# ultravideo/kvazzup

Hardware: AMD Instinct MI355X
Metric: hevc_encode_decode_fps (higher is better)
Workload: dtype u8

## Files before the change

### kvazzup_amd/csrc/enc_kernels.h

```cpp
#pragma once
#include <hip/hip_runtime.h>
#include "hevc_core.h"
namespace kvzx {
void launch_pad_input(const uint8_t *in, int w, int h, uint8_t *dy, uint8_t *du, uint8_t *dv, int cw, int ch, hipStream_t st);
void launch_me(const EncFrame &f, hipStream_t st);
void launch_luma_quarter(const uint8_t *src, uint8_t *q, int cw, int ch, hipStream_t st);
void launch_me_coarse(const EncFrame &f, hipStream_t st);
void launch_subpel(const EncFrame &f, hipStream_t st);
void launch_inter_recon(const EncFrame &f, hipStream_t st);
void launch_inter_signal(const EncFrame &f, hipStream_t st);
void launch_intra_analyse(const EncFrame &f, hipStream_t st);
void launch_intra_recon(const EncFrame &f, hipStream_t st);
void launch_deblock(const EncFrame &f, hipStream_t st);
void launch_vaq(const EncFrame &f, int vaq, int *act, int *sum, hipStream_t st);
void launch_sao(const EncFrame &f, hipStream_t st);
void launch_qp_resolve(const EncFrame &f, hipStream_t st);
void launch_deblock_v(const EncFrame &f, hipStream_t st);
void launch_deblock_h(const EncFrame &f, hipStream_t st, int part = 0);
void launch_tokenize(const EncFrame &f, hipStream_t st);
void launch_tok_compact(const EncFrame &f, hipStream_t st);
void launch_picture_begin(RcState *rc, uint32_t bits3, int slot3, int have3, int8_t *ctu_qt, const int8_t *roi, int nctu, int qp, int vaq, hipStream_t st,
                          void *zero_a = nullptr, size_t bytes_a = 0, void *zero_b = nullptr, size_t bytes_b = 0);
struct WpArgs {
  const unsigned long long *partial; int nblk;
  long long n;
  int64_t *stat;
  const int64_t *stat_ref[KVZ_MAX_LP_REFS];
  const uint8_t *in_ref[KVZ_MAX_LP_REFS];
  int nref;
  int32_t *cand; unsigned long long *acc;
  int32_t *rec, *rec_host;
};
struct WpPlaneArgs { const int32_t *rec; const uint8_t *from[KVZ_MAX_LP_REFS]; uint8_t *to[KVZ_MAX_LP_REFS]; };
int wp_stat_blocks(int height);
void launch_wp_stats(const uint8_t *src, int cw, int width, int height, unsigned long long *partial, hipStream_t st);
void launch_wp_decide(const WpArgs &a, int phase, hipStream_t st);
void launch_wp_check(const WpArgs &a, const uint8_t *cur, int cw, int width, int height, hipStream_t st);
void launch_wp_plane(const WpPlaneArgs &a, int nref, int cw, int ch, hipStream_t st);
struct CabacRowsArgs {
  const uint16_t *tok; const int32_t *count; const uint32_t *off;
  uint8_t *stage; uint32_t stage_cap;
  uint8_t *out; uint32_t out_cap;
  uint32_t *cursors;
  uint32_t *sub_off, *sub_len, *sub_bins;
  uint32_t *ctx_save, *ctx_ready;
  uint32_t gen;
  uint32_t *err;
  int wc, hc, wpp, tile_rows, init_type, qp, first_sub;
};
void launch_cabac_rows(const CabacRowsArgs &a, int nsub, hipStream_t st);
}
```

### kvazzup_amd/csrc/enc_kernels.hip

```cpp
#include <hip/hip_runtime.h>
#include <type_traits>
#include "hevc_core.h"
#include "enc_kernels.h"
#include "kernel_common.h"

namespace kvzx {

#define SPLIT_BITS 8
#define INTRA_P_GATE 24
#define INTRA_P_BITS 16

#define ME_MAXR 32
#define ME_WPITCH 100

template <bool MR, bool CO = false>
__global__ __launch_bounds__(256) void k_me(EncFrame f)
{
  using Key = typename std::conditional<MR || CO, unsigned long long, uint32_t>::type;
  constexpr int KS = CO ? 17 : (MR ? 16 : 13);
  constexpr Key KMAX = ~(Key)0;
  __shared__ __attribute__((aligned(16))) uint8_t wbuf[(32 + 2 * ME_MAXR + 1) * ME_WPITCH + 16];
  __shared__ __attribute__((aligned(16))) uint32_t cur[32 * 8];
  __shared__ Key red[5];
  const int tid = threadIdx.x, nthreads = blockDim.x;
  int bx_, by_; xcd_block_2d(bx_, by_);
  const int x0 = bx_ * 32, y0 = by_ * 32 + f.row0 * 64;
  const int R = f.range, W = 2 * R + 1, WW = 32 + 2 * R;
  const uint8_t *ref = f.me_ref, *src = f.src[0];
  const uint32_t lam = (uint32_t)f.lambda_q4;
  if (f.pb_on && blockIdx.x == 0 && blockIdx.y == 0) picture_begin_body(f.pb_rc, f.pb_bits3, f.pb_slot3, f.pb_have3, f.pb_qt, f.pb_roi, f.pb_nctu, f.qp, 0, tid, nthreads);
  if (tid == 0) red[0] = 0;
  __syncthreads();
  {
    uint32_t s0 = 0;
    for (int i = tid; i < 256; i += nthreads) {
      const size_t g = (size_t)(y0 + (i >> 3)) * f.cw + x0 + (i & 7) * 4;
      const uint32_t c = *reinterpret_cast<const uint32_t *>(src + g);
      cur[i] = c;
      if (f.me_early) s0 = __builtin_amdgcn_sad_u8(c, *reinterpret_cast<const uint32_t *>(ref + g), s0);
    }
    if (f.me_early) { s0 = wave_sum_u32(s0); if ((tid & 63) == 0) atomicAdd(&red[0], (Key)s0); }
  }
  __syncthreads();
  if (f.me_early && red[0] <= 64u * lam) {
    if (tid < 16) {
      const int i = b8idx(f, x0 + (tid & 3) * 8, y0 + (tid >> 2) * 8);
      f.cu_log2[i] = 5; f.cu_intra[i] = 0; f.cu_mv[i * 2] = 0; f.cu_mv[i * 2 + 1] = 0;
      f.cu_mvp_idx[i] = 0;
      if (MR) f.cu_ref[i] = 0;
    }
    if (f.intra_p && tid < 4) f.me_cost16[((y0 >> 4) + (tid >> 1)) * (f.cw >> 4) + (x0 >> 4) + (tid & 1)] = 0;
    return;
  }
  Key best[5] = {KMAX, KMAX, KMAX, KMAX, KMAX};
  const int nr = MR ? f.nref : 1;
#pragma unroll 1
  for (int it = 0; it < (CO ? 2 * nr : nr); it++) {
// ... 655 lines not shown
  __syncthreads();
  {
    auto px1 = [](int tu, int y, int x) { return tu * 256 + y * 16 + x; };
    auto px4 = [](int tu, int y, int x) { return (tu >> 2) * 256 + (((tu >> 1) & 1) * 8 + y) * 16 + (tu & 1) * 8 + x; };
    const size_t base = (size_t)(y0 >> 1) * cw2 + (x0 >> 1);
    int16_t *cb = f.coef[1] + base, *cr = f.coef[2] + base;
    auto ci1 = [=](int tu, int y, int x) { return (tu ? cr : cb) + (size_t)y * cw2 + x; };
    auto ci4 = [=](int tu, int y, int x) { return ((tu >> 2) ? cr : cb) + (size_t)(((tu >> 1) & 1) * 8 + y) * cw2 + (tu & 1) * 8 + x; };
    auto qpc_known = [&]() -> int { return qpc; };
    if constexpr (LL) { }
    else if (split) inter_transform<DEC, 3, 1, RC>(s, qpc, &s.nz[1], px4, ci4, tid, adj, qpc_known, &rc_cost, f.scaling ? f.scaling + scaling_offset(3, 1, 1) : nullptr, 4);
    else inter_transform<DEC, 4, 1, RC>(s, qpc, &s.nz[1], px1, ci1, tid, adj, qpc_known, &rc_cost, f.scaling ? f.scaling + scaling_offset(4, 1, 1) : nullptr, 1);
  }
  if (tid < 128) {
    const int pl = tid >> 6, y = (tid >> 2) & 15, x = (tid & 3) * 4;
    *(uint32_t *)&f.rec[1 + pl][(size_t)((y0 >> 1) + y) * cw2 + (x0 >> 1) + x] = *(const uint32_t *)&s.px[pl * 256 + y * 16 + x];
  }
  if (!DEC && tid < 16) {
    int bx = tid & 3, by = tid >> 2, k = split ? ((by >> 1) * 2 + (bx >> 1)) : 0;
    int cbf = (int)((s.nz[0] >> k) & 1);
    if (split) cbf |= (int)((s.nz[1] >> k) & 1) << 1 | (int)((s.nz[1] >> (4 + k)) & 1) << 2;
    else cbf |= (int)(s.nz[1] & 1) << 1 | (int)((s.nz[1] >> 1) & 1) << 2;
    f.cu_cbf[b8idx(f, x0 + bx * 8, y0 + by * 8)] = (uint8_t)cbf;
  }
  if constexpr (RC) rc_group_done(f, s, grp, rc_cost, tid);
}

template <bool TMVP, bool GOP = false>
__global__ __launch_bounds__(1024) void k_inter_signal(EncFrame f)
{
  const int w8 = f.cw >> 3, h8 = band_rows(f) * 8;
  const int i = blockIdx.x * blockDim.x + threadIdx.x;
  const bool valid = i < w8 * h8;
  const int x = valid ? (i % w8) * 8 : 0, y = valid ? (i / w8) * 8 + f.row0 * 64 : 0, g = b8idx(f, x, y);
  const int cl = f.cu_log2[g];
  const bool intra = f.cu_intra[g] != 0;
  int flags = 0;
  if (valid && !intra) {
    const int n = 1 << cl;
    CuSignal r;
    if constexpr (GOP) { FrameMvView v{f}; [[clang::always_inline]] r = decide_signalling_values(v, f.cw, f.chp, x & ~(n - 1), y & ~(n - 1), cl, f.cu_ref && f.nref > 1 ? f.nref : 1, TMVP ? f.col_prev : nullptr, TabDist{f.ref_dist}); }
    else if constexpr (TMVP) { FrameMvView v{f}; [[clang::always_inline]] r = decide_signalling_values(v, f.cw, f.chp, x & ~(n - 1), y & ~(n - 1), cl, f.cu_ref && f.nref > 1 ? f.nref : 1, f.col_prev); }
    else r = decide_signalling_values(f, x & ~(n - 1), y & ~(n - 1), cl);
    flags = r.flags;
    f.cu_flags[g] = (uint8_t)r.flags; f.cu_merge_idx[g] = (uint8_t)r.midx; f.cu_mvp_idx[g] = (uint8_t)r.mvp;
    *reinterpret_cast<uint32_t *>(&f.cu_mvd[g * 2]) = ((uint32_t)r.mvdx & 0xffffu) | ((uint32_t)r.mvdy << 16);
  }
  if constexpr (TMVP) {
    if (valid && !((x | y) & 15)) {
      ColMv c; c.mx = intra ? 0 : f.cu_mv[g * 2]; c.my = intra ? 0 : f.cu_mv[g * 2 + 1]; c.dist = intra ? 0 : (int16_t)(GOP ? TabDist{f.ref_dist}(cu_ref_at(f, g)) : cu_ref_at(f, g) + 1); c.pad = 0;
      f.col_out[(y >> 4) * (f.cw >> 4) + (x >> 4)] = c;
    }
  }
  if (f.tok_list) {
    uint32_t roles = 0;
    if (valid && !((x | y) & 15)) {
      const bool owner = !(cl == 5 && ((x | y) & 31));
      if (owner || ((x & 63) == 48 && (y & 63) == 48)) roles |= 8u;
      if (owner) {
        uint32_t cbf = 0;
        if (cl == 3) { cbf = f.cu_cbf[g] | f.cu_cbf[g + 1] | f.cu_cbf[g + w8] | f.cu_cbf[g + w8 + 1]; }
        else if (!(flags & CU_SKIP)) cbf = f.cu_cbf[g];
        roles |= cbf & 7u;
      }
    }
    const int lane = threadIdx.x & 63, nr = __builtin_popcount(roles);
    int pre = nr;
    for (int o = 1; o < 64; o <<= 1) { const int t = __shfl_up(pre, o); if (lane >= o) pre += t; }
    const int total = __shfl(pre, 63);
    uint32_t base = 0;
    if (lane == 63 && total) base = atomicAdd(&f.tok_list[0], (uint32_t)total);
    base = (uint32_t)__shfl((int)base, 63);
    uint32_t o = base + (uint32_t)(pre - nr);
    const uint32_t unit = (uint32_t)((y >> 4) * (f.cw >> 4) + (x >> 4));
    for (uint32_t m = roles; m; m &= m - 1) f.tok_list[1 + o++] = (unit << 2) | (uint32_t)__builtin_ctz(m);
  }
}

#ifdef KVZ_PROF
__shared__ long long g_prof[16];
#define PROF(k) do { if (threadIdx.x == 0) { long long t_ = clock64(); g_prof[k] += t_ - g_prof[15]; g_prof[15] = t_; } } while (0)
#else
#define PROF(k) do { } while (0)
#endif
struct IntraCtuLds {
  alignas(16) uint8_t pic[65 * 144];
  alignas(16) uint8_t src[64 * 64];
  alignas(16) int16_t lev[64 * 64];
  alignas(16) XfLaneF16 xf[4][64];
};


struct AnalyseLds {
  alignas(16) uint8_t src[32 * 32];
  alignas(16) uint8_t R[2][16 * 36 + 4 * 68 + 132];
  int dc[21];
  uint32_t cost[21][35];
  uint32_t bestc[21]; int bestm[21];
  int last;
  alignas(16) uint8_t srcT[32 * 32];
  alignas(16) uint8_t ext[16][4 * 32];
};
__device__ __forceinline__ int an_tile_of(int b) { return b < 16 ? (b >> 3) * 2 + ((b >> 1) & 1) : b - 16; }
__device__ __forceinline__ int an_roff(int b) { return b < 16 ? b * 36 : (b < 20 ? 16 * 36 + (b - 16) * 68 : 16 * 36 + 4 * 68); }

template <int L2>
__device__ __forceinline__ uint32_t analyse_item(const AnalyseLds &s, int b, int bx, int by, int mode, int lane)
{
  constexpr int N = 1 << L2;
  const bool filt = intra_filter_needed(N, 0, mode);
  const uint8_t *R = s.R[filt ? 1 : 0] + an_roff(b);
  const int angle = kIntraAngle[mode], inv = kInvAngle[mode];
  const bool edge = N < 32, vert = mode >= 18, e2 = edge && (mode == 26 || mode == 10);
  const int dcv = s.dc[b];
  uint32_t sad = 0;
#pragma unroll
  for (int it = 0; it < N * N / 64; it++) {
    const int pxi = it * 64 + lane, y = pxi >> L2, x = pxi & (N - 1);
    int p;
    if (mode == 0) p = pred_planar<L2>(R, x, y);
    else if (mode == 1) p = pred_dc<L2>(R, edge, dcv, x, y);
    else p = pred_angular<L2>(R, vert, e2, angle, inv, x, y);
    sad += (uint32_t)iabs((int)s.src[(by + y) * 32 + bx + x] - p);
  }
  return wave_sum_u32(sad);
}

__device__ __forceinline__ void analyse_tile_satd(AnalyseLds &s, int wave, int tile, int kind, int mode, int lane, uint32_t (&q)[4])
{
// ... 639 lines not shown
    } else *(uint32_t *)g = *(const uint32_t *)&ty_[y * P + x];
  }
  for (int i = tid; i < 2 * (TH / 2) * 9; i += 256) {
    const int pl = i / ((TH / 2) * 9), r = i - pl * ((TH / 2) * 9), y = r / 9, k = r - y * 9, gx = CX0 - 2 + 4 * k, gy = CY0 + y;
    if (gy < 0 || gx < 0) continue;
    uint8_t *g = &f.rec[1 + pl][(size_t)gy * cw2 + gx];
    const uint32_t v = *(const uint32_t *)&tc_[pl][y * PC + 4 * k];
    if (k == 0) *(uint16_t *)(g + 2) = (uint16_t)(v >> 16);
    else if (k == 8 && TW == 64) *(uint16_t *)g = (uint16_t)v;
    else *(uint32_t *)g = v;
  }
}

__global__ __launch_bounds__(256) void k_deblock_v(EncFrame f)
{
  int t = blockIdx.x * blockDim.x + threadIdx.x;
  int ne = (f.cw >> 3) - 1, ns = band_rows(f) * 16;
  if (t >= ne * ns) return;
  int x = ((t % ne) + 1) * 8, y = (t / ne) * 4 + f.row0 * 64;
  if (!is_cu_edge_v(f, x, y)) return;
  int bs = edge_bs(f, x - 1, y, x, y);
  if (!bs) return;
  const int qp = (cu_qpy(f, x - 1, y) + cu_qpy(f, x, y) + 1) >> 1;
  deblock_luma_segment(f.rec[0] + y * f.cw + x, 1, f.cw, bs, qp);
  if (bs == 2 && (x & 15) == 0) {
    int cw2 = f.cw >> 1;
    deblock_chroma_segment(f.rec[1] + (y >> 1) * cw2 + (x >> 1), 1, cw2, 2, qp);
    deblock_chroma_segment(f.rec[2] + (y >> 1) * cw2 + (x >> 1), 1, cw2, 2, qp);
  }
}
__global__ __launch_bounds__(256) void k_deblock_h(EncFrame f, int part)
{
  int t = blockIdx.x * blockDim.x + threadIdx.x;
  const int ylo = imax(8, f.row0 * 64), yhi = imin(f.ch - 8, (f.row0 + band_rows(f)) * 64);
  int ns = f.cw >> 2, ne = (yhi - ylo) / 8 + 1;
  if (t >= ne * ns) return;
  int x = (t % ns) * 4, y = ylo + (t / ns) * 8;
  if (part) {
    const bool boundary = y == f.row0 * 64 || y == (f.row0 + band_rows(f)) * 64;
    if (boundary != (part == 2)) return;
  }
  if (!is_cu_edge_h(f, x, y)) return;
  int bs = edge_bs(f, x, y - 1, x, y);
  if (!bs) return;
  const int qp = (cu_qpy(f, x, y - 1) + cu_qpy(f, x, y) + 1) >> 1;
  deblock_luma_segment(f.rec[0] + y * f.cw + x, f.cw, 1, bs, qp);
  if (bs == 2 && (y & 15) == 0) {
    int cw2 = f.cw >> 1;
    deblock_chroma_segment(f.rec[1] + (y >> 1) * cw2 + (x >> 1), cw2, 1, 2, qp);
    deblock_chroma_segment(f.rec[2] + (y >> 1) * cw2 + (x >> 1), cw2, 1, 2, qp);
  }
}

struct TileView {
  const CuRec *tile;
  int bx0, by0;
  __device__ CuRec at(int x, int y) const { return tile[((y >> 3) - by0) * 3 + ((x >> 3) - bx0)]; }
};

struct alignas(16) TokTabs { uint8_t sigk[3][5][16]; };
constexpr CoreTabs make_core_tabs() { CoreTabs t{}; for (int i = 0; i < 64; i++) core_tabs_fill_entry(t, i); return t; }
constexpr TokTabs make_tok_tabs()
{
  const CoreTabs c = make_core_tabs();
  TokTabs t{};
  for (int sc = 0; sc < 3; sc++) for (int k = 0; k < 16; k++) {
    for (int pc = 0; pc < 4; pc++) t.sigk[sc][pc][k] = c.sigpat[pc][c.pos4[sc][k]];
    t.sigk[sc][4][k] = c.ctxmap4x4[c.pos4[sc][k]];
  }
  return t;
}
static __device__ const CoreTabs g_core_tabs = make_core_tabs();
static __device__ const TokTabs g_tok_tabs = make_tok_tabs();
static_assert(sizeof(CoreTabs) % 4 == 0 && sizeof(TokTabs) % 16 == 0, "copied by dwords / 16-byte words");

struct SbRegs { uint32_t w[8]; uint32_t m; };
__device__ __forceinline__ int sb_level(const SbRegs &r, int k) { return (int)(int16_t)(uint16_t)(r.w[k >> 1] >> ((k & 1) * 16)); }

template <bool KEEP_LDS>
__device__ __forceinline__ void digest_build_wave(const CoreTabs *t, TuDigest &d, const int16_t *lv, int stride, int log2, int scan_idx, int lane, SbRegs &sb)
{
  const int sbl = log2 - 2, nsb2 = 1 << (2 * sbl);
  d.csbf[lane] = 0;
  wave_sync();
  bool nz = false;
  sb.m = 0;
#pragma unroll
  for (int k = 0; k < 8; k++) sb.w[k] = 0;
  if (lane < nsb2) {
    int xs, ys; scan_pos(t, scan_idx, sbl, lane, xs, ys);
    const int16_t *p = lv + (ys << 2) * stride + (xs << 2);
    uint2 r0 = *reinterpret_cast<const uint2 *>(p), r1 = *reinterpret_cast<const uint2 *>(p + stride);
    uint2 r2 = *reinterpret_cast<const uint2 *>(p + 2 * stride), r3 = *reinterpret_cast<const uint2 *>(p + 3 * stride);
    uint2 *dst = reinterpret_cast<uint2 *>(&d.scan[lane * 16]);
    dst[0] = r0; dst[1] = r1; dst[2] = r2; dst[3] = r3;
    const uint8_t *pos = t->pos4[scan_idx];
    int v[16];
    uint32_t m = 0;
#pragma unroll
    for (int k = 0; k < 16; k++) { v[k] = d.scan[lane * 16 + pos[k]]; if (v[k]) m |= 1u << k; }
#pragma unroll
    for (int k = 0; k < 8; k++) sb.w[k] = ((uint32_t)v[2 * k] & 0xffffu) | ((uint32_t)v[2 * k + 1] << 16);
    if (KEEP_LDS) {
      uint32_t *d32 = reinterpret_cast<uint32_t *>(&d.scan[lane * 16]);
#pragma unroll
      for (int k = 0; k < 8; k++) d32[k] = sb.w[k];
    }
    sb.m = m;
    d.mask[lane] = (uint16_t)m;
    nz = m != 0;
    if (nz) d.csbf[ys * 8 + xs] = 1;
  }
  uint64_t sb64 = __ballot(nz);
  if (lane == 0) d.sbmask = sb64;
  wave_sync();
}

__device__ __forceinline__ bool sb_g1_any(const SbRegs &r)
{
  bool any = false; int seen = 0;
#pragma unroll
  for (int k = 15; k >= 0; k--) if ((r.m >> k) & 1) { const int v = sb_level(r, k); if (seen < 8 && (v > 1 || v < -1)) any = true; seen++; }
  return any;
}

template <class S>
__device__ __forceinline__ void enc_subblock_regs(S &c, const TuDigest &d, const SbRegs &r, const uint32_t (&sk)[4], int i, int last_sb, int last_pos, bool prev_g1, int log2, int cidx, int scan_idx, int sign_hiding)
{
  const int sbl = log2 - 2, nsb = 1 << sbl;
  int xs, ys; scan_pos(c.tabs, scan_idx, sbl, i, xs, ys);
  const int right = (xs < nsb - 1) ? d.csbf[ys * 8 + xs + 1] : 0;
  const int below = (ys < nsb - 1) ? d.csbf[(ys + 1) * 8 + xs] : 0;
  const uint32_t m = r.m;
  int coded = m != 0, infer_dc = 0;
  if (i < last_sb && i > 0) {
    cabac_bin(c, CTX_CSBF + ((right | below) ? 1 : 0) + (cidx ? 2 : 0), coded);
    infer_dc = 1;
  } else coded = 1;
  if (!coded) return;
  const int sigbase = CTX_SIG + (cidx ? 27 : 0);
  const int off = log2 == 2 ? 0 : (cidx == 0 ? ((i > 0 ? 3 : 0) + ((log2 == 3) ? ((scan_idx == 0) ? 9 : 15) : 21)) : ((log2 == 3) ? 9 : 12));
  const int start = (i == last_sb) ? last_pos - 1 : 15;
  if constexpr (sink_counts_only<S>::value) {
    if (start >= 0) c.n += start + 1 - ((infer_dc && (m >> 1) == 0) ? 1 : 0);
  } else {
#pragma unroll
    for (int k = 15; k >= 1; k--) if (k <= start) cabac_bin(c, sigbase + (int)((sk[k >> 2] >> ((k & 3) * 8)) & 0xffu) + off, (int)((m >> k) & 1));
    if (start >= 0 && !(infer_dc && (m >> 1) == 0))
      cabac_bin(c, sigbase + ((i == 0 && log2 != 2) ? 0 : (int)(sk[0] & 0xffu) + off), (int)(m & 1));
  }
  if (!m) return;
  int ctx_set = (i > 0 && cidx == 0) ? 2 : 0;
  if (prev_g1) ctx_set++;
  int c1 = 1, nsig = 0, g1idx = -1, g2 = 0;
  uint32_t signs = 0;
#pragma unroll
  for (int k = 15; k >= 0; k--) if ((m >> k) & 1) {
    const int v = sb_level(r, k), a = v < 0 ? -v : v;
    signs = (signs << 1) | (v < 0 ? 1u : 0u);
    if (nsig < 8) {
      const int g1 = a > 1;
      cabac_bin(c, CTX_GT1 + (cidx ? 16 : 0) + ctx_set * 4 + c1, g1);
      if (g1) { c1 = 0; if (g1idx < 0) { g1idx = nsig; g2 = a > 2; } }
      else if (c1 > 0 && c1 < 3) c1++;
    }
    nsig++;
  }
  if (g1idx >= 0) cabac_bin(c, CTX_GT2 + (cidx ? 4 : 0) + ctx_set, g2);
  if (sign_hiding && (31 - __builtin_clz(m)) - __builtin_ctz(m) > 3) cabac_bypass_bits(c, signs >> 1, nsig - 1);
  else cabac_bypass_bits(c, signs, nsig);
  int rice = 0, j = 0;
#pragma unroll
  for (int k = 15; k >= 0; k--) if ((m >> k) & 1) {
    const int v = sb_level(r, k), a = v < 0 ? -v : v;
    const int base = (j < 8) ? ((j == g1idx) ? 3 : 2) : 1;
    if (a >= base) {
      enc_abs_remaining(c, a - base, rice);
      if (a > 3 * (1 << rice)) rice = imin(rice + 1, 4);
    }
    j++;
  }
}

#define TOK_HDR_CAP 192
#define TOK_ARENA 512
#define TOK_PIECES 17

#ifndef KVZ_TOK_WAVES
#define KVZ_TOK_WAVES 5
#endif
struct alignas(16) TokWave {
  TuDigest dg;
  TokTabs tk;
  CoreTabs tabs;
  CuRec tile[9];
  uint16_t hdr[TOK_HDR_CAP];
  uint16_t arena[TOK_ARENA];
  int hdr_n;
  uint32_t piece_off;
  uint32_t seg[TOK_PIECES][2];
};
template <bool ALLC, bool HDRW, bool REGS>
__device__ __forceinline__ void tok_unit(const EncFrame &f, TokWave &W, const int ux, const int uy, const int comp, const int lane, const bool have_tabs)
{
  CuRec *tile = W.tile; TuDigest &dg = W.dg; CoreTabs &tabs = W.tabs; uint16_t *hdr = W.hdr, *arena = W.arena;
  int &hdr_n = W.hdr_n; uint32_t &piece_off = W.piece_off; uint32_t (&seg)[TOK_PIECES][2] = W.seg;
  const int wc = f.cw >> 6, hc = f.ch >> 6;
  const int hdr_comp = HDRW ? 3 : 0;
  const bool hdr_role = ALLC || comp == hdr_comp;
  const int cx = ux >> 2, cy = uy >> 2, ctu = cy * wc + cx;
  const int X0 = ux * 16, Y0 = uy * 16;
  int z4 = 0;
  for (int b = 0; b < 2; b++) z4 |= (((ux & 3) >> b) & 1) << (2 * b) | (((uy & 3) >> b) & 1) << (2 * b + 1);
  unsigned long long *tr = (f.trace && hdr_role && lane == 0 && (z4 == 0 || z4 == 15)) ? f.trace + (size_t)wc * hc * 32 + (size_t)ctu * 8 : nullptr;
  if (tr) tr[z4 == 0 ? 5 : 6] = wall_clock64();
  unsigned long long *census = f.trace ? f.trace + (size_t)wc * hc * 40 + (size_t)ctu * 16 + (f.is_intra ? 6 : 0) : nullptr;
  const unsigned long long t_begin = census ? wall_clock64() : 0;
  int wave_class = 1;
#ifdef KVZ_TOK_PHASES
  unsigned long long *ph = (f.trace && comp == 0 && !f.is_intra) ? f.trace + (size_t)wc * hc * 56 + (size_t)ctu * 16 : nullptr;
  unsigned long long ph_t[9]; int ph_n = 0;
#define TOK_PH() do { if (ph && ph_n < 9) ph_t[ph_n++] = wall_clock64(); } while (0)
#define TOK_PH_SYNC() wave_sync()
#else
#define TOK_PH() do { } while (0)
#define TOK_PH_SYNC() do { } while (0)
#endif
  TOK_PH();
  auto mine = [&](int piece) { return ALLC || ((piece == 16 || (piece & 3) == 0) ? hdr_comp : (piece & 3) - 1) == comp; };
  if (!(hdr_role && z4 == 15)) {
    const int g0 = (uy * 2) * f.b8w + ux * 2, l0 = f.cu_log2[g0];
    bool work = !(l0 == 5 && ((X0 | Y0) & 31));
    if (!ALLC && work && comp != hdr_comp) {
      bool c = false;
      if (lane < (l0 == 3 ? 4 : 1)) { const int g = g0 + (lane >> 1) * f.b8w + (lane & 1); c = !(f.cu_flags[g] & CU_SKIP) && ((f.cu_cbf[g] >> comp) & 1); }
      work = __ballot(c) != 0;
    }
    if (!work) {
      if (lane < TOK_PIECES && mine(lane)) { uint32_t *e = f.tok_seg + ((size_t)(ctu * 16 + z4) * TOK_PIECES + lane) * 2; e[0] = 0; e[1] = 0; }
      if (census && lane == 0) { atomicAdd(&census[0], 1ull); atomicAdd(&census[1], wall_clock64() - t_begin); }
      return;
    }
  }
  TOK_PH();
  if (!have_tabs) {
    for (int i = lane; i < (int)(sizeof(CoreTabs) / 4); i += 64) reinterpret_cast<uint32_t *>(&tabs)[i] = reinterpret_cast<const uint32_t *>(&g_core_tabs)[i];
    if (lane < (int)(sizeof(TokTabs) / 16)) reinterpret_cast<uint4 *>(&W.tk)[lane] = reinterpret_cast<const uint4 *>(&g_tok_tabs)[lane];
  }
  if (lane < TOK_PIECES) { seg[lane][0] = 0; seg[lane][1] = 0; }
  if (lane == 0) hdr_n = 0;
  const int bx0 = ux * 2 - 1, by0 = uy * 2 - 1;
  if (lane < 9) {
    int bx = bx0 + lane % 3, by = by0 + lane / 3;
    CuRec r; r.log2 = 0; r.intra = 0; r.flags = 0; r.merge_idx = 0; r.mvp_idx = 0; r.intra_mode = 0; r.cbf = 0; r.ref = 0; r.mvdx = 0; r.mvdy = 0;
    if (bx >= 0 && by >= 0) {
      int g = by * f.b8w + bx;
      r.log2 = f.cu_log2[g]; r.intra = f.cu_intra[g]; r.flags = f.cu_flags[g]; r.merge_idx = f.cu_merge_idx[g];
      r.mvp_idx = f.cu_mvp_idx[g]; r.intra_mode = f.cu_intra_mode[g]; r.cbf = f.cu_cbf[g];
      r.mvdx = f.cu_mvd[g * 2]; r.mvdy = f.cu_mvd[g * 2 + 1]; r.ref = (uint8_t)cu_ref_at(f, g);
    }
    tile[lane] = r;
  }
  wave_sync();
  TOK_PH();
  uint16_t *slot = f.tok_buf + (size_t)ctu * f.tok_cap;
  int np = 0;
  auto reserve = [&](int total) -> uint32_t {
    if (lane == 0) {
      uint32_t o = atomicAdd(&f.tok_cursor[ctu], (uint32_t)total);
      if (o + (uint32_t)total > (uint32_t)f.tok_cap) { atomicOr(f.err, 16u); o = ~0u; }
      else { seg[np][0] = o; seg[np][1] = (uint32_t)total; }
      piece_off = o;
    }
    wave_sync();
    return piece_off;
  };
  TileView v; v.tile = tile; v.bx0 = bx0; v.by0 = by0;
  const int cl0 = v.at(X0, Y0).log2;
  const bool owner = !(cl0 == 5 && ((X0 | Y0) & 31));
  const int ncu = owner ? (cl0 == 3 ? 4 : 1) : 0;
  for (int k = 0; k < ncu; k++) {
    const int x0 = X0 + ((cl0 == 3) ? (k & 1) * 8 : 0), y0 = Y0 + ((cl0 == 3) ? (k >> 1) * 8 : 0);
    const CuRec cu = v.at(x0, y0);
    int z = 0;
    for (int b = 0; b < 3; b++) z |= ((((x0 & 63) >> 3) >> b) & 1) << (2 * b) | ((((y0 & 63) >> 3) >> b) & 1) << (2 * b + 1);
    if (lane == 0 && hdr_role) {
      TokOut t; t.tabs = &tabs; t.p = hdr; t.n = 0; t.cap = TOK_HDR_CAP;
      if (f.sao && z4 == 0 && k == 0) {
        const bool hl = cx > 0 && !tile_col_starts_at(wc, f.tile_cols, cx), hu = cy > 0 && !tile_row_starts_at(hc, f.tile_rows, cy);
        enc_sao(t, f.sao[ctu], hl ? &f.sao[ctu - 1] : nullptr, hu ? &f.sao[ctu - wc] : nullptr);
      }
      enc_split_flags(v, t, f.cw, f.chp, x0, y0, z, cu.log2);
      enc_cu_header(v, t, f.cw, f.chp, f.is_intra != 0, x0, y0, cu, f.lossless != 0, f.cu_ref ? f.nref : 1);
      if (f.ctu_qy && !(cu.flags & CU_SKIP) && cu.cbf && z == f.ctu_first[ctu]) enc_cu_qp_delta(t, f.ctu_delta[ctu]);
      hdr_n = t.n;
    }
    TOK_PH_SYNC(); TOK_PH();
    if (hdr_role) {
      np = 4 * k;
      wave_sync();
      const int hn = hdr_n > TOK_HDR_CAP ? TOK_HDR_CAP : hdr_n;
      if (hdr_n > TOK_HDR_CAP && lane == 0) atomicOr(f.err, 8u);
      const uint32_t o = reserve(hn);
      if (o != ~0u) for (int i = lane; i < hn; i += 64) slot[o + i] = hdr[i];
      wave_sync();
      if (lane == 0) hdr_n = 0;
      wave_sync();
    }
    const int cbf = (cu.flags & CU_SKIP) ? 0 : cu.cbf;
    for (int ci = (ALLC || comp == 3) ? 0 : comp; ci < (ALLC ? 3 : (comp == 3 ? 0 : comp + 1)); ci++) {
      np = 4 * k + 1 + ci;
      if ((cbf >> ci) & 1) {
        wave_class = 2;
        const int l2 = ci ? cu.log2 - 1 : cu.log2, pw = ci ? (f.cw >> 1) : f.cw;
        const int px = ci ? (x0 >> 1) : x0, py = ci ? (y0 >> 1) : y0;
        const int scan = intra_scan_idx(cu.intra, l2, ci, cu.intra_mode);
        SbRegs sb;
        digest_build_wave<!REGS>(&tabs, dg, f.coef[ci] + py * pw + px, pw, l2, scan, lane, sb);
        TOK_PH();
        const uint64_t sbm = dg.sbmask;
        const int last_sb = 63 - __builtin_clzll(sbm);
        const int last_pos = 31 - __builtin_clz((uint32_t)dg.mask[last_sb]);
        if (lane == 0) {
          TokOut t; t.tabs = &tabs; t.p = hdr; t.n = hdr_n; t.cap = TOK_HDR_CAP;
          int a, b; enc_last_pos(t, dg, l2, ci, scan, a, b);
          hdr_n = t.n;
        }
        const bool nzsb = (sbm >> lane) & 1;
        const bool g1 = nzsb && sb_g1_any(sb);
        const uint64_t g1m = __ballot(g1);
        bool prev_g1 = false;
        if (lane <= last_sb) {
          uint64_t above = (lane < 63) ? (sbm >> (lane + 1)) : 0;
          if (above) { int j = lane + 1 + __builtin_ctzll(above); prev_g1 = (g1m >> j) & 1; }
        }
        uint32_t sk[4] = {0, 0, 0, 0};
        if (lane <= last_sb) {
          const int sbl = l2 - 2, nsb = 1 << sbl;
          int xs, ys; scan_pos(&tabs, scan, sbl, lane, xs, ys);
          const int right = (xs < nsb - 1) ? dg.csbf[ys * 8 + xs + 1] : 0, below = (ys < nsb - 1) ? dg.csbf[(ys + 1) * 8 + xs] : 0;
          const uint4 q = *reinterpret_cast<const uint4 *>(W.tk.sigk[scan][l2 == 2 ? 4 : (right | (below << 1))]);
          sk[0] = q.x; sk[1] = q.y; sk[2] = q.z; sk[3] = q.w;
        }
        int n_l = 0;
        if (lane <= last_sb) {
          TokCount t; t.tabs = &tabs; t.n = 0;
          if (REGS) enc_subblock_regs(t, dg, sb, sk, lane, last_sb, last_pos, prev_g1, l2, ci, scan, f.signhide);
          else enc_subblock(t, dg, lane, last_sb, last_pos, prev_g1, l2, ci, scan, f.signhide);
          n_l = t.n;
        }
        int suffix = n_l;
        for (int o = 1; o < 64; o <<= 1) { int other = __shfl_down(suffix, o); if (lane + o < 64) suffix += other; }
        const int body = __shfl(suffix, 0);
        const int off = suffix - n_l;
        wave_sync();
        const int hn = hdr_n > TOK_HDR_CAP ? TOK_HDR_CAP : hdr_n, total = hn + body;
        if (hdr_n > TOK_HDR_CAP && lane == 0) atomicOr(f.err, 8u);
        TOK_PH();
        const uint32_t o = reserve(total);
        TOK_PH();
        if (o != ~0u) {
          const bool staged = total <= TOK_ARENA;
          uint16_t *dst = staged ? arena : slot + o;
          for (int i = lane; i < hn; i += 64) dst[i] = hdr[i];
          if (lane <= last_sb && n_l) {
            TokOut t; t.tabs = &tabs; t.p = dst + hn + off; t.n = 0; t.cap = n_l;
            if (REGS) enc_subblock_regs(t, dg, sb, sk, lane, last_sb, last_pos, prev_g1, l2, ci, scan, f.signhide);
            else enc_subblock(t, dg, lane, last_sb, last_pos, prev_g1, l2, ci, scan, f.signhide);
          }
          if (staged) {
            wave_sync();
            for (int i = lane; i < total; i += 64) slot[o + i] = arena[i];
          }
        }
        wave_sync();
        TOK_PH();
        if (lane == 0) hdr_n = 0;
      }
      wave_sync();
    }
  }
  if (z4 == 15 && hdr_role) {
    const bool last = (cy == hc - 1 && cx == wc - 1);
    const bool row_end = tile_col_ends_at(wc, f.tile_cols, cx);
    const bool sub_end = row_end && (f.wpp || tile_row_ends_at(hc, f.tile_rows, cy));
    const bool seg_end = last || (row_end && (f.slices == 1 || (f.slices == 2 && tile_row_ends_at(hc, f.tile_rows, cy))));
    const int n = 1 + ((sub_end && !seg_end) ? 1 : 0);
    wave_sync();
    np = 16;
    const uint32_t o = reserve(n);
    if (o != ~0u && lane == 0) {
      slot[o] = (uint16_t)(0xC000u | (seg_end ? 1u : 0u));
      if (n == 2) slot[o + 1] = 0xC001u;
    }
  }
  wave_sync();
  if (lane < TOK_PIECES && mine(lane)) {
    uint32_t *e = f.tok_seg + ((size_t)(ctu * 16 + z4) * TOK_PIECES + lane) * 2;
    e[0] = seg[lane][0]; e[1] = seg[lane][1];
  }
  TOK_PH();
#ifdef KVZ_TOK_PHASES
  if (ph && lane == 0 && ph_n == 9 && ncu == 1 && wave_class == 2) { for (int k = 0; k < 8; k++) atomicAdd(&ph[k], ph_t[k + 1] - ph_t[k]); atomicAdd(&ph[15], 1ull); }
#endif
#undef TOK_PH
#undef TOK_PH_SYNC
  if (tr && z4 == 15) tr[7] = wall_clock64();
  if (census && lane == 0) { atomicAdd(&census[wave_class * 2], 1ull); atomicAdd(&census[wave_class * 2 + 1], wall_clock64() - t_begin); }
}
template <bool ALLC, int NW, bool HDRW = true, bool REGS = true, bool LIST = false>
__global__ __launch_bounds__(NW * 64) __attribute__((amdgpu_waves_per_eu(REGS ? (LIST ? 3 : KVZ_TOK_WAVES) : 6))) void k_tokenize(EncFrame f)
{
  __shared__ TokWave tw[NW];
  const int wv = threadIdx.x >> 6, lane = threadIdx.x & 63;
  TokWave &W = tw[wv];
  if constexpr (LIST) {
    const uint32_t count = f.tok_list[0], uw = (uint32_t)(f.cw >> 4);
    bool have = false;
    for (uint32_t it = blockIdx.x; it < count; it += gridDim.x) {
      const uint32_t v = f.tok_list[1 + it], unit = v >> 2;
      tok_unit<ALLC, HDRW, REGS>(f, W, (int)(unit % uw), (int)(unit / uw), (int)(v & 3u), lane, have);
      have = true;
      wave_sync();
    }
  } else {
    const int ux = NW == 4 ? blockIdx.x * 2 + (wv & 1) : blockIdx.x, uy = NW == 4 ? (blockIdx.y + f.row0 * 2) * 2 + (wv >> 1) : blockIdx.y + f.row0 * 4, comp = ALLC ? 0 : (int)blockIdx.z;
    tok_unit<ALLC, HDRW, REGS>(f, W, ux, uy, comp, lane, false);
  }
}

__global__ __launch_bounds__(256) void k_tok_compact(EncFrame f)
{
  constexpr int NSEG = 16 * TOK_PIECES;
  __shared__ uint32_t soff[NSEG], start[NSEG + 1], utot[17];
  __shared__ uint32_t wsum[4];
  const int first = f.row0 * (f.cw >> 6), ctu = blockIdx.x + first, tid = threadIdx.x;
  unsigned long long *tr = f.trace ? f.trace + (size_t)(f.cw >> 6) * (f.ch >> 6) * 32 + (size_t)ctu * 8 : nullptr;
#define TC_STAMP(k) do { if (tr && tid == 0) tr[k] = wall_clock64(); } while (0)
  TC_STAMP(0);
  const uint32_t n = f.tok_cursor[ctu];
  uint32_t part = 0;
  for (int i = first + tid; i < ctu; i += 256) part += f.tok_cursor[i];
  part = wave_sum_u32(part);
  if ((tid & 63) == 0) wsum[tid >> 6] = part;
  if (tid == 0) { f.tok_cursor_next[ctu] = 0; if (blockIdx.x == 0) { *f.err_out = *f.err; if (f.ent_cursors) { f.ent_cursors[0] = 0; f.ent_cursors[1] = 0; } } }
  __syncthreads();
  const uint32_t base = wsum[0] + wsum[1] + wsum[2] + wsum[3];
  TC_STAMP(1);
  uint32_t *tab = f.tok_seg + (size_t)ctu * NSEG * 2;
  for (int i = tid; i < NSEG; i += 256) { const uint2 e = *reinterpret_cast<const uint2 *>(&tab[i * 2]); soff[i] = e.x; start[i] = e.y; *reinterpret_cast<uint2 *>(&tab[i * 2]) = make_uint2(0u, 0u); }
  if (f.tok_list && blockIdx.x == 0 && tid == 0) f.tok_list[0] = 0;
  if (base + n > f.tok_dense_cap) { if (tid == 0) f.tok_count_out[ctu] = -1; return; }
  __syncthreads();
  TC_STAMP(2);
  if (tid < 16) { uint32_t a = 0; for (int p = 0; p < TOK_PIECES; p++) { uint32_t l = start[tid * TOK_PIECES + p]; start[tid * TOK_PIECES + p] = a; a += l; } utot[tid] = a; }
  __syncthreads();
  if (tid == 0) { uint32_t a = 0; for (int u = 0; u < 16; u++) { uint32_t t = utot[u]; utot[u] = a; a += t; } utot[16] = a; }
  __syncthreads();
  for (int i = tid; i < NSEG; i += 256) start[i] += utot[i / TOK_PIECES];
  if (tid == 0) start[NSEG] = utot[16];
  __syncthreads();
  const uint32_t total = start[NSEG];
  TC_STAMP(3);
  if (total != n) { if (tid == 0) f.tok_count_out[ctu] = -1; return; }
  const uint16_t *slot = f.tok_buf + (size_t)ctu * f.tok_cap;
  uint16_t *dst = f.tok_dense + base;
  int lo = 0;
  for (uint32_t i = tid; i < n; i += 256) {
    if (start[lo + 1] <= i) {
      int hi = NSEG;
      while (hi - lo > 1) { int mid = (lo + hi) >> 1; if (start[mid] <= i) lo = mid; else hi = mid; }
    }
    dst[i] = slot[soff[lo] + (i - start[lo])];
  }
  if (tid == 0) { f.tok_off_out[ctu] = base; f.tok_count_out[ctu] = (int32_t)n; }
  TC_STAMP(4);
#undef TC_STAMP
}

__global__ __launch_bounds__(256) void k_pad_input(const uint8_t *in, int w, int h, uint8_t *dy, uint8_t *du, uint8_t *dv, int cw, int ch)
{
  int y0 = blockIdx.y * 16 + threadIdx.y * 4, plane = 0;
  if (y0 >= ch) { y0 -= ch; plane = 1; if (y0 >= ch / 2) { y0 -= ch / 2; plane = 2; } }
  const int pw = plane ? w / 2 : w, ph = plane ? h / 2 : h, pcw = plane ? cw / 2 : cw;
  const int x = (blockIdx.x * 64 + threadIdx.x) * 16;
  if (x >= pcw) return;
  const uint8_t *src = in + (plane == 0 ? 0 : (plane == 1 ? (size_t)w * h : (size_t)w * h + (size_t)(w / 2) * (h / 2)));
  uint8_t *dst = plane == 0 ? dy : (plane == 1 ? du : dv);
  kv_u32x4 v[4];
#pragma unroll
  for (int k = 0; k < 4; k++) {
    const uint8_t *row = src + (size_t)imin(y0 + k, ph - 1) * pw;
    if (x + 16 <= pw && (((uintptr_t)(row + x)) & 3) == 0) v[k] = *reinterpret_cast<const kv_u32x4 *>(row + x);
    else {
      uint32_t q[4] = {0, 0, 0, 0};
      for (int i = 0; i < 16; i++) q[i >> 2] |= (uint32_t)row[imin(x + i, pw - 1)] << (8 * (i & 3));
      v[k].x = q[0]; v[k].y = q[1]; v[k].z = q[2]; v[k].w = q[3];
    }
  }
#pragma unroll
  for (int k = 0; k < 4; k++) *reinterpret_cast<kv_u32x4 *>(dst + (size_t)(y0 + k) * pcw + x) = v[k];
}

#define KVZ_SAO_THREADS 1024
struct SaoLds {
  alignas(4) uint8_t win[66 * 72];
  alignas(4) uint8_t winc[2][34 * 40];
  int en[3][4][5], es[3][4][5], bn[3][32][16], bs[3][32][16];
  int eo_off[3][4][4], eo_dist[3][4][4], bo_off[3][32], bo_gain[3][32];
  int cand_dist[3][5], cand_bins[3][5], cand_band[3];
  SaoParams p;
};
__device__ __forceinline__ int sao_edge_idx(int c, int a, int b)
{
  const int e = 2 + ((c > a) - (c < a)) + ((c > b) - (c < b));
  return e == 2 ? 0 : (e < 2 ? e + 1 : e);
}
__device__ __forceinline__ int sao_rdiv(int a, int b) { return b == 0 ? 0 : (a >= 0 ? (2 * a + b) / (2 * b) : -((-2 * a + b) / (2 * b))); }
__device__ __forceinline__ int sao_off_bins(int o) { const int a = o < 0 ? -o : o; return a < 7 ? a + 1 : 7; }

template <int ROWS>
__device__ __forceinline__ void sao_stats_column(SaoLds &s, int c, const uint8_t *w, int pitch, int x, int ys, bool okh, int Y0, int ph, const int *o8, int tid)
{
  auto sgn = [](int d) { return d > 1 ? 1 : (d < -1 ? -1 : d); };
  const uint8_t *col = w + 4 + x - 1;
  int r0[3], r1[3], r2[3];
  for (int k = 0; k < 3; k++) { r0[k] = col[ys * pitch + k]; r1[k] = col[(ys + 1) * pitch + k]; }
  uint64_t acc[4] = {0, 0, 0, 0};
  int run_b = -1, run_n = 0, run_s = 0;
  int s_up = sgn(r1[1] - r0[1]);
// ... 284 lines not shown
void launch_intra_recon(const EncFrame &f, hipStream_t st)
{
  static const int diags_env = getenv("KVAZZUP_AMD_INTRA_DIAGS") ? atoi(getenv("KVAZZUP_AMD_INTRA_DIAGS")) : -1;
  const int diags = diags_env >= 0 ? diags_env : (f.chain_diags ? f.chain_diags : 3);
  const int wc = f.cw / 64, nr = band_rows(f), diag = nr < (wc + 1) / 2 ? nr : (wc + 1) / 2, want = diags > 0 ? 3 * diags * diag + 32 : 3 * wc * nr;
  const dim3 grid(want < 3 * wc * nr ? want : 3 * wc * nr), block(64 * KVZ_INTRA_WAVES);
  const bool adj = f.rdoq || f.signhide;
  if (!f.is_intra) {
    const dim3 all(3 * wc * nr);
    if (f.lossless) { hipLaunchKernelGGL((k_intra_recon<false, true, false, true>), all, block, 0, st, f); return; }
    if (f.scaling) { if (adj) hipLaunchKernelGGL((k_intra_recon<true, true, true>), all, block, 0, st, f); else hipLaunchKernelGGL((k_intra_recon<false, true, true>), all, block, 0, st, f); }
    else if (adj) hipLaunchKernelGGL((k_intra_recon<true, true>), all, block, 0, st, f); else hipLaunchKernelGGL((k_intra_recon<false, true>), all, block, 0, st, f);
    return;
  }
  if (f.lossless) hipLaunchKernelGGL((k_intra_recon<false, false, false, true>), grid, block, 0, st, f);
  else if (f.scaling) { if (adj) hipLaunchKernelGGL((k_intra_recon<true, false, true>), grid, block, 0, st, f); else hipLaunchKernelGGL((k_intra_recon<false, false, true>), grid, block, 0, st, f); }
  else if (adj) hipLaunchKernelGGL((k_intra_recon<true, false>), grid, block, 0, st, f);
  else hipLaunchKernelGGL((k_intra_recon<false, false>), grid, block, 0, st, f);
}
void launch_qp_resolve(const EncFrame &f, hipStream_t st)
{
  if (!f.ctu_qy) return;
  const int n = (f.cw / 64) * band_rows(f);
  if (f.wpp && f.cw / 64 <= 256) { hipLaunchKernelGGL(k_qp_rows, dim3(band_rows(f)), dim3(256), 0, st, f); return; }
  hipLaunchKernelGGL(k_qp_first, dim3(n), dim3(64), 0, st, f);
  hipLaunchKernelGGL(k_qp_chain, dim3((n + 255) / 256), dim3(256), 0, st, f);
}
void launch_deblock_v(const EncFrame &f, hipStream_t st)
{
  int nv = ((f.cw >> 3) - 1) * (band_rows(f) * 16);
  hipLaunchKernelGGL(k_deblock_v, dim3((nv + 255) / 256), dim3(256), 0, st, f);
}
void launch_deblock_h(const EncFrame &f, hipStream_t st, int part)
{
  const int ylo = imax(8, f.row0 * 64), yhi = imin(f.ch - 8, (f.row0 + band_rows(f)) * 64);
  int nh = (f.cw >> 2) * ((yhi - ylo) / 8 + 1);
  hipLaunchKernelGGL(k_deblock_h, dim3((nh + 255) / 256), dim3(256), 0, st, f, part);
}
void launch_deblock(const EncFrame &f, hipStream_t st)
{
  if (f.nrows > 0) { launch_deblock_v(f, st); launch_deblock_h(f, st, 0); return; }
  hipLaunchKernelGGL(k_deblock_tile, dim3((f.cw / 64) * (f.ch / 64)), dim3(256), 0, st, f);
}
void launch_vaq(const EncFrame &f, int vaq, int *act, int *sum, hipStream_t st)
{
  const int nctu = (f.cw / 64) * (f.ch / 64);
  hipMemsetAsync(sum, 0, sizeof(int), st);
  hipLaunchKernelGGL(k_vaq_stats, dim3(nctu), dim3(256), 0, st, f, act, sum);
  hipLaunchKernelGGL(k_vaq_apply, dim3((nctu + 255) / 256), dim3(256), 0, st, f, vaq, (const int *)act, (const int *)sum, nctu);
}
void launch_sao(const EncFrame &f, hipStream_t st) { hipLaunchKernelGGL(k_sao<false>, dim3((f.cw / 64) * (f.ch / 64)), dim3(KVZ_SAO_THREADS), 0, st, f); }
void launch_tokenize(const EncFrame &f, hipStream_t st)
{
  const int units = (f.cw / 16) * band_rows(f) * 4;
  static const int list_mode = [] { const char *e = getenv("KVAZZUP_AMD_TOK_LIST"); return e ? atoi(e) : -1; }();
  if (!f.is_intra && f.tok_list && f.nrows == 0 && units < 65536 && (list_mode > 0 || (list_mode < 0 && units > 16384))) {
    hipLaunchKernelGGL((k_tokenize<false, 1, true, true, true>), dim3(units / 2 < 256 ? 256 : units / 2), dim3(64), 0, st, f);
    return;
  }
  if (units >= 65536) hipLaunchKernelGGL((k_tokenize<true, 1>), dim3(f.cw / 16, band_rows(f) * 4), dim3(64), 0, st, f);
  else if (units > 16384) hipLaunchKernelGGL((k_tokenize<false, 1, false, false>), dim3(f.cw / 16, band_rows(f) * 4, 3), dim3(64), 0, st, f);
  else hipLaunchKernelGGL((k_tokenize<false, 1, true>), dim3(f.cw / 16, band_rows(f) * 4, 4), dim3(64), 0, st, f);
}
void launch_tok_compact(const EncFrame &f, hipStream_t st)
{
  hipLaunchKernelGGL(k_tok_compact, dim3((f.cw / 64) * band_rows(f)), dim3(256), 0, st, f);
}

}
```

### kvazzup_amd/csrc/encoder.h

```cpp
#pragma once
#include <hip/hip_runtime.h>
#include <stdint.h>
#include <condition_variable>
#include <deque>
#include <mutex>
#include <string>
#include <thread>
#include <vector>
#include "hevc_core.h"
#include "hevc_headers.h"
#include "entropy_host.h"
#include "enc_kernels.h"

namespace kvzx {

enum KernelId { K_PAD = 0, K_ME, K_INTER_RECON, K_INTER_SIGNAL, K_INTRA_ANALYSE, K_INTRA_RECON, K_DEBLOCK, K_TOKENIZE, K_HOST_ARITH, K_SAO, K_TOK_COMPACT, K_CABAC_ROWS, K_SUBPEL, K_INTRA_ANALYSE_P, K_INTRA_RECON_P, K_COUNT };

struct EncoderConfig {
  int width = 0, height = 0;
  int qp = 32, intra_period = 64, vps_period = 1;
  int me_range = 16;
  int fps_num = 30, fps_den = 1;
  int wpp = 1, deblock = 1;
  int band_row0 = 0, band_rows = 0;
// ... 100 lines not shown
  hipEvent_t ev_h2d_[kInRing] = {}, ev_pad_[kInRing] = {}; bool pad_pending_[kInRing] = {}, h2d_pending_[kInRing] = {};
  long in_count_ = 0;
  hipStream_t stream_rec_ = nullptr;
  static constexpr int kSets = 8;
  uint8_t *src_[kSets][3] = {};
  static constexpr int kMaxDepth = 16;
  static constexpr int kMaxRefDist = kSets - 1;
  static constexpr int kRecRing = kMaxDepth + 2 + kMaxRefDist;
  uint8_t *rec_[kRecRing][3] = {};
  bool spin_wait_ = false;
  int rc_delay_ = 3;
  int nrec_ = 3;
  int cur_idx_ = 0, ref_idx_ = 2, out_idx_ = 2;
  int16_t *coef_[kSets][3] = {};
  uint8_t *cu_bytes_[kSets] = {};
  int16_t *cu_mv_[kSets] = {}, *cu_mvd_[kSets] = {};
  uint8_t *cu_ref_[kSets] = {};
  uint8_t *mc_q_[kSets] = {}; int16_t *mc_centres_[kSets] = {};
  ColMv *col_[kSets] = {};
  int set_ = 0, out_set_ = 0;
  int32_t out_gop_[8] = {0, 0, 0, 0, 0, 0, 0, 0};
  unsigned long long *wp_partial_[kSets] = {}; int64_t *wp_stat_[kSets] = {}; int32_t *wp_rec_[kSets] = {};
  int32_t *wp_cand_ = nullptr; unsigned long long *wp_acc_ = nullptr; uint8_t *wp_plane_[KVZ_MAX_LP_REFS] = {};
  int32_t out_wp_[3 * KVZ_MAX_LP_REFS] = {0, 64, 0, 0, 64, 0, 0, 64, 0, 0, 64, 0};
  bool wp_stage(const EncFrame &f, const Plan &p, const Slot &sl);
  EncFrame wp_search_frame(const EncFrame &f, const Plan &p, hipStream_t st);
  char prio_[3] = {'h', 'n', 'n'};
  std::vector<int8_t> roi_; int roi_w_ = 0, roi_h_ = 0;
  std::vector<int8_t> roi_sub_; int roi_sub_w_ = 0, roi_sub_h_ = 0;
  int8_t *ctu_qt_[kSets] = {}, *ctu_qy_[kSets] = {}, *ctu_delta_[kSets] = {}; uint8_t *ctu_first_[kSets] = {};
  int8_t *h_ctu_qt_[kSets] = {};
  int8_t *ctu_roi_[kSets] = {};
  bool stage_roi(hipStream_t st);
  const int8_t *roi_dev_ = nullptr;
  int *vaq_act_ = nullptr, *vaq_sum_ = nullptr;
  uint32_t next_chain_gen();
  bool picture_begin(const EncFrame &f, hipStream_t qt_stream, EncFrame *fold = nullptr, bool zero = false);
  int qp_cur_ = 0; int64_t rc_debt_ = 0; uint32_t rc_bytes_[8] = {0, 0, 0, 0, 0, 0, 0, 0}; uint32_t rc_known_ = 0;
  void rate_control();
  RcState *rc_state_ = nullptr;
  bool band_picture_setup();
  EncFrame band_f_{};
  hipStream_t stream_tok_ = nullptr;
  hipStream_t stream_in_ = nullptr;
  hipEvent_t ev_src_free_[kSets] = {}; bool src_busy_[kSets] = {};
  uint8_t *work_[3] = {nullptr, nullptr, nullptr};
  SaoParams *sao_[kSets] = {};

  hipStream_t stream_idr_ = nullptr; hipEvent_t ev_idr_done_ = nullptr; bool idr_pending_ = false, idr_side_ = false, all_intra_alt_ = false;
  uint32_t *sync_idr_ = nullptr; uint32_t *edge_col_idr_ = nullptr; uint32_t chain_gen_ = 0; unsigned long long *edge_row_ = nullptr, *edge_row_idr_ = nullptr; uint8_t *work_idr_[3] = {nullptr, nullptr, nullptr};
  hipEvent_t ev_signalled_ = nullptr, ev_tok_done_[kSets] = {}; bool tok_pending_[kSets] = {};
  uint8_t *intra_scratch_ = nullptr;
  uint8_t *d_scaling_ = nullptr;
  uint16_t *tok_buf_ = nullptr; int tok_cap_ = 0; int32_t *tok_count_ = nullptr; uint32_t *tok_seg_ = nullptr; uint32_t *tok_list_ = nullptr; int tok_nctu_ = 0;
  size_t tok_dense_cap_ = 0;
  std::vector<std::vector<uint8_t>> band_subs_; uint64_t band_bins_ = 0; bool band_coded_ = false;
  bool me_ahead_ = false; uint32_t *me_block_[kSets] = {}; uint32_t *sync_set_[kSets] = {}; int prev_set_ = 0;
  uint32_t *sync_ = nullptr; uint32_t *me_cost16_ = nullptr; uint32_t *edge_col_ = nullptr; uint32_t *intra_order_ = nullptr; uint32_t *err_ = nullptr; unsigned long long *trace_ = nullptr;
  struct EvPair { hipEvent_t a, b; KernelId id; };
  struct Slot {
    uint16_t *h_tok_dense = nullptr, *d_tok_dense = nullptr; int32_t *h_tok_count = nullptr, *d_tok_count = nullptr;
    uint32_t *h_tok_off = nullptr, *d_tok_off = nullptr;
    uint32_t *h_err = nullptr, *d_err = nullptr;
    int32_t *h_wp = nullptr, *d_wp = nullptr;
    uint16_t *g_tok = nullptr; int32_t *g_count = nullptr; uint32_t *g_off = nullptr;
    uint8_t *g_stage = nullptr; uint32_t *g_cursors = nullptr, *g_ctx_save = nullptr, *g_ctx_ready = nullptr;
    uint8_t *h_out = nullptr, *d_out = nullptr; uint32_t *h_sub = nullptr, *d_sub = nullptr;
    hipStream_t ent_stream = nullptr; hipEvent_t tok_ev = nullptr; uint32_t gen = 0;
    hipEvent_t done = nullptr, rec_done = nullptr;
    hipEvent_t sink_done = nullptr; bool has_sink = false;
    int poc = 0, rec_idx = 0, set = 0, qp = 0; bool intra = false, write_ps = false; long pic_idx = 0;
    int layer = 0, nref = 0; int8_t dist[KVZ_MAX_LP_REFS] = {0, 0, 0, 0};
    std::vector<EvPair> ev; size_t ev_used = 0;
    EncodedPicture result; bool ready = false, ok = true;
    EncFrame f_tok{}; bool prof = false, tok_failed = false;
  };
  Slot slot_[kMaxDepth + 2]; Slot *cur_slot_ = nullptr; int nslots_ = 1, depth_ = 0;
  size_t stage_cap_ = 0, out_cap_ = 0;
  std::thread bg_[2]; std::mutex bm_; std::condition_variable bcv_; std::deque<int> bq_; bool bquit_ = false;
  bool tok_deferred_ = false; std::thread tok_thread_; std::mutex tm_; std::condition_variable tcv_; std::deque<int> tq_; bool tquit_ = false;
  void tok_launcher();
  bool launch_tokenizer(Slot &sl, const EncFrame &f, bool intra, bool wait_on_stream, bool prof);
  void timed_slot(Slot &sl, bool prof, KernelId id, hipStream_t st, const std::function<void()> &launch);
  std::mutex stat_m_;
  long submitted_ = 0, collected_ = 0, accepted_ = 0;
  struct SubmitJob { const uint8_t *src = nullptr; bool host = false; std::vector<int8_t> roi; int roi_w = 0, roi_h = 0; int slot = 0; uint8_t *sink[3] = {nullptr, nullptr, nullptr}; };
  uint8_t *sink_[3] = {nullptr, nullptr, nullptr}, *sink_sub_[3] = {nullptr, nullptr, nullptr};
  std::thread sub_thread_; std::mutex sm_; std::condition_variable scv_; std::deque<SubmitJob> sq_; bool squit_ = false, sbusy_ = false;
  void submitter();
  void drain_submitter();
  bool enqueue(const uint8_t *src, bool host, EncodedPicture *out);
  bool upload_and_submit(const uint8_t *y, const uint8_t *u, const uint8_t *v, bool pinned);
  hipEvent_t in_done_ = nullptr; bool in_pending_ = false;
  EntropyHost *entropy_ = nullptr, *entropy2_ = nullptr;
  std::vector<std::vector<uint8_t>> rows_out_, rows_out2_;
  int frame_idx_ = 0, poc_ = 0, intra_count_ = 0;
  bool profiling_ = false, prof_now_ = false; int prof_every_ = 1;
  double t_submit_ = 0, t_wait_ = 0, t_arith_ = 0, t_asm_ = 0, t_in_ = 0;
  double k_ms_[K_COUNT] = {0}; uint64_t k_n_[K_COUNT] = {0};
  StreamParams sp_{};
};

}
```

### kvazzup_amd/csrc/encoder.hip

```cpp
#include <chrono>
#include <functional>
#include <cstdio>
#include <cstdlib>
#include <cstring>
#include "encoder.h"
#include "enc_kernels.h"
#include "stream_pool.h"
#include "scaling_tables.h"
#include "pic_hash.h"

namespace kvzx {

static const unsigned kDeviceEvent = hipEventDisableTiming | hipEventDisableSystemFence;

#define HIP_OK(expr) do { hipError_t e_ = (expr); if (e_ != hipSuccess) { if (error) *error = std::string(#expr) + ": " + hipGetErrorString(e_); return false; } } while (0)
#define HIP_CHECK(expr) do { hipError_t e_ = (expr); if (e_ != hipSuccess) { fprintf(stderr, "kvazzup_amd: %s failed: %s\n", #expr, hipGetErrorString(e_)); return false; } } while (0)

static void point_me_block(EncFrame &f, uint32_t *block)
{
  const size_t n16 = (size_t)(f.cw / 16) * (f.ch / 16);
  f.me_cost16 = block; f.me_cand = block + n16;
  f.ip_arrive = f.me_cand + 1 + n16 / 4; f.ip_scratch = (uint64_t *)(block + ((n16 + 1 + n16 / 4 + n16 / 4 + 1) & ~(size_t)1));
}

// ... 83 lines not shown
    HIP_OK(hipMalloc(&cu_bytes_[k], nb8 * 7)); HIP_OK(hipMemset(cu_bytes_[k], 0, nb8 * 7));
    HIP_OK(hipMalloc(&cu_mv_[k], nb8 * 2 * sizeof(int16_t))); HIP_OK(hipMemset(cu_mv_[k], 0, nb8 * 2 * sizeof(int16_t)));
    HIP_OK(hipMalloc(&cu_mvd_[k], nb8 * 2 * sizeof(int16_t))); HIP_OK(hipMemset(cu_mvd_[k], 0, nb8 * 2 * sizeof(int16_t)));
    if (cfg.lp_refs > 1) { HIP_OK(hipMalloc(&cu_ref_[k], nb8)); HIP_OK(hipMemset(cu_ref_[k], 0, nb8)); }
    if (cfg.tmvp) { HIP_OK(hipMalloc(&col_[k], nb8 / 4 * sizeof(ColMv))); HIP_OK(hipMemset(col_[k], 0, nb8 / 4 * sizeof(ColMv))); }
    if (cfg.me_coarse) {
      HIP_OK(hipMalloc(&mc_q_[k], npx / 16)); HIP_OK(hipMemset(mc_q_[k], 0, npx / 16));
      HIP_OK(hipMalloc(&mc_centres_[k], (size_t)KVZ_MAX_LP_REFS * (nb8 / 16) * 2 * sizeof(int16_t))); HIP_OK(hipMemset(mc_centres_[k], 0, (size_t)KVZ_MAX_LP_REFS * (nb8 / 16) * 2 * sizeof(int16_t)));
    }
    if (cfg.weightp) {
      HIP_OK(hipMalloc(&wp_partial_[k], (size_t)wp_stat_blocks(cfg.height) * 2 * sizeof(unsigned long long)));
      HIP_OK(hipMalloc(&wp_stat_[k], 2 * sizeof(int64_t))); HIP_OK(hipMemset(wp_stat_[k], 0, 2 * sizeof(int64_t)));
      HIP_OK(hipMalloc(&wp_rec_[k], 3 * KVZ_MAX_LP_REFS * sizeof(int32_t))); HIP_OK(hipMemset(wp_rec_[k], 0, 3 * KVZ_MAX_LP_REFS * sizeof(int32_t)));
    }
    HIP_OK(hipEventCreateWithFlags(&ev_tok_done_[k], kDeviceEvent));
  }
  if (cfg.weightp) {
    HIP_OK(hipMalloc(&wp_cand_, 3 * KVZ_MAX_LP_REFS * sizeof(int32_t))); HIP_OK(hipMalloc(&wp_acc_, 2 * KVZ_MAX_LP_REFS * sizeof(unsigned long long)));
    for (int r = 0; r < cfg.lp_refs; r++) HIP_OK(hipMalloc(&wp_plane_[r], npx));
  }
  if (cfg.qp_in_cu) {
    const size_t nctu = (size_t)(cw_ / 64) * rows_;
    for (int k = 0; k < kSets; k++) {
      HIP_OK(hipMalloc(&ctu_qt_[k], nctu)); HIP_OK(hipMalloc(&ctu_qy_[k], nctu)); HIP_OK(hipMalloc(&ctu_delta_[k], nctu)); HIP_OK(hipMalloc(&ctu_first_[k], nctu));
      HIP_OK(hipHostMalloc(&h_ctu_qt_[k], nctu, hipHostMallocDefault));
      HIP_OK(hipMalloc(&ctu_roi_[k], nctu));
    }
    if (cfg.vaq > 0) { HIP_OK(hipMalloc(&vaq_act_, nctu * sizeof(int))); HIP_OK(hipMalloc(&vaq_sum_, sizeof(int))); }
  }
  if (cfg.sao) {
    for (int c = 0; c < 3; c++) HIP_OK(hipMalloc(&work_[c], c ? npx / 4 : npx));
    for (int k = 0; k < kSets; k++) HIP_OK(hipMalloc(&sao_[k], sizeof(SaoParams) * (size_t)(cw_ / 64) * rows_));
  }
  if (cfg.rc_bands > 0) { HIP_OK(hipMalloc(&rc_state_, sizeof(RcState))); HIP_OK(hipMemset(rc_state_, 0, sizeof(RcState))); }
  HIP_OK(stream_acquire(&stream_tok_, cfg.device, 'T', prio_[1]));
  HIP_OK(stream_acquire(&stream_in_, cfg.device, 'I', prio_[2]));
  for (int k = 0; k < kSets; k++) HIP_OK(hipEventCreateWithFlags(&ev_src_free_[k], kDeviceEvent));
  HIP_OK(hipEventCreateWithFlags(&ev_signalled_, kDeviceEvent));
  idr_side_ = depth_ >= 2 && cfg.vaq == 0 && cfg.band_rows == 0 && cfg.intra_period != 1;
  all_intra_alt_ = depth_ >= 2 && cfg.vaq == 0 && cfg.band_rows == 0 && cfg.intra_period == 1;
  if (idr_side_ || all_intra_alt_) {
    const size_t nsync = ((size_t)rows_ * (cw_ / 64) * 3 + 2 + 3) & ~(size_t)3, nctu_ = (size_t)(cw_ / 64) * rows_;
    HIP_OK(hipMalloc(&sync_idr_, sizeof(uint32_t) * nsync)); HIP_OK(hipMemset(sync_idr_, 0, sizeof(uint32_t) * nsync));
    HIP_OK(hipMalloc(&edge_col_idr_, nctu_ * 128 * sizeof(uint32_t))); HIP_OK(hipMemset(edge_col_idr_, 0, nctu_ * 128 * sizeof(uint32_t)));
    HIP_OK(hipMalloc(&edge_row_idr_, nctu_ * 32 * 8)); HIP_OK(hipMemset(edge_row_idr_, 0, nctu_ * 32 * 8));
    if (cfg.sao) { const size_t npx_ = (size_t)cw_ * ch_; for (int c = 0; c < 3; c++) HIP_OK(hipMalloc(&work_idr_[c], c ? npx_ / 4 : npx_)); }
    if (all_intra_alt_) HIP_OK(stream_acquire(&stream_idr_, cfg.device, 'X', prio_[0])); else stream_idr_ = stream_in_;
    HIP_OK(hipEventCreateWithFlags(&ev_idr_done_, kDeviceEvent));
  }
  size_t isz = nb8 * 4 + nb8 + nb8 / 4 + nb8 + nb8 / 4 + nb8 / 16 + 64;
  HIP_OK(hipMalloc(&intra_scratch_, isz));
  const int nctu = (cw_ / 64) * rows_;
  tok_cap_ = 49152;
  HIP_OK(hipMalloc(&tok_buf_, (size_t)nctu * tok_cap_ * sizeof(uint16_t)));
  HIP_OK(hipMalloc(&tok_count_, sizeof(uint32_t) * nctu * 2));
  HIP_OK(hipMalloc(&tok_seg_, sizeof(uint32_t) * nctu * 16 * 17 * 2));
  HIP_OK(hipMemset(tok_seg_, 0, sizeof(uint32_t) * nctu * 16 * 17 * 2));
  if (cfg.band_rows == 0) { HIP_OK(hipMalloc(&tok_list_, sizeof(uint32_t) * (1 + (size_t)nctu * 16 * 4))); HIP_OK(hipMemset(tok_list_, 0, sizeof(uint32_t) * (1 + (size_t)nctu * 16 * 4))); }
  HIP_OK(hipMemset(tok_count_, 0, sizeof(uint32_t) * nctu * 2)); tok_nctu_ = nctu;
  tok_dense_cap_ = (size_t)nctu * tok_cap_;
  if (tok_dense_cap_ > ((size_t)1 << 27)) tok_dense_cap_ = (size_t)1 << 27;
  spin_wait_ = getenv("KVAZZUP_AMD_SPIN") != nullptr;
  nslots_ = depth_ + 1;
  stage_cap_ = tok_dense_cap_ * 2 + 256 * (size_t)rows_; if (stage_cap_ > 0xfff00000u) stage_cap_ = 0xfff00000u;
  out_cap_ = (size_t)cw_ * ch_ * 3 + 4096; if (out_cap_ > stage_cap_) out_cap_ = stage_cap_;
  for (int i = 0; i < nslots_; i++) {
    Slot &sl = slot_[i];
    void *dp = nullptr;
    if (cfg.entropy_gpu) {
      HIP_OK(hipMalloc(&sl.g_tok, tok_dense_cap_ * sizeof(uint16_t)));
      HIP_OK(hipMalloc(&sl.g_count, sizeof(int32_t) * nctu)); HIP_OK(hipMalloc(&sl.g_off, sizeof(uint32_t) * nctu));
      sl.d_tok_dense = sl.g_tok; sl.d_tok_count = sl.g_count; sl.d_tok_off = sl.g_off;
      HIP_OK(hipMalloc(&sl.g_stage, stage_cap_));
      HIP_OK(hipMalloc(&sl.g_cursors, 2 * sizeof(uint32_t))); HIP_OK(hipMemset(sl.g_cursors, 0, 2 * sizeof(uint32_t)));
      HIP_OK(hipMalloc(&sl.g_ctx_save, sizeof(uint32_t) * 40 * rows_));
      HIP_OK(hipMalloc(&sl.g_ctx_ready, sizeof(uint32_t) * rows_)); HIP_OK(hipMemset(sl.g_ctx_ready, 0, sizeof(uint32_t) * rows_));
      HIP_OK(hipHostMalloc(&sl.h_out, out_cap_, hipHostMallocMapped));
      HIP_OK(hipHostGetDevicePointer(&dp, sl.h_out, 0)); sl.d_out = (uint8_t *)dp;
      HIP_OK(hipHostMalloc(&sl.h_sub, sizeof(uint32_t) * 3 * rows_, hipHostMallocMapped));
      HIP_OK(hipHostGetDevicePointer(&dp, sl.h_sub, 0)); sl.d_sub = (uint32_t *)dp;
      HIP_OK(stream_acquire(&sl.ent_stream, cfg.device, 'E', 'l'));
      HIP_OK(hipEventCreateWithFlags(&sl.tok_ev, hipEventDisableTiming));
    } else {
      HIP_OK(hipHostMalloc(&sl.h_tok_dense, tok_dense_cap_ * sizeof(uint16_t), hipHostMallocMapped));
      HIP_OK(hipHostMalloc(&sl.h_tok_count, sizeof(int32_t) * nctu, hipHostMallocMapped));
      HIP_OK(hipHostGetDevicePointer(&dp, sl.h_tok_dense, 0)); sl.d_tok_dense = (uint16_t *)dp;
      HIP_OK(hipHostGetDevicePointer(&dp, sl.h_tok_count, 0)); sl.d_tok_count = (int32_t *)dp;
      HIP_OK(hipHostMalloc(&sl.h_tok_off, sizeof(uint32_t) * nctu, hipHostMallocMapped));
      HIP_OK(hipHostGetDevicePointer(&dp, sl.h_tok_off, 0)); sl.d_tok_off = (uint32_t *)dp;
    }
    HIP_OK(hipHostMalloc(&sl.h_err, sizeof(uint32_t), hipHostMallocMapped)); *sl.h_err = 0;
    HIP_OK(hipHostGetDevicePointer(&dp, sl.h_err, 0)); sl.d_err = (uint32_t *)dp;
    if (cfg.weightp) {
      HIP_OK(hipHostMalloc(&sl.h_wp, 3 * KVZ_MAX_LP_REFS * sizeof(int32_t), hipHostMallocMapped));
      for (int r = 0; r < KVZ_MAX_LP_REFS; r++) { sl.h_wp[3 * r] = 0; sl.h_wp[3 * r + 1] = 64; sl.h_wp[3 * r + 2] = 0; }
      HIP_OK(hipHostGetDevicePointer(&dp, sl.h_wp, 0)); sl.d_wp = (int32_t *)dp;
    }
    HIP_OK(hipEventCreateWithFlags(&sl.done, hipEventDisableTiming));
    HIP_OK(hipEventCreateWithFlags(&sl.rec_done, hipEventDisableTiming));
  }
  HIP_OK(hipEventCreateWithFlags(&in_done_, kDeviceEvent));
  HIP_OK(hipMalloc(&sync_, sizeof(uint32_t) * ((rows_ * (cw_ / 64) * 3 + 2 + 3) & ~3))); HIP_OK(hipMemset(sync_, 0, sizeof(uint32_t) * ((rows_ * (cw_ / 64) * 3 + 2 + 3) & ~3)));
  if (cfg.intra_in_p) { const size_t n16 = (size_t)(cw_ / 16) * (ch_ / 16); HIP_OK(hipMalloc(&me_cost16_, sizeof(uint32_t) * (n16 + 2 + n16 / 4 + n16 / 4 + (n16 / 4) * 40))); HIP_OK(hipMemset(me_cost16_, 0, sizeof(uint32_t) * (n16 + 2 + n16 / 4 + n16 / 4 + (n16 / 4) * 40))); }
  me_ahead_ = cfg.me_source != 0;
  if (me_ahead_ && cfg.intra_in_p) {
    const size_t n16 = (size_t)(cw_ / 16) * (ch_ / 16), nme = sizeof(uint32_t) * (n16 + 2 + n16 / 4 + n16 / 4 + (n16 / 4) * 40), nsy = sizeof(uint32_t) * ((rows_ * (cw_ / 64) * 3 + 2 + 3) & ~3);
    for (int k = 0; k < kSets; k++) { HIP_OK(hipMalloc(&me_block_[k], nme)); HIP_OK(hipMemset(me_block_[k], 0, nme)); HIP_OK(hipMalloc(&sync_set_[k], nsy)); HIP_OK(hipMemset(sync_set_[k], 0, nsy)); }
  }
  {
    const int wc = cw_ / 64, r0 = cfg.band_rows > 0 ? cfg.band_row0 : 0, nr = cfg.band_rows > 0 ? cfg.band_rows : rows_;
    std::vector<uint32_t> order;
    for (int d = 0; d < wc + 2 * nr; d++) for (int cy = 0; cy < nr; cy++) { const int cx = d - 2 * cy; if (cx >= 0 && cx < wc) order.push_back((uint32_t)((r0 + cy) * wc + cx)); }
    HIP_OK(hipMalloc(&intra_order_, sizeof(uint32_t) * order.size()));
    HIP_OK(hipMemcpy(intra_order_, order.data(), sizeof(uint32_t) * order.size(), hipMemcpyHostToDevice));
  }
  { const size_t nctu = (size_t)(cw_ / 64) * rows_; HIP_OK(hipMalloc(&edge_col_, nctu * 128 * sizeof(uint32_t))); HIP_OK(hipMemset(edge_col_, 0, nctu * 128 * sizeof(uint32_t)));
    HIP_OK(hipMalloc(&edge_row_, nctu * 32 * 8)); HIP_OK(hipMemset(edge_row_, 0, nctu * 32 * 8)); }
  HIP_OK(hipMalloc(&err_, sizeof(uint32_t))); HIP_OK(hipMemset(err_, 0, sizeof(uint32_t)));
  if (getenv("KVAZZUP_AMD_INTRA_TRACE")) { HIP_OK(hipMalloc(&trace_, sizeof(unsigned long long) * (rows_ * (cw_ / 64) * 72))); HIP_OK(hipMemset(trace_, 0, sizeof(unsigned long long) * (rows_ * (cw_ / 64) * 72))); }
  int eth = cfg.entropy_threads;
  if (const char *e = getenv("KVAZZUP_AMD_ENTROPY_THREADS")) eth = atoi(e) < 1 ? 1 : atoi(e);
  if (cfg.entropy_gpu) { entropy_ = nullptr; entropy2_ = nullptr; }
  else if (cfg.owf >= 2 && eth >= 4) {
    entropy_ = new EntropyHost((eth + 1) / 2 < rows_ ? (eth + 1) / 2 : rows_);
    entropy2_ = new EntropyHost(eth / 2 < rows_ ? eth / 2 : rows_);
  } else entropy_ = new EntropyHost(eth < rows_ ? eth : rows_);

  if (cfg.scaling_list) {
    uint8_t tab[KVZ_SCALING_BYTES];
    scaling_factors(scaling_defaults(), tab);
    HIP_OK(hipMalloc(&d_scaling_, KVZ_SCALING_BYTES)); HIP_OK(hipMemcpy(d_scaling_, tab, KVZ_SCALING_BYTES, hipMemcpyHostToDevice));
  }
  EncFrame &b = base_;
  b.cw = cw_; b.ch = ch_; b.b8w = cw_ / 8; b.b8h = ch_ / 8;
  b.tile_rows = cfg.tile_rows; b.tile_cols = cfg.tile_cols; b.chp = pack_height(ch_, cfg.tile_rows, cfg.tile_cols);
  b.row0 = cfg.band_rows > 0 ? cfg.band_row0 : 0; b.nrows = cfg.band_rows > 0 ? cfg.band_rows : 0;
  b.range = cfg.me_range; b.scaling = d_scaling_; b.intra_chain = cfg.intra_chain;
  b.lossless = cfg.lossless; b.rdoq = cfg.rdoq; b.signhide = cfg.signhide; b.intra_p = cfg.intra_in_p;
  if (me_cost16_) point_me_block(b, me_cost16_);
  b.wpp = cfg.wpp; b.mv_frame = cfg.mv_frame; b.me_early = cfg.me_early; b.satd = cfg.satd; b.subme = cfg.subme; b.slices = cfg.slices;
  uint8_t *p = intra_scratch_;
  b.ic8 = (uint32_t *)p; p += nb8 * 4; b.ic16 = (uint32_t *)p; p += nb8; b.ic32 = (uint32_t *)p; p += nb8 / 4;
  b.im8 = p; p += nb8; b.im16 = p; p += nb8 / 4; b.im32 = p;
  b.tok_buf = tok_buf_; b.tok_cap = tok_cap_; b.tok_seg = tok_seg_; b.tok_list = tok_list_; b.tok_dense_cap = (uint32_t)tok_dense_cap_;
  point_chain(b, sync_, edge_col_, edge_row_);
  b.err = err_; b.trace = trace_; b.intra_order = intra_order_;
  b.analyse_alone = depth_ < 2 && cfg.band_rows == 0 ? 1 : 0;
  b.chain_diags = all_intra_alt_ ? 2 : 0;

  sp_.cw = cw_; sp_.ch = ch_; sp_.width = cfg.width; sp_.height = cfg.height; sp_.qp = cfg.qp; sp_.wpp = cfg.wpp; sp_.tile_rows = cfg.tile_rows; sp_.tile_cols = cfg.tile_cols; sp_.qp_in_cu = cfg.qp_in_cu; sp_.sao = cfg.sao; sp_.slices = cfg.slices; sp_.signhide = cfg.signhide; sp_.scaling_list = cfg.scaling_list; sp_.tq_bypass = cfg.lossless;
  sp_.lp_refs = cfg.lp_refs > 1 ? cfg.lp_refs : 0;
  sp_.tmvp = cfg.tmvp;
  sp_.weightp = cfg.weightp;
  sp_.deblock = cfg.deblock; sp_.fps_num = cfg.fps_num; sp_.fps_den = cfg.fps_den;
  HIP_OK(hipStreamSynchronize(stream_));
  HIP_OK(hipDeviceSynchronize());
  tok_deferred_ = depth_ >= 2 && cfg.sao && !cfg.entropy_gpu && cfg.band_rows == 0 && cfg.owf <= kSets - 1;
  HIP_OK(hipDeviceSynchronize());
  if (tok_deferred_) tok_thread_ = std::thread([this] { name_this_thread("kvzx-enc-tok"); tok_launcher(); });
  if (depth_ >= 2) { bg_[0] = std::thread([this] { name_this_thread("kvzx-enc-bg0"); background(0); }); if (entropy2_) bg_[1] = std::thread([this] { name_this_thread("kvzx-enc-bg1"); background(1); }); }
  if (depth_ >= 2 && cfg.band_rows == 0) sub_thread_ = std::thread([this] { name_this_thread("kvzx-enc-sub"); submitter(); });
  return true;
}

namespace { struct Tick { std::chrono::steady_clock::time_point t0 = std::chrono::steady_clock::now(); double ms() const { return std::chrono::duration<double, std::milli>(std::chrono::steady_clock::now() - t0).count(); } }; }

Encoder::~Encoder()
{
  if (getenv("KVAZZUP_AMD_TRACE")) fprintf(stderr, "kvazzup_amd encoder thread ms: submit %.1f  wait_gpu %.1f  arith %.1f  assemble %.1f  wait_input %.1f  (pictures %ld)\n", t_submit_, t_wait_, t_arith_, t_asm_, t_in_, collected_);
  { std::lock_guard<std::mutex> l(sm_); squit_ = true; }
  scv_.notify_all();
  if (sub_thread_.joinable()) sub_thread_.join();
  { std::lock_guard<std::mutex> l(tm_); tquit_ = true; }
  tcv_.notify_all();
  if (tok_thread_.joinable()) tok_thread_.join();
  { std::lock_guard<std::mutex> l(bm_); bquit_ = true; }
  bcv_.notify_all();
  for (auto &t : bg_) if (t.joinable()) t.join();
  if (stream_) hipStreamSynchronize(stream_);
  if (stream_idr_ && stream_idr_ != stream_in_) hipStreamSynchronize(stream_idr_);
  if (stream_tok_) hipStreamSynchronize(stream_tok_);
  if (stream_in_) hipStreamSynchronize(stream_in_);
  for (Slot &sl : slot_) {
    for (auto &e : sl.ev) { hipEventDestroy(e.a); hipEventDestroy(e.b); }
    if (sl.sink_done) { hipEventSynchronize(sl.sink_done); hipEventDestroy(sl.sink_done); }
    if (sl.h_tok_dense) hipHostFree(sl.h_tok_dense);
    if (sl.h_tok_count) hipHostFree(sl.h_tok_count);
    if (sl.h_err) hipHostFree(sl.h_err);
    if (sl.h_wp) hipHostFree(sl.h_wp);
    if (sl.h_tok_off) hipHostFree(sl.h_tok_off);
    stream_release(sl.ent_stream, cfg_.device, 'E', 'l');
    if (sl.tok_ev) hipEventDestroy(sl.tok_ev);
    hipFree(sl.g_tok); hipFree(sl.g_count); hipFree(sl.g_off); hipFree(sl.g_stage); hipFree(sl.g_cursors); hipFree(sl.g_ctx_save); hipFree(sl.g_ctx_ready);
    if (sl.h_out) hipHostFree(sl.h_out);
    if (sl.h_sub) hipHostFree(sl.h_sub);
    if (sl.done) hipEventDestroy(sl.done);
    if (sl.rec_done) hipEventDestroy(sl.rec_done);
  }
  if (in_done_) hipEventDestroy(in_done_);
  for (int k = 0; k < kInRing; k++) { hipFree(d_in_[k]); if (h_in_[k]) hipHostFree(h_in_[k]); if (ev_h2d_[k]) hipEventDestroy(ev_h2d_[k]); if (ev_pad_[k]) hipEventDestroy(ev_pad_[k]); }
  stream_release(stream_rec_, cfg_.device, 'R', 'n');
  for (int c = 0; c < 3; c++) { for (int k = 0; k < kSets; k++) { hipFree(src_[k][c]); hipFree(coef_[k][c]); } for (int b = 0; b < kRecRing; b++) hipFree(rec_[b][c]); }
  hipFree(vaq_act_); hipFree(vaq_sum_); hipFree(rc_state_);
  for (int k = 0; k < kSets; k++) { hipFree(ctu_qt_[k]); hipFree(ctu_qy_[k]); hipFree(ctu_delta_[k]); hipFree(ctu_first_[k]); if (h_ctu_qt_[k]) hipHostFree(h_ctu_qt_[k]); hipFree(ctu_roi_[k]); }
  for (int k = 0; k < kSets; k++) { hipFree(cu_bytes_[k]); hipFree(cu_mv_[k]); hipFree(cu_mvd_[k]); if (cu_ref_[k]) hipFree(cu_ref_[k]); if (col_[k]) hipFree(col_[k]); if (mc_q_[k]) hipFree(mc_q_[k]); if (mc_centres_[k]) hipFree(mc_centres_[k]); if (ev_tok_done_[k]) hipEventDestroy(ev_tok_done_[k]); }
  for (int k = 0; k < kSets; k++) { hipFree(wp_partial_[k]); hipFree(wp_stat_[k]); hipFree(wp_rec_[k]); }
  hipFree(wp_cand_); hipFree(wp_acc_); for (int r = 0; r < KVZ_MAX_LP_REFS; r++) hipFree(wp_plane_[r]);
  for (int c = 0; c < 3; c++) { hipFree(work_[c]); hipFree(work_idr_[c]); }
  hipFree(sync_idr_); hipFree(edge_col_idr_); hipFree(edge_row_); hipFree(edge_row_idr_);
  for (int k = 0; k < kSets; k++) hipFree(sao_[k]);
  if (ev_signalled_) hipEventDestroy(ev_signalled_);
  for (int k = 0; k < kSets; k++) if (ev_src_free_[k]) hipEventDestroy(ev_src_free_[k]);
  stream_release(stream_tok_, cfg_.device, 'T', prio_[1]);
  stream_release(stream_in_, cfg_.device, 'I', prio_[2]);
  if (stream_idr_ && stream_idr_ != stream_in_) stream_release(stream_idr_, cfg_.device, 'X', prio_[0]);
  if (ev_idr_done_) hipEventDestroy(ev_idr_done_);
  hipFree(intra_scratch_); hipFree(d_scaling_);
  delete entropy_; delete entropy2_;
  for (int k = 0; k < kSets; k++) { hipFree(me_block_[k]); hipFree(sync_set_[k]); }
  hipFree(trace_); hipFree(intra_order_); hipFree(tok_buf_); hipFree(tok_count_); hipFree(tok_seg_); hipFree(tok_list_); hipFree(sync_); hipFree(me_cost16_); hipFree(edge_col_); hipFree(err_);
  stream_release(stream_, cfg_.device, 'M', prio_[0]);
}

void Encoder::timed(KernelId id, hipStream_t st, const std::function<void()> &launch) { timed_slot(*cur_slot_, prof_now_, id, st, launch); }
void Encoder::timed_slot(Slot &sl, bool prof, KernelId id, hipStream_t st, const std::function<void()> &launch)
{
  if (!prof) { launch(); return; }
  if (sl.ev_used == sl.ev.size()) {
    EvPair p; hipEventCreate(&p.a); hipEventCreate(&p.b); p.id = id; sl.ev.push_back(p);
  }
  EvPair &p = sl.ev[sl.ev_used++]; p.id = id;
  hipEventRecord(p.a, st);
  launch();
  hipEventRecord(p.b, st);
}

void Encoder::get_kernel_times(double *ms, uint64_t *launches, bool reset)
{
  std::lock_guard<std::mutex> l(stat_m_);
  for (int i = 0; i < K_COUNT; i++) { if (ms) ms[i] = k_ms_[i]; if (launches) launches[i] = k_n_[i]; }
  if (reset) for (int i = 0; i < K_COUNT; i++) { k_ms_[i] = 0; k_n_[i] = 0; }
}

bool Encoder::upload_and_submit(const uint8_t *y, const uint8_t *u, const uint8_t *v, bool pinned)
{
  const size_t ny = (size_t)cfg_.width * cfg_.height, bytes = ny * 3 / 2;
  const int k = (int)(in_count_++ % kInRing);
  if (!d_in_[k]) {
    HIP_CHECK(hipMalloc(&d_in_[k], bytes));
    HIP_CHECK(hipEventCreateWithFlags(&ev_h2d_[k], hipEventDisableTiming)); HIP_CHECK(hipEventCreateWithFlags(&ev_pad_[k], hipEventDisableTiming));
  }
  const uint8_t *src = y;
  if (!pinned) {
    if (!h_in_[k]) HIP_CHECK(hipHostMalloc(&h_in_[k], bytes, hipHostMallocDefault));
    if (h2d_pending_[k]) { Tick tk; HIP_CHECK(hipEventSynchronize(ev_h2d_[k])); h2d_pending_[k] = false; t_in_ += tk.ms(); }
    memcpy(h_in_[k], y, ny); memcpy(h_in_[k] + ny, u, ny / 4); memcpy(h_in_[k] + ny + ny / 4, v, ny / 4);
    src = h_in_[k];
  }
  if (pad_pending_[k]) {
    if (hipEventQuery(ev_pad_[k]) != hipSuccess) HIP_CHECK(hipStreamWaitEvent(stream_in_, ev_pad_[k], 0));
    pad_pending_[k] = false;
  }
  HIP_CHECK(hipMemcpyAsync(d_in_[k], src, bytes, hipMemcpyHostToDevice, stream_in_));
  HIP_CHECK(hipEventRecord(ev_h2d_[k], stream_in_)); h2d_pending_[k] = true;
  { Tick tk; if (!submit(d_in_[k], k)) return false; t_submit_ += tk.ms(); }
  in_pending_ = false;
  return true;
}

bool Encoder::encode_host(const uint8_t *y, const uint8_t *u, const uint8_t *v, EncodedPicture *out, bool pinned)
{
  const size_t ny = (size_t)cfg_.width * cfg_.height;
  HIP_CHECK(hipSetDevice(cfg_.device));
// ... 171 lines not shown
  if (gop_on() && !p.intra) {
    const int g = cfg_.gop_g, d = cfg_.gop_d, pos = ((poc_ - 1) % g) + 1;
    int layer = 1;
    while (layer < d && pos % (layer == 1 ? g : 1 << (d - layer)) != 0) layer++;
    p.layer = layer; p.qp = clip3(0, 51, qp_cur_ + layer);
    int n = 0; int8_t set[KVZ_MAX_LP_REFS];
    set[n++] = 1;
    if (p.nref >= 2) { const int key = ((poc_ - 2) / g) * g; if (poc_ - key <= kMaxRefDist) set[n++] = (int8_t)(poc_ - key); }
    for (int back = 2; n < p.nref; back++) { bool have = false; for (int k = 0; k < n; k++) have |= set[k] == back; if (!have) set[n++] = (int8_t)back; }
    for (int k = 0; k < n; k++) { int j = k; const int8_t v = set[k]; for (; j > 0 && set[j - 1] > v; j--) set[j] = set[j - 1]; set[j] = v; }
    for (int k = 0; k < KVZ_MAX_LP_REFS; k++) p.dist[k] = k < n ? set[k] : 1;
  }
  p.ahead = me_ahead_ && !p.intra;
  p.side = p.intra && (idr_side_ || (all_intra_alt_ && (frame_idx_ & 1)));
  p.ms = p.side ? stream_idr_ : stream_;
  return p;
}

EncFrame Encoder::picture_frame(const Plan &p, const Slot &sl, uint32_t chain_gen) const
{
  EncFrame f = base_;
  const int k = set_;
  const size_t nb8 = (size_t)cw_ * ch_ / 64;
  uint8_t *cu = cu_bytes_[k];
  for (int c = 0; c < 3; c++) { f.coef[c] = coef_[k][c]; f.src[c] = src_[k][c]; }
  f.cu_log2 = cu; f.cu_intra = cu + nb8; f.cu_flags = cu + 2 * nb8; f.cu_merge_idx = cu + 3 * nb8;
  f.cu_mvp_idx = cu + 4 * nb8; f.cu_intra_mode = cu + 5 * nb8; f.cu_cbf = cu + 6 * nb8;
  f.cu_mv = cu_mv_[k]; f.cu_mvd = cu_mvd_[k];
  f.cu_ref = cu_ref_[k];
  f.sao = sao_[k];
  f.ctu_qt = ctu_qt_[k]; f.ctu_qy = ctu_qy_[k]; f.ctu_delta = ctu_delta_[k]; f.ctu_first = ctu_first_[k];
  f.qp = p.qp; f.qpc = kChromaQp[p.qp]; f.lambda_q4 = kLambdaQ4[p.qp];
  f.is_intra = p.intra; f.poc = poc_;
  for (int c = 0; c < 3; c++) { f.rec[c] = cfg_.sao ? work_[c] : rec_[cur_idx_][c]; f.sao_out[c] = rec_[cur_idx_][c]; f.ref[c] = rec_[ref_idx_][c]; }
  f.me_ref = p.ahead ? src_[prev_set_][0] : f.ref[0];
  if (f.cu_ref) {
    f.nref = p.nref;
    for (int r = 0; r < KVZ_MAX_LP_REFS; r++) {
      const int back = r < f.nref ? p.dist[r] : 1, slot = (cur_idx_ + nrec_ - back) % nrec_;
      for (int c = 0; c < 3; c++) f.refs[r][c] = rec_[slot][c];
      f.me_refs[r] = p.ahead ? src_[(k + kSets - back) % kSets][0] : f.refs[r][0];
    }
  }
  if (gop_on() && !p.intra) f.ref_dist = (uint32_t)(uint8_t)p.dist[0] | (uint32_t)(uint8_t)p.dist[1] << 8 | (uint32_t)(uint8_t)p.dist[2] << 16 | (uint32_t)(uint8_t)p.dist[3] << 24;
  if (mc_q_[k]) {
    f.mc_rq = cfg_.me_coarse / 4; f.mc_q = mc_q_[k]; f.mc_centres = mc_centres_[k];
    const int nr = f.cu_ref ? f.nref : 1;
    for (int r = 0; r < KVZ_MAX_LP_REFS; r++) f.mc_qrefs[r] = mc_q_[(k + kSets - (r < nr ? p.dist[r] : 1)) % kSets];
  }
  if (wp_rec_[k] && !p.intra) f.wp = wp_rec_[k];
  if (col_[k] && !p.intra) { f.col_out = col_[k]; f.col_prev = poc_ >= 2 ? col_[(k + kSets - 1) % kSets] : nullptr; }
  if (p.ahead && me_block_[k]) { point_me_block(f, me_block_[k]); f.sync = sync_set_[k]; }
  f.tok_dense = sl.d_tok_dense; f.tok_count_out = sl.d_tok_count; f.tok_off_out = sl.d_tok_off; f.err_out = sl.d_err; f.ent_cursors = sl.g_cursors;
  f.tok_cursor = (uint32_t *)tok_count_ + (size_t)(frame_idx_ & 1) * tok_nctu_; f.tok_cursor_next = (uint32_t *)tok_count_ + (size_t)((frame_idx_ + 1) & 1) * tok_nctu_;
  f.chain_gen = chain_gen;
  if (p.side) {
    point_chain(f, sync_idr_, edge_col_idr_, edge_row_idr_);
    f.me_cand = nullptr;
    if (cfg_.sao) for (int c = 0; c < 3; c++) f.rec[c] = work_idr_[c];
  }
  return f;
}

bool Encoder::submit(const uint8_t *d_i420, int in_ring)
{
  Slot &sl = slot_[submitted_ % nslots_];
  cur_slot_ = &sl;
  prof_now_ = profiling_ && (frame_idx_ % prof_every_) == 0;
  const Plan p = plan((int)(submitted_ % kSets));
  const EncFrame f = picture_frame(p, sl, next_chain_gen());
  if (all_intra_alt_) idr_pending_ = false;
  if (!p.side && idr_pending_) { HIP_CHECK(hipStreamWaitEvent(stream_, ev_idr_done_, 0)); idr_pending_ = false; }
  return input_stage(f, p, d_i420, in_ring) && chain_stage(f, p) && hand_off(f, p, sl, in_ring);
}

bool Encoder::input_stage(const EncFrame &f, const Plan &p, const uint8_t *d_i420, int in_ring)
{
  if (src_busy_[set_]) { HIP_CHECK(hipStreamWaitEvent(stream_in_, ev_src_free_[set_], 0)); src_busy_[set_] = false; }
  timed(K_PAD, stream_in_, [&] { launch_pad_input(d_i420, cfg_.width, cfg_.height, src_[set_][0], src_[set_][1], src_[set_][2], cw_, ch_, stream_in_); });
  if (in_ring >= 0) { HIP_CHECK(hipEventRecord(ev_pad_[in_ring], stream_in_)); pad_pending_[in_ring] = true; }
  if (f.mc_rq) launch_luma_quarter(src_[set_][0], f.mc_q, cw_, ch_, stream_in_);
  if (cfg_.weightp && !wp_stage(f, p, *cur_slot_)) return false;
  if (tok_pending_[set_]) { HIP_CHECK(hipStreamWaitEvent(stream_in_, ev_tok_done_[set_], 0)); tok_pending_[set_] = false; }
  if (p.intra) {
    timed(K_INTRA_ANALYSE, stream_in_, [&] { launch_intra_analyse(f, stream_in_); });
  }
  if (f.mc_rq && !p.intra) launch_me_coarse(f, stream_in_);
  if (p.ahead) {
    const EncFrame fs = f.wp ? wp_search_frame(f, p, stream_in_) : f;
    timed(K_ME, stream_in_, [&] { launch_me(fs, stream_in_); });
    if (cfg_.intra_in_p) timed(K_INTRA_ANALYSE_P, stream_in_, [&] { launch_intra_analyse(f, stream_in_); });
  }
  if (!stage_roi(stream_in_)) return false;
  HIP_CHECK(hipEventRecord(in_done_, stream_in_)); in_pending_ = true;
  return true;
}

bool Encoder::chain_stage(const EncFrame &f, const Plan &p)
{
  const hipStream_t ms = p.ms;
  HIP_CHECK(hipStreamWaitEvent(ms, in_done_, 0));
  EncFrame fm = f;
  if (p.intra) { if (!picture_begin(f, ms, nullptr, true)) return false; }
  else if (!picture_begin(f, ms, p.ahead && cfg_.subme == 0 ? nullptr : &fm)) return false;
  if (p.intra) {
    timed(K_INTRA_RECON, ms, [&] { launch_intra_recon(f, ms); });
  } else {
// ... 59 lines not shown
  if (cfg_.entropy_gpu) {
    HIP_CHECK(hipEventRecord(sl.tok_ev, stream_tok_));
    HIP_CHECK(hipStreamWaitEvent(sl.ent_stream, sl.tok_ev, 0));
    const int nsub = cfg_.wpp ? rows_ : cfg_.tile_rows;
    CabacRowsArgs a;
    a.tok = sl.g_tok; a.count = sl.g_count; a.off = sl.g_off; a.stage = sl.g_stage; a.stage_cap = (uint32_t)stage_cap_; a.out = sl.d_out; a.out_cap = (uint32_t)out_cap_;
    a.cursors = sl.g_cursors; a.sub_off = sl.d_sub; a.sub_len = sl.d_sub + rows_; a.sub_bins = sl.d_sub + 2 * rows_;
    a.ctx_save = sl.g_ctx_save; a.ctx_ready = sl.g_ctx_ready; a.gen = ++sl.gen; a.err = err_;
    a.wc = cw_ / 64; a.hc = rows_; a.wpp = cfg_.wpp; a.tile_rows = cfg_.tile_rows; a.init_type = p.intra ? 0 : 1; a.qp = f.qp; a.first_sub = 0;
    timed(K_CABAC_ROWS, sl.ent_stream, [&] { launch_cabac_rows(a, nsub, sl.ent_stream); });
    HIP_CHECK(hipEventRecord(sl.done, sl.ent_stream));
  } else if (!tok_deferred_) HIP_CHECK(hipEventRecord(sl.done, stream_tok_));
  if (!cfg_.sao) HIP_CHECK(hipEventRecord(sl.rec_done, ms));
  sl.has_sink = false;
  if (sink_sub_[0] && in_ring >= 0) {
    if (!stream_rec_) HIP_CHECK(stream_acquire(&stream_rec_, cfg_.device, 'R', 'n'));
    if (!sl.sink_done) HIP_CHECK(hipEventCreateWithFlags(&sl.sink_done, hipEventDisableTiming));
    HIP_CHECK(hipStreamWaitEvent(stream_rec_, cfg_.sao ? ev_src_free_[set_] : sl.rec_done, 0));
    for (int c = 0; c < 3; c++) {
      const int pw = c ? cfg_.width / 2 : cfg_.width, ph = c ? cfg_.height / 2 : cfg_.height, cp = c ? cw_ / 2 : cw_;
      if (pw == cp) HIP_CHECK(hipMemcpyAsync(sink_sub_[c], rec_[cur_idx_][c], (size_t)pw * ph, hipMemcpyDeviceToHost, stream_rec_));
      else HIP_CHECK(hipMemcpy2DAsync(sink_sub_[c], (size_t)pw, rec_[cur_idx_][c], (size_t)cp, (size_t)pw, (size_t)ph, hipMemcpyDeviceToHost, stream_rec_));
    }
    HIP_CHECK(hipEventRecord(sl.sink_done, stream_rec_));
    sl.has_sink = true;
  }
  sink_sub_[0] = sink_sub_[1] = sink_sub_[2] = nullptr;
  sl.pic_idx = submitted_; sl.poc = poc_; sl.intra = p.intra; sl.rec_idx = cur_idx_; sl.qp = f.qp; sl.write_ps = false;
  if (sl_gop_timeline(p)) { char w[12]; snprintf(w, sizeof(w), "g%dq%02dd%d%d%d%d", p.layer, f.qp, p.nref > 0 ? p.dist[0] : 0, p.nref > 1 ? p.dist[1] : 0, p.nref > 2 ? p.dist[2] : 0, p.nref > 3 ? p.dist[3] : 0); tl(w, submitted_); }
  sl.layer = p.layer; sl.nref = gop_on() && !p.intra ? p.nref : 0; for (int r = 0; r < KVZ_MAX_LP_REFS; r++) sl.dist[r] = r < sl.nref ? p.dist[r] : 0;
  if (p.intra) {
    sl.write_ps = (intra_count_ == 0) || (cfg_.vps_period > 0 && (intra_count_ % cfg_.vps_period) == 0);
    intra_count_++;
  }
  frame_idx_++; prev_set_ = set_;
  ref_idx_ = cur_idx_; cur_idx_ = (cur_idx_ + 1) % nrec_;
  submitted_++;
  if (tok_deferred_) {
    { std::lock_guard<std::mutex> l(bm_); sl.ready = false; }
    { std::lock_guard<std::mutex> l(tm_); tq_.push_back((int)((submitted_ - 1) % nslots_)); }
    tcv_.notify_all();
  } else if (depth_ >= 2) {
    { std::lock_guard<std::mutex> l(bm_); sl.ready = false; bq_.push_back((int)((submitted_ - 1) % nslots_)); }
    bcv_.notify_all();
  }
  return true;
}

bool Encoder::launch_tokenizer(Slot &sl, const EncFrame &f, bool intra, bool wait_on_stream, bool prof)
{
  if (wait_on_stream) HIP_CHECK(hipStreamWaitEvent(stream_tok_, cfg_.sao ? ev_src_free_[sl.set] : ev_signalled_, 0));
  if (!intra) timed_slot(sl, prof, K_INTER_SIGNAL, stream_tok_, [&] { launch_inter_signal(f, stream_tok_); });
  timed_slot(sl, prof, K_TOKENIZE, stream_tok_, [&] { launch_tokenize(f, stream_tok_); });
  timed_slot(sl, prof, K_TOK_COMPACT, stream_tok_, [&] { launch_tok_compact(f, stream_tok_); });
  HIP_CHECK(hipEventRecord(ev_tok_done_[sl.set], stream_tok_));
  if (tok_deferred_) HIP_CHECK(hipEventRecord(sl.done, stream_tok_));
  return true;
}

void Encoder::tok_launcher()
{
  hipSetDevice(cfg_.device);
  for (;;) {
    int idx;
    { std::unique_lock<std::mutex> l(tm_); tcv_.wait(l, [&] { return tquit_ || !tq_.empty(); }); if (tq_.empty()) return; idx = tq_.front(); tq_.pop_front(); }
    Slot &sl = slot_[idx];
    hipEvent_t e = ev_src_free_[sl.set];
    const bool chain_ok = nap_until([&] { hipError_t r = hipEventQuery(e); return r == hipSuccess ? 1 : (r == hipErrorNotReady ? 0 : -1); });
    tl("tok0", sl.pic_idx);
    sl.tok_failed = !chain_ok || !launch_tokenizer(sl, sl.f_tok, sl.intra, false, sl.prof);
    if (sl.tok_failed) fprintf(stderr, chain_ok ? "kvazzup_amd: the tokenizer of picture %ld could not be launched\n" : "kvazzup_amd: the kernels of picture %ld failed; it is not entropy coded\n", sl.pic_idx);
    { std::lock_guard<std::mutex> l(bm_); bq_.push_back(idx); }
    bcv_.notify_all();
  }
}

bool Encoder::collect(EncodedPicture *out)
{
  Slot &sl = slot_[collected_ % nslots_];
  tl("col0", collected_);
  struct OnExit { long p; ~OnExit() { tl("col1", p); } } on_exit_{collected_};
  collected_++;
  bool ok;
  if (depth_ >= 2) {
    Tick tk;
    std::unique_lock<std::mutex> l(bm_);
    bcv_.wait(l, [&] { return sl.ready; });
    t_wait_ += tk.ms();
    ok = sl.ok;
    std::swap(*out, sl.result);
  } else ok = finish_slot(sl, out);
  out_idx_ = sl.rec_idx; out_set_ = sl.set;
  out_gop_[0] = gop_on(); out_gop_[1] = out->layer; out_gop_[2] = out->qp; out_gop_[3] = out->nref; for (int r = 0; r < KVZ_MAX_LP_REFS; r++) out_gop_[4 + r] = out->dist[r];
  memcpy(out_wp_, out->wp, sizeof(out_wp_));
  rc_bytes_[(collected_ - 1) & 7] = (uint32_t)out->au.size();
  return ok;
}

void Encoder::background(int worker)
{
  hipSetDevice(cfg_.device);
  for (;;) {
    int idx;
    { std::unique_lock<std::mutex> l(bm_); bcv_.wait(l, [&] { return bquit_ || !bq_.empty(); }); if (bq_.empty()) return; idx = bq_.front(); bq_.pop_front(); }
    Slot &sl = slot_[idx];
    tl("bg0", sl.pic_idx);
    const bool ok = finish_slot(sl, &sl.result, worker);
// ... 124 lines not shown
  if (cfg_.deblock) launch_deblock_v(f, stream_);
  HIP_CHECK(hipStreamSynchronize(stream_));
  return true;
}

size_t Encoder::halo_bytes() const { return (size_t)cw_ * 4 + (size_t)(cw_ / 2) * 2 * 2 + (size_t)(cw_ / 8) * 3 + (size_t)(cw_ / 8) * 4; }

bool Encoder::band_export_halo(uint8_t *d_up, uint8_t *d_down)
{
  const EncFrame &f = band_f_;
  const int Y0 = f.row0 * 64, Y1 = (f.row0 + band_rows(f)) * 64, b8w = f.b8w, cw2 = cw_ / 2;
  for (int side = 0; side < 2; side++) {
    uint8_t *dst = side ? d_down : d_up;
    if (!dst) continue;
    const int y = side ? Y1 - 4 : Y0, b8y = side ? Y1 / 8 - 1 : Y0 / 8;
    size_t o = 0;
    HIP_CHECK(hipMemcpyAsync(dst + o, f.rec[0] + (size_t)y * cw_, (size_t)cw_ * 4, hipMemcpyDeviceToDevice, stream_)); o += (size_t)cw_ * 4;
    for (int c = 1; c < 3; c++) { HIP_CHECK(hipMemcpyAsync(dst + o, f.rec[c] + (size_t)(y / 2) * cw2, (size_t)cw2 * 2, hipMemcpyDeviceToDevice, stream_)); o += (size_t)cw2 * 2; }
    const uint8_t *arr[3] = {f.cu_log2, f.cu_intra, f.cu_cbf};
    for (int k = 0; k < 3; k++) { HIP_CHECK(hipMemcpyAsync(dst + o, arr[k] + (size_t)b8y * b8w, (size_t)b8w, hipMemcpyDeviceToDevice, stream_)); o += (size_t)b8w; }
    HIP_CHECK(hipMemcpyAsync(dst + o, f.cu_mv + (size_t)b8y * b8w * 2, (size_t)b8w * 4, hipMemcpyDeviceToDevice, stream_));
  }
  HIP_CHECK(hipStreamSynchronize(stream_));
  return true;
}

bool Encoder::band_import_halo(const uint8_t *d_from_up, const uint8_t *d_from_down)
{
  const EncFrame &f = band_f_;
  const int Y0 = f.row0 * 64, Y1 = (f.row0 + band_rows(f)) * 64, b8w = f.b8w, cw2 = cw_ / 2;
  for (int side = 0; side < 2; side++) {
    const uint8_t *src = side ? d_from_down : d_from_up;
    if (!src) continue;
    const int y = side ? Y1 : Y0 - 4, b8y = side ? Y1 / 8 : Y0 / 8 - 1;
    if (y < 0 || y + 4 > ch_) return false;
    size_t o = 0;
    HIP_CHECK(hipMemcpyAsync(f.rec[0] + (size_t)y * cw_, src + o, (size_t)cw_ * 4, hipMemcpyDeviceToDevice, stream_)); o += (size_t)cw_ * 4;
    for (int c = 1; c < 3; c++) { HIP_CHECK(hipMemcpyAsync(f.rec[c] + (size_t)(y / 2) * cw2, src + o, (size_t)cw2 * 2, hipMemcpyDeviceToDevice, stream_)); o += (size_t)cw2 * 2; }
    uint8_t *arr[3] = {f.cu_log2, f.cu_intra, f.cu_cbf};
    for (int k = 0; k < 3; k++) { HIP_CHECK(hipMemcpyAsync(arr[k] + (size_t)b8y * b8w, src + o, (size_t)b8w, hipMemcpyDeviceToDevice, stream_)); o += (size_t)b8w; }
    HIP_CHECK(hipMemcpyAsync(f.cu_mv + (size_t)b8y * b8w * 2, src + o, (size_t)b8w * 4, hipMemcpyDeviceToDevice, stream_));
  }
  HIP_CHECK(hipStreamSynchronize(stream_));
  return true;
}

bool Encoder::band_phase2a()
{
  if (cfg_.band_rows <= 0) return false;
  HIP_CHECK(hipSetDevice(cfg_.device));
  const EncFrame &f = band_f_;
  Slot &sl = slot_[0];
  if (cfg_.deblock) launch_deblock_h(f, stream_, 1);
  launch_tokenize(f, stream_); launch_tok_compact(f, stream_);
  HIP_CHECK(hipStreamSynchronize(stream_));
  if (*sl.h_err) { fprintf(stderr, "kvazzup_amd: device error flags 0x%x\n", *sl.h_err); return false; }
  const int wc = cw_ / 64;
  for (int i = f.row0 * wc; i < (f.row0 + band_rows(f)) * wc; i++) if (sl.h_tok_count[i] < 0) { fprintf(stderr, "kvazzup_amd: token array overflow (CTU %d)\n", i); return false; }
  band_bins_ = 0;
  entropy_->code_band(sl.h_tok_dense, sl.h_tok_count, sl.h_tok_off, wc, rows_, cfg_.wpp != 0, cfg_.tile_rows, f.is_intra ? 0 : 1, qp_cur_,
                      f.row0, band_rows(f), band_subs_, &band_bins_);
  band_coded_ = true;
  return true;
}

bool Encoder::band_phase2b(std::vector<std::vector<uint8_t>> *substreams, EncodedPicture *info)
{
  if (cfg_.band_rows <= 0 || !substreams || !band_coded_) return false;
  HIP_CHECK(hipSetDevice(cfg_.device));
  if (cfg_.deblock) { launch_deblock_h(band_f_, stream_, 2); HIP_CHECK(hipStreamSynchronize(stream_)); }
  substreams->swap(band_subs_);
  band_coded_ = false;
  if (info) { info->valid = true; info->poc = poc_; info->qp = qp_cur_; info->is_intra = band_f_.is_intra; info->bins = band_bins_; info->au.clear(); }
  frame_idx_++;
  if (band_f_.is_intra) intra_count_++;
  ref_idx_ = cur_idx_; cur_idx_ = (cur_idx_ + 1) % nrec_; out_idx_ = ref_idx_;
  return true;
}

bool Encoder::band_phase2(std::vector<std::vector<uint8_t>> *substreams, EncodedPicture *info) { return band_phase2a() && band_phase2b(substreams, info); }

bool Encoder::download_recon(uint8_t *y, uint8_t *u, uint8_t *v)
{
  uint8_t *dst[3] = {y, u, v};
  HIP_CHECK(hipSetDevice(cfg_.device));
  if (!stream_rec_) HIP_CHECK(stream_acquire(&stream_rec_, cfg_.device, 'R', 'n'));
  if (pending() == 0) HIP_CHECK(hipStreamSynchronize(stream_));
  for (int c = 0; c < 3; c++) {
    int w = c ? cfg_.width / 2 : cfg_.width, h = c ? cfg_.height / 2 : cfg_.height, pw = c ? cw_ / 2 : cw_;
    if (w == pw) HIP_CHECK(hipMemcpyAsync(dst[c], rec_[out_idx_][c], (size_t)w * h, hipMemcpyDeviceToHost, stream_rec_));
    else HIP_CHECK(hipMemcpy2DAsync(dst[c], (size_t)w, rec_[out_idx_][c], (size_t)pw, (size_t)w, (size_t)h, hipMemcpyDeviceToHost, stream_rec_));
  }
  HIP_CHECK(hipStreamSynchronize(stream_rec_));
  return true;
}

bool Encoder::debug_copy(const char *what, void *dst, size_t bytes)
{
  const size_t npx = (size_t)cw_ * ch_, nb8 = npx / 64;
  const void *src = nullptr; size_t have = 0;
  std::string w(what);
  static const char *names[7] = {"cu_log2", "cu_intra", "cu_flags", "cu_merge_idx", "cu_mvp_idx", "cu_intra_mode", "cu_cbf"};
  for (int i = 0; i < 7; i++) if (w == names[i]) { src = cu_bytes_[out_set_] + i * nb8; have = nb8; }
  if (w == "lp_gop") { if (bytes > sizeof(out_gop_)) return false; memcpy(dst, out_gop_, bytes); return true; }
  if (w == "wp") { if (!cfg_.weightp || bytes > sizeof(out_wp_)) return false; memcpy(dst, out_wp_, bytes); return true; }
  if (w == "cu_mv") { src = cu_mv_[out_set_]; have = nb8 * 4; }
  if (w == "cu_mvd") { src = cu_mvd_[out_set_]; have = nb8 * 4; }
// ... 17 lines not shown
```

### kvazzup_amd/csrc/hevc_core.h

```cpp
#pragma once
#include "hevc_tables.h"

namespace kvzx {

KVZ_HD int iabs(int v) { return v < 0 ? -v : v; }
KVZ_HD int imin(int a, int b) { return a < b ? a : b; }
KVZ_HD int imax(int a, int b) { return a > b ? a : b; }
KVZ_HD int clip3(int lo, int hi, int v) { return v < lo ? lo : (v > hi ? hi : v); }
KVZ_HD int clip8(int v) { return v < 0 ? 0 : (v > 255 ? 255 : v); }
KVZ_HD int ilog2(unsigned v) { int n = 0; while (v > 1) { v >>= 1; n++; } return n; }
KVZ_HD int kv_clz32(uint32_t v) { return __builtin_clz(v); }
KVZ_HD int kv_ctz32(uint32_t v) { return __builtin_ctz(v); }

struct SaoParams {
  uint8_t type[3], eo_class[3], band_pos[3];
  int8_t offset[3][4];
};


#define KVZ_SCALING_BYTES 4064
KVZ_HD int scaling_offset(int log2n, int plane, int inter)
{
  switch (log2n) {
    case 2: return (3 * inter + plane) * 16;
    case 3: return 96 + (3 * inter + plane) * 64;
    case 4: return 480 + (3 * inter + plane) * 256;
    default: return 2016 + inter * 1024;
  }
}


#define KVZ_RC_ACC_STRIDE 16
#define KVZ_MAX_LP_REFS 4
struct RcState {
  uint32_t ratio_q8, ratio_valid, cost_sofar; uint32_t cost[8], cost_valid[8];
  alignas(128) uint32_t decided;
  alignas(128) unsigned long long acc[8 * KVZ_RC_ACC_STRIDE];
};
struct ColMv { int16_t mx, my, dist, pad; };
struct EncFrame {
  int cw, ch, b8w, b8h;
  int qp, qpc, lambda_q4, range;
  int is_intra, poc;
  int wpp;
  int satd;
  int me_early;
  int subme;
  const uint8_t *scaling;
  int lossless;
  int intra_chain;
  int intra_p;
  uint32_t *me_cost16;
  uint32_t *edge_col[3];
  unsigned long long *edge_row[3];
  uint32_t chain_gen;
  int analyse_alone;
  int chain_diags;
  uint32_t *ip_arrive; uint64_t *ip_scratch;
  uint32_t *me_cand;
  int rdoq, signhide;
  int slices;
  int mv_frame;
  int tile_rows;
  int tile_cols;
  int row0, nrows;
  int chp;
  const uint8_t *src[3];
  uint8_t *rec[3];
  const uint8_t *ref[3];
  const uint8_t *me_ref;
  int16_t *coef[3];
  uint8_t *cu_log2, *cu_intra, *cu_flags, *cu_merge_idx, *cu_mvp_idx, *cu_intra_mode, *cu_cbf;
  int16_t *cu_mv, *cu_mvd;
  uint8_t *im8, *im16, *im32; uint32_t *ic8, *ic16, *ic32;
  uint32_t *tok_list;
  uint16_t *tok_buf; int tok_cap; uint32_t *tok_cursor; uint32_t *tok_seg; uint32_t *tok_cursor_next;
  uint16_t *tok_dense; uint32_t tok_dense_cap; int32_t *tok_count_out; uint32_t *tok_off_out; uint32_t *err_out;
  uint32_t *ent_cursors;
  const int8_t *ctu_qt; int8_t *ctu_qy, *ctu_delta; uint8_t *ctu_first;
  SaoParams *sao; uint8_t *sao_out[3];
  uint32_t *sync;
  uint32_t *err;
  const uint32_t *intra_order;
  RcState *pb_rc; int8_t *pb_qt; const int8_t *pb_roi; uint32_t pb_bits3; int pb_nctu; int8_t pb_on, pb_slot3, pb_have3, pb_pad;
  RcState *rc; long long rc_target; int rc_nb, rc_slot;
  unsigned long long *trace;
  int nref;
  uint32_t ref_dist;
  uint8_t *cu_ref;
  const uint8_t *refs[KVZ_MAX_LP_REFS][3];
  const uint8_t *me_refs[KVZ_MAX_LP_REFS];
  ColMv *col_out;
  const ColMv *col_prev;
  int mc_rq;
  uint8_t *mc_q;
  const uint8_t *mc_qrefs[KVZ_MAX_LP_REFS];
  int16_t *mc_centres;
  const int32_t *wp;
};

KVZ_HD uint32_t wp_isqrt(uint64_t v)
{
  uint64_t r = 0, bit = (uint64_t)1 << 62;
  while (bit > v) bit >>= 2;
  while (bit) { if (v >= r + bit) { v -= r + bit; r = (r >> 1) + bit; } else r >>= 1; bit >>= 2; }
  return (uint32_t)r;
}
KVZ_HD void wp_moments(uint64_t s1, uint64_t s2, uint64_t n, int64_t *m, int64_t *v)
{
  const int64_t mm = (int64_t)((256 * s1 + n / 2) / n), q = (int64_t)((256 * s2 + n / 2) / n), vv = 256 * q - mm * mm;
  *m = mm; *v = vv < 0 ? 0 : vv;
}
KVZ_HD bool wp_candidate(int64_t m_c, int64_t v_c, int64_t m_r, int64_t v_r, int *w, int *o)
{
  int ww = 64;
  if (v_c != 0 && v_r != 0) ww = clip3(16, 127, (int)((wp_isqrt((uint64_t)(16384 * v_c) / (uint64_t)v_r) + 1) >> 1));
  const int64_t t = (64 * m_c - ww * m_r + 8192) >> 14;
  const int oo = t < -128 ? -128 : (t > 127 ? 127 : (int)t);
  *w = ww; *o = oo;
  return iabs(ww - 64) >= 2 || oo != 0;
}
KVZ_HD bool wp_accept(bool candidate, uint64_t plain, uint64_t wt) { return candidate && 16 * wt < 15 * plain; }
KVZ_HD int wp_sample(int s, int w, int o) { return clip8(((s * w + 32) >> 6) + o); }
KVZ_HD int wp_pred14(int p, int w, int o) { return clip8(((p * w + 2048) >> 12) + o); }

KVZ_HD const uint8_t *ref_plane(const EncFrame &f, int k, int c) { return f.cu_ref ? f.refs[k][c] : f.ref[c]; }
KVZ_HD int cu_ref_at(const EncFrame &f, int i) { return f.cu_ref ? f.cu_ref[i] : 0; }
KVZ_HD int ref_bins(int k, int n) { return n <= 1 ? 0 : (k < n - 1 ? k + 1 : n - 1); }

// ... 317 lines not shown
{
  int off, sh, mx = (log2 << 1) - 1;
  if (cidx == 0) { off = 3 * (log2 - 2) + ((log2 - 1) >> 2); sh = (log2 + 1) >> 2; }
  else { off = 15; sh = log2 - 2; }
  for (int i = 0; i < prefix; i++) cabac_bin(c, base + off + (i >> sh), 1);
  if (prefix < mx) cabac_bin(c, base + off + (prefix >> sh), 0);
}

template <class S>
KVZ_HD void enc_abs_remaining(S &c, int v, int rice)
{
  int q = v >> rice;
  if (q < 4) {
    cabac_bypass_bits(c, (1u << (q + 1)) - 2u, q + 1);
    if (rice) cabac_bypass_bits(c, (uint32_t)(v & ((1 << rice) - 1)), rice);
  } else {
    int x = v - (4 << rice), k = rice + 1, ones = 4;
    while (x >= (1 << k)) { x -= 1 << k; k++; ones++; }
    cabac_bypass_bits(c, (1u << (ones + 1)) - 2u, ones + 1);
    cabac_bypass_bits(c, (uint32_t)x, k);
  }
}

struct TuDigest {
  int16_t scan[64 * 16];
  uint16_t mask[64];
  uint8_t csbf[64];
  uint64_t sbmask;
};

KVZ_HD int scan_raster4(const CoreTabs *t, int scan_idx, int k) { return t->pos4[scan_idx][k]; }

KVZ_HD void digest_build_serial(const CoreTabs *t, TuDigest &d, const int16_t *lv, int stride, int log2, int scan_idx)
{
  const int sbl = log2 - 2, nsb2 = 1 << (2 * sbl);
  d.sbmask = 0;
  for (int i = 0; i < 64; i++) d.csbf[i] = 0;
  for (int i = 0; i < nsb2; i++) {
    int xs, ys; scan_pos(t, scan_idx, sbl, i, xs, ys);
    uint32_t m = 0;
    for (int k = 0; k < 16; k++) {
      const int r = t->pos4[scan_idx][k];
      const int16_t v = lv[((ys << 2) + (r >> 2)) * stride + (xs << 2) + (r & 3)];
      d.scan[i * 16 + k] = v;
      if (v) m |= 1u << k;
    }
    d.mask[i] = (uint16_t)m;
    d.csbf[ys * 8 + xs] = m != 0;
    if (m) d.sbmask |= 1ull << i;
  }
}

template <class S>
KVZ_HD void enc_last_pos(S &c, const TuDigest &d, int log2, int cidx, int scan_idx, int &last_sb, int &last_pos)
{
  const int sbl = log2 - 2;
  const CoreTabs *t = c.tabs;
  last_sb = 63;
  while (!((d.sbmask >> last_sb) & 1)) last_sb--;
  last_pos = 15;
  { uint32_t m = d.mask[last_sb]; while (!((m >> last_pos) & 1)) last_pos--; }
  int xs0, ys0, xp0, yp0;
  scan_pos(t, scan_idx, sbl, last_sb, xs0, ys0); scan_pos(t, scan_idx, 2, last_pos, xp0, yp0);
  int lx = (xs0 << 2) + xp0, ly = (ys0 << 2) + yp0;
  if (scan_idx == 2) { int tt = lx; lx = ly; ly = tt; }
  int pfx[2], nbs[2], sfx[2];
  for (int dd = 0; dd < 2; dd++) {
    int v = dd ? ly : lx;
    if (v < 4) { pfx[dd] = v; nbs[dd] = 0; sfx[dd] = 0; }
    else { int len = ilog2((unsigned)v); pfx[dd] = 2 * len + ((v >> (len - 1)) & 1); nbs[dd] = len - 1; sfx[dd] = v & ((1 << (len - 1)) - 1); }
  }
  enc_last_prefix(c, CTX_LAST_X, log2, cidx, pfx[0]);
  enc_last_prefix(c, CTX_LAST_Y, log2, cidx, pfx[1]);
  if (pfx[0] > 3) cabac_bypass_bits(c, (uint32_t)sfx[0], nbs[0]);
  if (pfx[1] > 3) cabac_bypass_bits(c, (uint32_t)sfx[1], nbs[1]);
}

KVZ_HD bool subblock_g1_any(const CoreTabs *, const TuDigest &d, int i, int)
{
  uint32_t mm = d.mask[i];
  for (int seen = 0; mm && seen < 8; seen++) {
    const int k = 31 - kv_clz32(mm); mm ^= 1u << k;
    const int v = d.scan[i * 16 + k];
    if (v > 1 || v < -1) return true;
  }
  return false;
}

template <class S>
KVZ_HD void enc_subblock(S &c, const TuDigest &d, int i, int last_sb, int last_pos, bool prev_g1, int log2, int cidx, int scan_idx, int sign_hiding = 0)
{
  const int sbl = log2 - 2, nsb = 1 << sbl;
  const CoreTabs *t = c.tabs;
  int xs, ys; scan_pos(t, scan_idx, sbl, i, xs, ys);
  const int right = (xs < nsb - 1) ? d.csbf[ys * 8 + xs + 1] : 0;
  const int below = (ys < nsb - 1) ? d.csbf[(ys + 1) * 8 + xs] : 0;
  const uint32_t m = d.mask[i];
  int coded = m != 0, infer_dc = 0;
  if (i < last_sb && i > 0) {
    cabac_bin(c, CTX_CSBF + ((right | below) ? 1 : 0) + (cidx ? 2 : 0), coded);
    infer_dc = 1;
  } else coded = 1;
  if (!coded) return;
  const uint8_t *pat = t->sigpat[right | (below << 1)], *pos = t->pos4[scan_idx];
  const int sigbase = CTX_SIG + (cidx ? 27 : 0);
  const int off = cidx == 0 ? ((i > 0 ? 3 : 0) + ((log2 == 3) ? ((scan_idx == 0) ? 9 : 15) : 21)) : ((log2 == 3) ? 9 : 12);
  const int start = (i == last_sb) ? last_pos - 1 : 15;
  if constexpr (sink_counts_only<S>::value) {
    if (start >= 0) c.n += start + 1 - ((infer_dc && (m >> 1) == 0) ? 1 : 0);
  } else {
    for (int k = start; k >= 0; k--) {
      if (k > 0 || !infer_dc) {
        const int p = pos[k];
        int sc;
// ... 621 lines not shown
```

Measured before the change: 9534.

## Rewrite tokenizer as per-CTU block with lane-parallel coefficient coding

Replaces the per-16x16-unit wave tokenizer, which coded coefficients sequentially per subblock, with one 1024-thread block per CTU. Each lane handles one coefficient, and ballot-derived masks compute significance, greater-than-1/2 and rice contexts in parallel, with token counts prefix-summed into a CTU stage buffer. The token list construction in the signalling kernel and the separate compaction kernel are removed. This cuts serial CABAC-token generation and extra kernel launches, at the cost of a large shared-memory footprint per block and more complex context derivation that must stay bit-exact.

```diff
diff --git a/kvazzup_amd/csrc/enc_kernels.h b/kvazzup_amd/csrc/enc_kernels.h
--- a/kvazzup_amd/csrc/enc_kernels.h
+++ b/kvazzup_amd/csrc/enc_kernels.h
@@ -18,7 +18,6 @@
 void launch_deblock_v(const EncFrame &f, hipStream_t st);
 void launch_deblock_h(const EncFrame &f, hipStream_t st, int part = 0);
 void launch_tokenize(const EncFrame &f, hipStream_t st);
-void launch_tok_compact(const EncFrame &f, hipStream_t st);
 void launch_picture_begin(RcState *rc, uint32_t bits3, int slot3, int have3, int8_t *ctu_qt, const int8_t *roi, int nctu, int qp, int vaq, hipStream_t st,
                           void *zero_a = nullptr, size_t bytes_a = 0, void *zero_b = nullptr, size_t bytes_b = 0);
 struct WpArgs {
diff --git a/kvazzup_amd/csrc/enc_kernels.hip b/kvazzup_amd/csrc/enc_kernels.hip
--- a/kvazzup_amd/csrc/enc_kernels.hip
+++ b/kvazzup_amd/csrc/enc_kernels.hip
@@ -3,6 +3,7 @@
 #include "hevc_core.h"
 #include "enc_kernels.h"
 #include "kernel_common.h"
+#include "tok_lanes.h"
 
 namespace kvzx {
 
@@ -764,29 +765,6 @@
       f.col_out[(y >> 4) * (f.cw >> 4) + (x >> 4)] = c;
     }
   }
-  if (f.tok_list) {
-    uint32_t roles = 0;
-    if (valid && !((x | y) & 15)) {
-      const bool owner = !(cl == 5 && ((x | y) & 31));
-      if (owner || ((x & 63) == 48 && (y & 63) == 48)) roles |= 8u;
-      if (owner) {
-        uint32_t cbf = 0;
-        if (cl == 3) { cbf = f.cu_cbf[g] | f.cu_cbf[g + 1] | f.cu_cbf[g + w8] | f.cu_cbf[g + w8 + 1]; }
-        else if (!(flags & CU_SKIP)) cbf = f.cu_cbf[g];
-        roles |= cbf & 7u;
-      }
-    }
-    const int lane = threadIdx.x & 63, nr = __builtin_popcount(roles);
-    int pre = nr;
-    for (int o = 1; o < 64; o <<= 1) { const int t = __shfl_up(pre, o); if (lane >= o) pre += t; }
-    const int total = __shfl(pre, 63);
-    uint32_t base = 0;
-    if (lane == 63 && total) base = atomicAdd(&f.tok_list[0], (uint32_t)total);
-    base = (uint32_t)__shfl((int)base, 63);
-    uint32_t o = base + (uint32_t)(pre - nr);
-    const uint32_t unit = (uint32_t)((y >> 4) * (f.cw >> 4) + (x >> 4));
-    for (uint32_t m = roles; m; m &= m - 1) f.tok_list[1 + o++] = (unit << 2) | (uint32_t)__builtin_ctz(m);
-  }
 }
 
 #ifdef KVZ_PROF
@@ -1532,12 +1510,6 @@
   }
 }
 
-struct TileView {
-  const CuRec *tile;
-  int bx0, by0;
-  __device__ CuRec at(int x, int y) const { return tile[((y >> 3) - by0) * 3 + ((x >> 3) - bx0)]; }
-};
-
 struct alignas(16) TokTabs { uint8_t sigk[3][5][16]; };
 constexpr CoreTabs make_core_tabs() { CoreTabs t{}; for (int i = 0; i < 64; i++) core_tabs_fill_entry(t, i); return t; }
 constexpr TokTabs make_tok_tabs()
@@ -1552,410 +1524,206 @@
 }
 static __device__ const CoreTabs g_core_tabs = make_core_tabs();
 static __device__ const TokTabs g_tok_tabs = make_tok_tabs();
-static_assert(sizeof(CoreTabs) % 4 == 0 && sizeof(TokTabs) % 16 == 0, "copied by dwords / 16-byte words");
-
-struct SbRegs { uint32_t w[8]; uint32_t m; };
-__device__ __forceinline__ int sb_level(const SbRegs &r, int k) { return (int)(int16_t)(uint16_t)(r.w[k >> 1] >> ((k & 1) * 16)); }
-
-template <bool KEEP_LDS>
-__device__ __forceinline__ void digest_build_wave(const CoreTabs *t, TuDigest &d, const int16_t *lv, int stride, int log2, int scan_idx, int lane, SbRegs &sb)
-{
-  const int sbl = log2 - 2, nsb2 = 1 << (2 * sbl);
-  d.csbf[lane] = 0;
-  wave_sync();
-  bool nz = false;
-  sb.m = 0;
-#pragma unroll
-  for (int k = 0; k < 8; k++) sb.w[k] = 0;
-  if (lane < nsb2) {
-    int xs, ys; scan_pos(t, scan_idx, sbl, lane, xs, ys);
-    const int16_t *p = lv + (ys << 2) * stride + (xs << 2);
-    uint2 r0 = *reinterpret_cast<const uint2 *>(p), r1 = *reinterpret_cast<const uint2 *>(p + stride);
-    uint2 r2 = *reinterpret_cast<const uint2 *>(p + 2 * stride), r3 = *reinterpret_cast<const uint2 *>(p + 3 * stride);
-    uint2 *dst = reinterpret_cast<uint2 *>(&d.scan[lane * 16]);
-    dst[0] = r0; dst[1] = r1; dst[2] = r2; dst[3] = r3;
-    const uint8_t *pos = t->pos4[scan_idx];
-    int v[16];
-    uint32_t m = 0;
-#pragma unroll
-    for (int k = 0; k < 16; k++) { v[k] = d.scan[lane * 16 + pos[k]]; if (v[k]) m |= 1u << k; }
-#pragma unroll
-    for (int k = 0; k < 8; k++) sb.w[k] = ((uint32_t)v[2 * k] & 0xffffu) | ((uint32_t)v[2 * k + 1] << 16);
-    if (KEEP_LDS) {
-      uint32_t *d32 = reinterpret_cast<uint32_t *>(&d.scan[lane * 16]);
-#pragma unroll
-      for (int k = 0; k < 8; k++) d32[k] = sb.w[k];
-    }
-    sb.m = m;
-    d.mask[lane] = (uint16_t)m;
-    nz = m != 0;
-    if (nz) d.csbf[ys * 8 + xs] = 1;
-  }
-  uint64_t sb64 = __ballot(nz);
-  if (lane == 0) d.sbmask = sb64;
-  wave_sync();
-}
-
-__device__ __forceinline__ bool sb_g1_any(const SbRegs &r)
-{
-  bool any = false; int seen = 0;
-#pragma unroll
-  for (int k = 15; k >= 0; k--) if ((r.m >> k) & 1) { const int v = sb_level(r, k); if (seen < 8 && (v > 1 || v < -1)) any = true; seen++; }
-  return any;
-}
-
-template <class S>
-__device__ __forceinline__ void enc_subblock_regs(S &c, const TuDigest &d, const SbRegs &r, const uint32_t (&sk)[4], int i, int last_sb, int last_pos, bool prev_g1, int log2, int cidx, int scan_idx, int sign_hiding)
-{
-  const int sbl = log2 - 2, nsb = 1 << sbl;
-  int xs, ys; scan_pos(c.tabs, scan_idx, sbl, i, xs, ys);
-  const int right = (xs < nsb - 1) ? d.csbf[ys * 8 + xs + 1] : 0;
-  const int below = (ys < nsb - 1) ? d.csbf[(ys + 1) * 8 + xs] : 0;
-  const uint32_t m = r.m;
-  int coded = m != 0, infer_dc = 0;
-  if (i < last_sb && i > 0) {
-    cabac_bin(c, CTX_CSBF + ((right | below) ? 1 : 0) + (cidx ? 2 : 0), coded);
-    infer_dc = 1;
-  } else coded = 1;
-  if (!coded) return;
-  const int sigbase = CTX_SIG + (cidx ? 27 : 0);
-  const int off = log2 == 2 ? 0 : (cidx == 0 ? ((i > 0 ? 3 : 0) + ((log2 == 3) ? ((scan_idx == 0) ? 9 : 15) : 21)) : ((log2 == 3) ? 9 : 12));
-  const int start = (i == last_sb) ? last_pos - 1 : 15;
-  if constexpr (sink_counts_only<S>::value) {
-    if (start >= 0) c.n += start + 1 - ((infer_dc && (m >> 1) == 0) ? 1 : 0);
-  } else {
-#pragma unroll
-    for (int k = 15; k >= 1; k--) if (k <= start) cabac_bin(c, sigbase + (int)((sk[k >> 2] >> ((k & 3) * 8)) & 0xffu) + off, (int)((m >> k) & 1));
-    if (start >= 0 && !(infer_dc && (m >> 1) == 0))
-      cabac_bin(c, sigbase + ((i == 0 && log2 != 2) ? 0 : (int)(sk[0] & 0xffu) + off), (int)(m & 1));
-  }
-  if (!m) return;
-  int ctx_set = (i > 0 && cidx == 0) ? 2 : 0;
-  if (prev_g1) ctx_set++;
-  int c1 = 1, nsig = 0, g1idx = -1, g2 = 0;
-  uint32_t signs = 0;
-#pragma unroll
-  for (int k = 15; k >= 0; k--) if ((m >> k) & 1) {
-    const int v = sb_level(r, k), a = v < 0 ? -v : v;
-    signs = (signs << 1) | (v < 0 ? 1u : 0u);
-    if (nsig < 8) {
-      const int g1 = a > 1;
-      cabac_bin(c, CTX_GT1 + (cidx ? 16 : 0) + ctx_set * 4 + c1, g1);
-      if (g1) { c1 = 0; if (g1idx < 0) { g1idx = nsig; g2 = a > 2; } }
-      else if (c1 > 0 && c1 < 3) c1++;
-    }
-    nsig++;
-  }
-  if (g1idx >= 0) cabac_bin(c, CTX_GT2 + (cidx ? 4 : 0) + ctx_set, g2);
-  if (sign_hiding && (31 - __builtin_clz(m)) - __builtin_ctz(m) > 3) cabac_bypass_bits(c, signs >> 1, nsig - 1);
-  else cabac_bypass_bits(c, signs, nsig);
-  int rice = 0, j = 0;
-#pragma unroll
-  for (int k = 15; k >= 0; k--) if ((m >> k) & 1) {
-    const int v = sb_level(r, k), a = v < 0 ? -v : v;
-    const int base = (j < 8) ? ((j == g1idx) ? 3 : 2) : 1;
-    if (a >= base) {
-      enc_abs_remaining(c, a - base, rice);
-      if (a > 3 * (1 << rice)) rice = imin(rice + 1, 4);
-    }
-    j++;
-  }
-}
-
-#define TOK_HDR_CAP 192
-#define TOK_ARENA 512
-#define TOK_PIECES 17
-
-#ifndef KVZ_TOK_WAVES
-#define KVZ_TOK_WAVES 5
-#endif
-struct alignas(16) TokWave {
-  TuDigest dg;
-  TokTabs tk;
-  CoreTabs tabs;
-  CuRec tile[9];
-  uint16_t hdr[TOK_HDR_CAP];
-  uint16_t arena[TOK_ARENA];
-  int hdr_n;
-  uint32_t piece_off;
-  uint32_t seg[TOK_PIECES][2];
-};
-template <bool ALLC, bool HDRW, bool REGS>
-__device__ __forceinline__ void tok_unit(const EncFrame &f, TokWave &W, const int ux, const int uy, const int comp, const int lane, const bool have_tabs)
-{
-  CuRec *tile = W.tile; TuDigest &dg = W.dg; CoreTabs &tabs = W.tabs; uint16_t *hdr = W.hdr, *arena = W.arena;
-  int &hdr_n = W.hdr_n; uint32_t &piece_off = W.piece_off; uint32_t (&seg)[TOK_PIECES][2] = W.seg;
+static __device__ const TokInvScan g_tok_inv = make_tok_inv_scan();
+
+__device__ __forceinline__ SbMasks tok_masks(int v, int g)
+{
+  const int a = v < 0 ? -v : v;
+  SbMasks s;
+  s.m = sb_mask_of(__ballot(v != 0), g); s.g1 = sb_mask_of(__ballot(a > 1), g); s.g2 = sb_mask_of(__ballot(a > 2), g); s.neg = sb_mask_of(__ballot(v < 0), g);
+  s.t = (uint64_t)sb_mask_of(__ballot(a > 3), g) | ((uint64_t)sb_mask_of(__ballot(a > 6), g) << 16) | ((uint64_t)sb_mask_of(__ballot(a > 12), g) << 32) | ((uint64_t)sb_mask_of(__ballot(a > 24), g) << 48);
+  return s;
+}
+__global__ __launch_bounds__(1024) void k_tokenize(EncFrame f)
+{
+  __shared__ TokCtu S;
+  const int tid = threadIdx.x, wv = tid >> 6, lane = tid & 63, g = lane >> 4, l16 = lane & 15, k = 15 - l16;
   const int wc = f.cw >> 6, hc = f.ch >> 6;
-  const int hdr_comp = HDRW ? 3 : 0;
-  const bool hdr_role = ALLC || comp == hdr_comp;
-  const int cx = ux >> 2, cy = uy >> 2, ctu = cy * wc + cx;
-  const int X0 = ux * 16, Y0 = uy * 16;
-  int z4 = 0;
-  for (int b = 0; b < 2; b++) z4 |= (((ux & 3) >> b) & 1) << (2 * b) | (((uy & 3) >> b) & 1) << (2 * b + 1);
-  unsigned long long *tr = (f.trace && hdr_role && lane == 0 && (z4 == 0 || z4 == 15)) ? f.trace + (size_t)wc * hc * 32 + (size_t)ctu * 8 : nullptr;
-  if (tr) tr[z4 == 0 ? 5 : 6] = wall_clock64();
-  unsigned long long *census = f.trace ? f.trace + (size_t)wc * hc * 40 + (size_t)ctu * 16 + (f.is_intra ? 6 : 0) : nullptr;
-  const unsigned long long t_begin = census ? wall_clock64() : 0;
-  int wave_class = 1;
-#ifdef KVZ_TOK_PHASES
-  unsigned long long *ph = (f.trace && comp == 0 && !f.is_intra) ? f.trace + (size_t)wc * hc * 56 + (size_t)ctu * 16 : nullptr;
-  unsigned long long ph_t[9]; int ph_n = 0;
-#define TOK_PH() do { if (ph && ph_n < 9) ph_t[ph_n++] = wall_clock64(); } while (0)
-#define TOK_PH_SYNC() wave_sync()
-#else
-#define TOK_PH() do { } while (0)
-#define TOK_PH_SYNC() do { } while (0)
-#endif
-  TOK_PH();
-  auto mine = [&](int piece) { return ALLC || ((piece == 16 || (piece & 3) == 0) ? hdr_comp : (piece & 3) - 1) == comp; };
-  if (!(hdr_role && z4 == 15)) {
-    const int g0 = (uy * 2) * f.b8w + ux * 2, l0 = f.cu_log2[g0];
-    bool work = !(l0 == 5 && ((X0 | Y0) & 31));
-    if (!ALLC && work && comp != hdr_comp) {
-      bool c = false;
-      if (lane < (l0 == 3 ? 4 : 1)) { const int g = g0 + (lane >> 1) * f.b8w + (lane & 1); c = !(f.cu_flags[g] & CU_SKIP) && ((f.cu_cbf[g] >> comp) & 1); }
-      work = __ballot(c) != 0;
-    }
-    if (!work) {
-      if (lane < TOK_PIECES && mine(lane)) { uint32_t *e = f.tok_seg + ((size_t)(ctu * 16 + z4) * TOK_PIECES + lane) * 2; e[0] = 0; e[1] = 0; }
-      if (census && lane == 0) { atomicAdd(&census[0], 1ull); atomicAdd(&census[1], wall_clock64() - t_begin); }
-      return;
-    }
-  }
-  TOK_PH();
-  if (!have_tabs) {
-    for (int i = lane; i < (int)(sizeof(CoreTabs) / 4); i += 64) reinterpret_cast<uint32_t *>(&tabs)[i] = reinterpret_cast<const uint32_t *>(&g_core_tabs)[i];
-    if (lane < (int)(sizeof(TokTabs) / 16)) reinterpret_cast<uint4 *>(&W.tk)[lane] = reinterpret_cast<const uint4 *>(&g_tok_tabs)[lane];
-  }
-  if (lane < TOK_PIECES) { seg[lane][0] = 0; seg[lane][1] = 0; }
-  if (lane == 0) hdr_n = 0;
-  const int bx0 = ux * 2 - 1, by0 = uy * 2 - 1;
-  if (lane < 9) {
-    int bx = bx0 + lane % 3, by = by0 + lane / 3;
+  const int ctu = (int)blockIdx.x + f.row0 * wc, cx = ctu % wc, cy = ctu / wc;
+  const int ux4 = (wv & 1) | ((wv >> 1) & 2), uy4 = ((wv >> 1) & 1) | ((wv >> 2) & 2);
+  if (tid < 81) {
+    const int bx = cx * 8 - 1 + tid % 9, by = cy * 8 - 1 + tid / 9;
     CuRec r; r.log2 = 0; r.intra = 0; r.flags = 0; r.merge_idx = 0; r.mvp_idx = 0; r.intra_mode = 0; r.cbf = 0; r.ref = 0; r.mvdx = 0; r.mvdy = 0;
-    if (bx >= 0 && by >= 0) {
-      int g = by * f.b8w + bx;
-      r.log2 = f.cu_log2[g]; r.intra = f.cu_intra[g]; r.flags = f.cu_flags[g]; r.merge_idx = f.cu_merge_idx[g];
-      r.mvp_idx = f.cu_mvp_idx[g]; r.intra_mode = f.cu_intra_mode[g]; r.cbf = f.cu_cbf[g];
-      r.mvdx = f.cu_mvd[g * 2]; r.mvdy = f.cu_mvd[g * 2 + 1]; r.ref = (uint8_t)cu_ref_at(f, g);
-    }
-    tile[lane] = r;
-  }
-  wave_sync();
-  TOK_PH();
-  uint16_t *slot = f.tok_buf + (size_t)ctu * f.tok_cap;
-  int np = 0;
-  auto reserve = [&](int total) -> uint32_t {
-    if (lane == 0) {
-      uint32_t o = atomicAdd(&f.tok_cursor[ctu], (uint32_t)total);
-      if (o + (uint32_t)total > (uint32_t)f.tok_cap) { atomicOr(f.err, 16u); o = ~0u; }
-      else { seg[np][0] = o; seg[np][1] = (uint32_t)total; }
-      piece_off = o;
-    }
+    if (bx >= 0 && by >= 0 && bx < f.b8w && by < f.b8h) {
+      const int gi = by * f.b8w + bx;
+      r.log2 = f.cu_log2[gi]; r.intra = f.cu_intra[gi]; r.flags = f.cu_flags[gi]; r.merge_idx = f.cu_merge_idx[gi];
+      r.mvp_idx = f.cu_mvp_idx[gi]; r.intra_mode = f.cu_intra_mode[gi]; r.cbf = f.cu_cbf[gi];
+      r.mvdx = f.cu_mvd[gi * 2]; r.mvdy = f.cu_mvd[gi * 2 + 1]; r.ref = (uint8_t)cu_ref_at(f, gi);
+    }
+    S.tile[tid] = r;
+  }
+  for (int i = tid; i < 3 * 64 * 2; i += 1024) { (&S.tb_nz[0][0][0])[i] = 0; (&S.tb_g1[0][0][0])[i] = 0; }
+  if (tid < 64) S.hdr_n[tid] = 0;
+  if (tid < 192) (&S.lp_n[0][0])[tid] = 0;
+  if (blockIdx.x == 0 && tid == 0) {
+    *f.err_out = *f.err;
+    if (f.ent_cursors) { f.ent_cursors[0] = 0; f.ent_cursors[1] = 0; }
+  }
+  __syncthreads();
+  CtuView view; view.tile = S.tile; view.bx0 = cx * 8 - 1; view.by0 = cy * 8 - 1;
+  const CuRec urec = S.tile[(uy4 * 2 + 1) * 9 + ux4 * 2 + 1];
+  const int ncu = (urec.log2 == 5 && ((ux4 | uy4) & 1)) ? 0 : (urec.log2 == 3 ? 4 : 1);
+  auto cu_header = [&](TokOut &t, int c, int z) {
+    const int x0 = cx * 64 + ux4 * 16 + (ncu == 4 ? (c & 1) * 8 : 0), y0 = cy * 64 + uy4 * 16 + (ncu == 4 ? (c >> 1) * 8 : 0);
+    const CuRec cu = view.at(x0, y0);
+    if (f.sao && z == 0) {
+      const bool hl = cx > 0 && !tile_col_starts_at(wc, f.tile_cols, cx), hu = cy > 0 && !tile_row_starts_at(hc, f.tile_rows, cy);
+      enc_sao(t, f.sao[ctu], hl ? &f.sao[ctu - 1] : nullptr, hu ? &f.sao[ctu - wc] : nullptr);
+    }
+    enc_split_flags(view, t, f.cw, f.chp, x0, y0, z, cu.log2);
+    enc_cu_header(view, t, f.cw, f.chp, f.is_intra != 0, x0, y0, cu, f.lossless != 0, f.cu_ref ? f.nref : 1);
+    if (f.ctu_qy && !(cu.flags & CU_SKIP) && cu.cbf && z == f.ctu_first[ctu]) enc_cu_qp_delta(t, f.ctu_delta[ctu]);
+  };
+  const int hdr_cap = TOK_HDR_SLOT << (2 * ((urec.log2 < 3 ? 3 : urec.log2 > 5 ? 5 : urec.log2) - 3));
+  int lv0 = 0, lv1 = 0, lv2 = 0, lv3 = 0, lv4 = 0, lv5 = 0;
+  auto level_of = [&](int it) { return it == 0 ? lv0 : it == 1 ? lv1 : it == 2 ? lv2 : it == 3 ? lv3 : it == 4 ? lv4 : lv5; };
+#pragma nounroll
+  for (int it = 0; it < 6; it++) {
+    const SbGeo q = tok_geo(S, g_tok_inv, ux4, uy4, it, g);
+    int v = 0;
+    if (q.coded) {
+      const int r = g_core_tabs.pos4[q.scan][k], sh = q.ci ? 1 : 0, pw = f.cw >> sh;
+      v = f.coef[q.ci][(size_t)(((cy * 64) >> sh) + q.SY * 4 + (r >> 2)) * pw + ((cx * 64) >> sh) + q.SX * 4 + (r & 3)];
+    }
+    if (it == 0) lv0 = v; else if (it == 1) lv1 = v; else if (it == 2) lv2 = v; else if (it == 3) lv3 = v; else if (it == 4) lv4 = v; else lv5 = v;
+    const SbMasks s = tok_masks(v, g);
+    if (l16 == 0) {
+      S.sbm[q.ci][q.SY * q.W + q.SX] = (uint16_t)s.m;
+      if (s.m) {
+        atomicOr(&S.tb_nz[q.ci][q.z8o][q.i >> 5], 1u << (q.i & 31));
+        if (sb_g1_any(s)) atomicOr(&S.tb_g1[q.ci][q.z8o][q.i >> 5], 1u << (q.i & 31));
+      }
+    }
+  }
+  if (lane < ncu) {
+    const int z = wv * 4 + lane;
+    TokOut t; t.tabs = &g_core_tabs; t.p = S.hdr + z * TOK_HDR_SLOT; t.n = 0; t.cap = hdr_cap;
+    cu_header(t, lane, z);
+    S.hdr_n[z] = (uint16_t)t.n;
+  }
+  __syncthreads();
+#pragma nounroll
+  for (int it = 0; it < 6; it++) {
+    const SbGeo q = tok_geo(S, g_tok_inv, ux4, uy4, it, g);
+    const int v = level_of(it), a = v < 0 ? -v : v;
+    const SbMasks s = tok_masks(v, g);
+    SbCtx c;
+    const bool on = tok_ctx(S, &g_core_tabs, q, f.signhide, c);
+    int n = 0, rem = 0;
+    if (on) {
+      const SbHead h = sb_head(c, s);
+      const SbLane l = sb_lane(c, s, h, k, a, g_tok_tabs.sigk[q.scan][q.l2 == 2 ? 4 : c.patt][k]);
+      n = h.head; rem = l.rem_n;
+    }
+    for (int o = 1; o < 16; o <<= 1) rem += __shfl_xor(rem, o, 16);
+    if (l16 == 0) {
+      S.cnt[q.idx] = (uint32_t)(n + rem);
+      if (on && c.i == c.last_sb) {
+        TokOut t; t.tabs = &g_core_tabs; t.p = S.lp[q.ci] + q.z8o * TOK_LP_SLOT; t.n = 0; t.cap = TOK_LP_SLOT << (2 * (q.l2 - (q.ci ? 2 : 3)));
+        enc_last_pos_at(t, q.l2, q.ci, q.scan, c.last_sb, c.last_pos);
+        S.lp_n[q.ci][q.z8o] = (uint8_t)(t.n < t.cap ? t.n : t.cap);
+      }
+    }
+  }
+  __syncthreads();
+  if (wv == 0) {
+    uint32_t loc[6], s = 0;
+#pragma unroll
+    for (int j = 0; j < 6; j++) { loc[j] = S.cnt[lane * 6 + j]; s += loc[j]; }
+    uint32_t inc = s;
+    for (int o = 1; o < 64; o <<= 1) { const uint32_t t = (uint32_t)__shfl_up((int)inc, o); if (lane >= o) inc += t; }
+    uint32_t run = inc - s;
+#pragma unroll
+    for (int j = 0; j < 6; j++) { S.cnt[lane * 6 + j] = run; run += loc[j]; }
+    if (lane == 63) S.cnt[384] = inc;
     wave_sync();
-    return piece_off;
-  };
-  TileView v; v.tile = tile; v.bx0 = bx0; v.by0 = by0;
-  const int cl0 = v.at(X0, Y0).log2;
-  const bool owner = !(cl0 == 5 && ((X0 | Y0) & 31));
-  const int ncu = owner ? (cl0 == 3 ? 4 : 1) : 0;
-  for (int k = 0; k < ncu; k++) {
-    const int x0 = X0 + ((cl0 == 3) ? (k & 1) * 8 : 0), y0 = Y0 + ((cl0 == 3) ? (k >> 1) * 8 : 0);
-    const CuRec cu = v.at(x0, y0);
-    int z = 0;
-    for (int b = 0; b < 3; b++) z |= ((((x0 & 63) >> 3) >> b) & 1) << (2 * b) | ((((y0 & 63) >> 3) >> b) & 1) << (2 * b + 1);
-    if (lane == 0 && hdr_role) {
-      TokOut t; t.tabs = &tabs; t.p = hdr; t.n = 0; t.cap = TOK_HDR_CAP;
-      if (f.sao && z4 == 0 && k == 0) {
-        const bool hl = cx > 0 && !tile_col_starts_at(wc, f.tile_cols, cx), hu = cy > 0 && !tile_row_starts_at(hc, f.tile_rows, cy);
-        enc_sao(t, f.sao[ctu], hl ? &f.sao[ctu - 1] : nullptr, hu ? &f.sao[ctu - wc] : nullptr);
-      }
-      enc_split_flags(v, t, f.cw, f.chp, x0, y0, z, cu.log2);
-      enc_cu_header(v, t, f.cw, f.chp, f.is_intra != 0, x0, y0, cu, f.lossless != 0, f.cu_ref ? f.nref : 1);
-      if (f.ctu_qy && !(cu.flags & CU_SKIP) && cu.cbf && z == f.ctu_first[ctu]) enc_cu_qp_delta(t, f.ctu_delta[ctu]);
-      hdr_n = t.n;
-    }
-    TOK_PH_SYNC(); TOK_PH();
-    if (hdr_role) {
-      np = 4 * k;
-      wave_sync();
-      const int hn = hdr_n > TOK_HDR_CAP ? TOK_HDR_CAP : hdr_n;
-      if (hdr_n > TOK_HDR_CAP && lane == 0) atomicOr(f.err, 8u);
-      const uint32_t o = reserve(hn);
-      if (o != ~0u) for (int i = lane; i < hn; i += 64) slot[o + i] = hdr[i];
-      wave_sync();
-      if (lane == 0) hdr_n = 0;
-      wave_sync();
-    }
-    const int cbf = (cu.flags & CU_SKIP) ? 0 : cu.cbf;
-    for (int ci = (ALLC || comp == 3) ? 0 : comp; ci < (ALLC ? 3 : (comp == 3 ? 0 : comp + 1)); ci++) {
-      np = 4 * k + 1 + ci;
-      if ((cbf >> ci) & 1) {
-        wave_class = 2;
-        const int l2 = ci ? cu.log2 - 1 : cu.log2, pw = ci ? (f.cw >> 1) : f.cw;
-        const int px = ci ? (x0 >> 1) : x0, py = ci ? (y0 >> 1) : y0;
-        const int scan = intra_scan_idx(cu.intra, l2, ci, cu.intra_mode);
-        SbRegs sb;
-        digest_build_wave<!REGS>(&tabs, dg, f.coef[ci] + py * pw + px, pw, l2, scan, lane, sb);
-        TOK_PH();
-        const uint64_t sbm = dg.sbmask;
-        const int last_sb = 63 - __builtin_clzll(sbm);
-        const int last_pos = 31 - __builtin_clz((uint32_t)dg.mask[last_sb]);
-        if (lane == 0) {
-          TokOut t; t.tabs = &tabs; t.p = hdr; t.n = hdr_n; t.cap = TOK_HDR_CAP;
-          int a, b; enc_last_pos(t, dg, l2, ci, scan, a, b);
-          hdr_n = t.n;
-        }
-        const bool nzsb = (sbm >> lane) & 1;
-        const bool g1 = nzsb && sb_g1_any(sb);
-        const uint64_t g1m = __ballot(g1);
-        bool prev_g1 = false;
-        if (lane <= last_sb) {
-          uint64_t above = (lane < 63) ? (sbm >> (lane + 1)) : 0;
-          if (above) { int j = lane + 1 + __builtin_ctzll(above); prev_g1 = (g1m >> j) & 1; }
-        }
-        uint32_t sk[4] = {0, 0, 0, 0};
-        if (lane <= last_sb) {
-          const int sbl = l2 - 2, nsb = 1 << sbl;
-          int xs, ys; scan_pos(&tabs, scan, sbl, lane, xs, ys);
-          const int right = (xs < nsb - 1) ? dg.csbf[ys * 8 + xs + 1] : 0, below = (ys < nsb - 1) ? dg.csbf[(ys + 1) * 8 + xs] : 0;
-          const uint4 q = *reinterpret_cast<const uint4 *>(W.tk.sigk[scan][l2 == 2 ? 4 : (right | (below << 1))]);
-          sk[0] = q.x; sk[1] = q.y; sk[2] = q.z; sk[3] = q.w;
-        }
-        int n_l = 0;
-        if (lane <= last_sb) {
-          TokCount t; t.tabs = &tabs; t.n = 0;
-          if (REGS) enc_subblock_regs(t, dg, sb, sk, lane, last_sb, last_pos, prev_g1, l2, ci, scan, f.signhide);
-          else enc_subblock(t, dg, lane, last_sb, last_pos, prev_g1, l2, ci, scan, f.signhide);
-          n_l = t.n;
-        }
-        int suffix = n_l;
-        for (int o = 1; o < 64; o <<= 1) { int other = __shfl_down(suffix, o); if (lane + o < 64) suffix += other; }
-        const int body = __shfl(suffix, 0);
-        const int off = suffix - n_l;
-        wave_sync();
-        const int hn = hdr_n > TOK_HDR_CAP ? TOK_HDR_CAP : hdr_n, total = hn + body;
-        if (hdr_n > TOK_HDR_CAP && lane == 0) atomicOr(f.err, 8u);
-        TOK_PH();
-        const uint32_t o = reserve(total);
-        TOK_PH();
-        if (o != ~0u) {
-          const bool staged = total <= TOK_ARENA;
-          uint16_t *dst = staged ? arena : slot + o;
-          for (int i = lane; i < hn; i += 64) dst[i] = hdr[i];
-          if (lane <= last_sb && n_l) {
-            TokOut t; t.tabs = &tabs; t.p = dst + hn + off; t.n = 0; t.cap = n_l;
-            if (REGS) enc_subblock_regs(t, dg, sb, sk, lane, last_sb, last_pos, prev_g1, l2, ci, scan, f.signhide);
-            else enc_subblock(t, dg, lane, last_sb, last_pos, prev_g1, l2, ci, scan, f.signhide);
-          }
-          if (staged) {
-            wave_sync();
-            for (int i = lane; i < total; i += 64) slot[o + i] = arena[i];
-          }
-        }
-        wave_sync();
-        TOK_PH();
-        if (lane == 0) hdr_n = 0;
-      }
-      wave_sync();
-    }
-  }
-  if (z4 == 15 && hdr_role) {
+    const int z = lane;
+    const CuRec cu = S.tile[(tok_unz(z >> 1) + 1) * 9 + tok_unz(z) + 1];
+    const int cl = cu.log2 < 3 ? 3 : (cu.log2 > 5 ? 5 : cu.log2);
+    const bool origin = !((tok_unz(z) | tok_unz(z >> 1)) & ((1 << (cl - 3)) - 1));
+    const bool res = origin && !(cu.flags & CU_SKIP);
+    auto piece_len = [&](int ci) -> uint32_t {
+      if (!res || !((cu.cbf >> ci) & 1)) return 0;
+      const int base = ci ? 256 + (ci - 1) * 64 + z : z * 4, nsb2 = 1 << (2 * ((ci ? cl - 1 : cl) - 2));
+      return S.lp_n[ci][z] + S.cnt[base + nsb2] - S.cnt[base];
+    };
+    const uint32_t p0 = S.hdr_n[z], p1 = piece_len(0), p2 = piece_len(1), p3 = piece_len(2);
+    const uint32_t ps = p0 + p1 + p2 + p3;
+    inc = ps;
+    for (int o = 1; o < 64; o <<= 1) { const uint32_t t = (uint32_t)__shfl_up((int)inc, o); if (lane >= o) inc += t; }
+    run = inc - ps;
+    S.pbase[z * 4] = run; S.pbase[z * 4 + 1] = run + p0; S.pbase[z * 4 + 2] = run + p0 + p1; S.pbase[z * 4 + 3] = run + p0 + p1 + p2;
+    if (lane == 63) {
+      S.pbase[256] = inc;
+      const uint32_t total = inc + 2;
+      S.total = (total > (uint32_t)f.tok_cap || (uint64_t)ctu * (uint32_t)f.tok_cap + total > f.tok_dense_cap) ? -1 : (int)inc;
+    }
+  }
+  __syncthreads();
+  if (S.total < 0) {
+    if (tid == 0) { f.tok_count_out[ctu] = -1; atomicOr(f.err, 16u); }
+    return;
+  }
+  uint16_t *const slot = f.tok_dense + (size_t)ctu * f.tok_cap;
+  int total = S.total;
+  int n_term = 0;
+  {
     const bool last = (cy == hc - 1 && cx == wc - 1);
     const bool row_end = tile_col_ends_at(wc, f.tile_cols, cx);
     const bool sub_end = row_end && (f.wpp || tile_row_ends_at(hc, f.tile_rows, cy));
     const bool seg_end = last || (row_end && (f.slices == 1 || (f.slices == 2 && tile_row_ends_at(hc, f.tile_rows, cy))));
-    const int n = 1 + ((sub_end && !seg_end) ? 1 : 0);
-    wave_sync();
-    np = 16;
-    const uint32_t o = reserve(n);
-    if (o != ~0u && lane == 0) {
-      slot[o] = (uint16_t)(0xC000u | (seg_end ? 1u : 0u));
-      if (n == 2) slot[o + 1] = 0xC001u;
-    }
-  }
-  wave_sync();
-  if (lane < TOK_PIECES && mine(lane)) {
-    uint32_t *e = f.tok_seg + ((size_t)(ctu * 16 + z4) * TOK_PIECES + lane) * 2;
-    e[0] = seg[lane][0]; e[1] = seg[lane][1];
-  }
-  TOK_PH();
-#ifdef KVZ_TOK_PHASES
-  if (ph && lane == 0 && ph_n == 9 && ncu == 1 && wave_class == 2) { for (int k = 0; k < 8; k++) atomicAdd(&ph[k], ph_t[k + 1] - ph_t[k]); atomicAdd(&ph[15], 1ull); }
-#endif
-#undef TOK_PH
-#undef TOK_PH_SYNC
-  if (tr && z4 == 15) tr[7] = wall_clock64();
-  if (census && lane == 0) { atomicAdd(&census[wave_class * 2], 1ull); atomicAdd(&census[wave_class * 2 + 1], wall_clock64() - t_begin); }
-}
-template <bool ALLC, int NW, bool HDRW = true, bool REGS = true, bool LIST = false>
-__global__ __launch_bounds__(NW * 64) __attribute__((amdgpu_waves_per_eu(REGS ? (LIST ? 3 : KVZ_TOK_WAVES) : 6))) void k_tokenize(EncFrame f)
-{
-  __shared__ TokWave tw[NW];
-  const int wv = threadIdx.x >> 6, lane = threadIdx.x & 63;
-  TokWave &W = tw[wv];
-  if constexpr (LIST) {
-    const uint32_t count = f.tok_list[0], uw = (uint32_t)(f.cw >> 4);
-    bool have = false;
-    for (uint32_t it = blockIdx.x; it < count; it += gridDim.x) {
-      const uint32_t v = f.tok_list[1 + it], unit = v >> 2;
-      tok_unit<ALLC, HDRW, REGS>(f, W, (int)(unit % uw), (int)(unit / uw), (int)(v & 3u), lane, have);
-      have = true;
-      wave_sync();
-    }
-  } else {
-    const int ux = NW == 4 ? blockIdx.x * 2 + (wv & 1) : blockIdx.x, uy = NW == 4 ? (blockIdx.y + f.row0 * 2) * 2 + (wv >> 1) : blockIdx.y + f.row0 * 4, comp = ALLC ? 0 : (int)blockIdx.z;
-    tok_unit<ALLC, HDRW, REGS>(f, W, ux, uy, comp, lane, false);
-  }
-}
-
-__global__ __launch_bounds__(256) void k_tok_compact(EncFrame f)
-{
-  constexpr int NSEG = 16 * TOK_PIECES;
-  __shared__ uint32_t soff[NSEG], start[NSEG + 1], utot[17];
-  __shared__ uint32_t wsum[4];
-  const int first = f.row0 * (f.cw >> 6), ctu = blockIdx.x + first, tid = threadIdx.x;
-  unsigned long long *tr = f.trace ? f.trace + (size_t)(f.cw >> 6) * (f.ch >> 6) * 32 + (size_t)ctu * 8 : nullptr;
-#define TC_STAMP(k) do { if (tr && tid == 0) tr[k] = wall_clock64(); } while (0)
-  TC_STAMP(0);
-  const uint32_t n = f.tok_cursor[ctu];
-  uint32_t part = 0;
-  for (int i = first + tid; i < ctu; i += 256) part += f.tok_cursor[i];
-  part = wave_sum_u32(part);
-  if ((tid & 63) == 0) wsum[tid >> 6] = part;
-  if (tid == 0) { f.tok_cursor_next[ctu] = 0; if (blockIdx.x == 0) { *f.err_out = *f.err; if (f.ent_cursors) { f.ent_cursors[0] = 0; f.ent_cursors[1] = 0; } } }
-  __syncthreads();
-  const uint32_t base = wsum[0] + wsum[1] + wsum[2] + wsum[3];
-  TC_STAMP(1);
-  uint32_t *tab = f.tok_seg + (size_t)ctu * NSEG * 2;
-  for (int i = tid; i < NSEG; i += 256) { const uint2 e = *reinterpret_cast<const uint2 *>(&tab[i * 2]); soff[i] = e.x; start[i] = e.y; *reinterpret_cast<uint2 *>(&tab[i * 2]) = make_uint2(0u, 0u); }
-  if (f.tok_list && blockIdx.x == 0 && tid == 0) f.tok_list[0] = 0;
-  if (base + n > f.tok_dense_cap) { if (tid == 0) f.tok_count_out[ctu] = -1; return; }
-  __syncthreads();
-  TC_STAMP(2);
-  if (tid < 16) { uint32_t a = 0; for (int p = 0; p < TOK_PIECES; p++) { uint32_t l = start[tid * TOK_PIECES + p]; start[tid * TOK_PIECES + p] = a; a += l; } utot[tid] = a; }
-  __syncthreads();
-  if (tid == 0) { uint32_t a = 0; for (int u = 0; u < 16; u++) { uint32_t t = utot[u]; utot[u] = a; a += t; } utot[16] = a; }
-  __syncthreads();
-  for (int i = tid; i < NSEG; i += 256) start[i] += utot[i / TOK_PIECES];
-  if (tid == 0) start[NSEG] = utot[16];
-  __syncthreads();
-  const uint32_t total = start[NSEG];
-  TC_STAMP(3);
-  if (total != n) { if (tid == 0) f.tok_count_out[ctu] = -1; return; }
-  const uint16_t *slot = f.tok_buf + (size_t)ctu * f.tok_cap;
-  uint16_t *dst = f.tok_dense + base;
-  int lo = 0;
-  for (uint32_t i = tid; i < n; i += 256) {
-    if (start[lo + 1] <= i) {
-      int hi = NSEG;
-      while (hi - lo > 1) { int mid = (lo + hi) >> 1; if (start[mid] <= i) lo = mid; else hi = mid; }
-    }
-    dst[i] = slot[soff[lo] + (i - start[lo])];
-  }
-  if (tid == 0) { f.tok_off_out[ctu] = base; f.tok_count_out[ctu] = (int32_t)n; }
-  TC_STAMP(4);
-#undef TC_STAMP
+    n_term = 1 + ((sub_end && !seg_end) ? 1 : 0);
+    const bool staged0 = total + n_term <= TOK_STAGE;
+    if (tid == 0) {
+      uint16_t *d = staged0 ? S.stage : slot;
+      d[total] = (uint16_t)(0xC000u | (seg_end ? 1u : 0u));
+      if (n_term == 2) d[total + 1] = 0xC001u;
+    }
+  }
+  total += n_term;
+  const bool staged = total <= TOK_STAGE;
+  uint16_t *const dst = staged ? S.stage : slot;
+  for (int c = 0; c < ncu; c++) {
+    const int z = wv * 4 + c, n = S.hdr_n[z];
+    uint16_t *d = dst + S.pbase[z * 4];
+    if (n <= hdr_cap) { for (int i = lane; i < n; i += 64) d[i] = S.hdr[z * TOK_HDR_SLOT + i]; }
+    else if (lane == 0) { TokOut t; t.tabs = &g_core_tabs; t.p = d; t.n = 0; t.cap = n; cu_header(t, c, z); }
+  }
+#pragma nounroll
+  for (int it = 0; it < 6; it++) {
+    const SbGeo q = tok_geo(S, g_tok_inv, ux4, uy4, it, g);
+    const int v = level_of(it), a = v < 0 ? -v : v;
+    const SbMasks s = tok_masks(v, g);
+    SbCtx c;
+    const bool on = tok_ctx(S, &g_core_tabs, q, f.signhide, c);
+    SbHead h{}; SbLane l{}; l.sig_off = -1; l.gt1_off = -1;
+    if (on) {
+      h = sb_head(c, s);
+      l = sb_lane(c, s, h, k, a, g_tok_tabs.sigk[q.scan][q.l2 == 2 ? 4 : c.patt][k]);
+    }
+    int inc = l.rem_n;
+    for (int o = 1; o < 16; o <<= 1) { const int t = __shfl_up(inc, o, 16); if (l16 >= o) inc += t; }
+    if (on) {
+      const int lpn = S.lp_n[q.ci][q.z8o];
+      uint16_t *piece = dst + S.pbase[q.z8o * 4 + 1 + q.ci];
+      if (c.i == c.last_sb) for (int j = l16; j < lpn; j += 16) piece[j] = S.lp[q.ci][q.z8o * TOK_LP_SLOT + j];
+      uint16_t *p = piece + lpn + (S.cnt[q.idx] - S.cnt[q.base]);
+      if (l.sig_off >= 0) p[l.sig_off] = (uint16_t)l.sig_tok;
+      if (l.gt1_off >= 0) p[l.gt1_off] = (uint16_t)l.gt1_tok;
+      if (l16 == 0) {
+        if (h.n_csbf) p[0] = (uint16_t)h.csbf_tok;
+        uint16_t *e = p + h.n_csbf + h.n_sig + h.n_gt1;
+        if (h.n_gt2) e[0] = (uint16_t)h.gt2_tok;
+        if (h.n_sign) { const uint32_t sg = sb_sign_tokens(s, h); e[h.n_gt2] = (uint16_t)sg; if (h.n_sign > 1) e[h.n_gt2 + 1] = (uint16_t)(sg >> 16); }
+      }
+      if (l.rem_n) { TokOut t; t.tabs = &g_core_tabs; t.p = p + h.head + (inc - l.rem_n); t.n = 0; t.cap = l.rem_n; enc_abs_remaining(t, l.rem_v, l.rice); }
+    }
+  }
+  if (staged) {
+    __syncthreads();
+    for (int i = tid; i < (total + 7) / 8; i += 1024) reinterpret_cast<uint4 *>(slot)[i] = reinterpret_cast<const uint4 *>(S.stage)[i];
+  }
+  if (tid == 0) { f.tok_off_out[ctu] = (uint32_t)ctu * (uint32_t)f.tok_cap; f.tok_count_out[ctu] = total; }
 }
 
 __global__ __launch_bounds__(256) void k_pad_input(const uint8_t *in, int w, int h, uint8_t *dy, uint8_t *du, uint8_t *dv, int cw, int ch)
@@ -2346,19 +2114,7 @@
 void launch_sao(const EncFrame &f, hipStream_t st) { hipLaunchKernelGGL(k_sao<false>, dim3((f.cw / 64) * (f.ch / 64)), dim3(KVZ_SAO_THREADS), 0, st, f); }
 void launch_tokenize(const EncFrame &f, hipStream_t st)
 {
-  const int units = (f.cw / 16) * band_rows(f) * 4;
-  static const int list_mode = [] { const char *e = getenv("KVAZZUP_AMD_TOK_LIST"); return e ? atoi(e) : -1; }();
-  if (!f.is_intra && f.tok_list && f.nrows == 0 && units < 65536 && (list_mode > 0 || (list_mode < 0 && units > 16384))) {
-    hipLaunchKernelGGL((k_tokenize<false, 1, true, true, true>), dim3(units / 2 < 256 ? 256 : units / 2), dim3(64), 0, st, f);
-    return;
-  }
-  if (units >= 65536) hipLaunchKernelGGL((k_tokenize<true, 1>), dim3(f.cw / 16, band_rows(f) * 4), dim3(64), 0, st, f);
-  else if (units > 16384) hipLaunchKernelGGL((k_tokenize<false, 1, false, false>), dim3(f.cw / 16, band_rows(f) * 4, 3), dim3(64), 0, st, f);
-  else hipLaunchKernelGGL((k_tokenize<false, 1, true>), dim3(f.cw / 16, band_rows(f) * 4, 4), dim3(64), 0, st, f);
-}
-void launch_tok_compact(const EncFrame &f, hipStream_t st)
-{
-  hipLaunchKernelGGL(k_tok_compact, dim3((f.cw / 64) * band_rows(f)), dim3(256), 0, st, f);
-}
-
-}
+  hipLaunchKernelGGL(k_tokenize, dim3((f.cw / 64) * band_rows(f)), dim3(1024), 0, st, f);
+}
+
+}
diff --git a/kvazzup_amd/csrc/encoder.h b/kvazzup_amd/csrc/encoder.h
--- a/kvazzup_amd/csrc/encoder.h
+++ b/kvazzup_amd/csrc/encoder.h
@@ -176,7 +176,7 @@
   hipEvent_t ev_signalled_ = nullptr, ev_tok_done_[kSets] = {}; bool tok_pending_[kSets] = {};
   uint8_t *intra_scratch_ = nullptr;
   uint8_t *d_scaling_ = nullptr;
-  uint16_t *tok_buf_ = nullptr; int tok_cap_ = 0; int32_t *tok_count_ = nullptr; uint32_t *tok_seg_ = nullptr; uint32_t *tok_list_ = nullptr; int tok_nctu_ = 0;
+  int tok_cap_ = 0;
   size_t tok_dense_cap_ = 0;
   std::vector<std::vector<uint8_t>> band_subs_; uint64_t band_bins_ = 0; bool band_coded_ = false;
   bool me_ahead_ = false; uint32_t *me_block_[kSets] = {}; uint32_t *sync_set_[kSets] = {}; int prev_set_ = 0;
diff --git a/kvazzup_amd/csrc/encoder.hip b/kvazzup_amd/csrc/encoder.hip
--- a/kvazzup_amd/csrc/encoder.hip
+++ b/kvazzup_amd/csrc/encoder.hip
@@ -159,12 +159,6 @@
   HIP_OK(hipMalloc(&intra_scratch_, isz));
   const int nctu = (cw_ / 64) * rows_;
   tok_cap_ = 49152;
-  HIP_OK(hipMalloc(&tok_buf_, (size_t)nctu * tok_cap_ * sizeof(uint16_t)));
-  HIP_OK(hipMalloc(&tok_count_, sizeof(uint32_t) * nctu * 2));
-  HIP_OK(hipMalloc(&tok_seg_, sizeof(uint32_t) * nctu * 16 * 17 * 2));
-  HIP_OK(hipMemset(tok_seg_, 0, sizeof(uint32_t) * nctu * 16 * 17 * 2));
-  if (cfg.band_rows == 0) { HIP_OK(hipMalloc(&tok_list_, sizeof(uint32_t) * (1 + (size_t)nctu * 16 * 4))); HIP_OK(hipMemset(tok_list_, 0, sizeof(uint32_t) * (1 + (size_t)nctu * 16 * 4))); }
-  HIP_OK(hipMemset(tok_count_, 0, sizeof(uint32_t) * nctu * 2)); tok_nctu_ = nctu;
   tok_dense_cap_ = (size_t)nctu * tok_cap_;
   if (tok_dense_cap_ > ((size_t)1 << 27)) tok_dense_cap_ = (size_t)1 << 27;
   spin_wait_ = getenv("KVAZZUP_AMD_SPIN") != nullptr;
@@ -249,7 +243,7 @@
   uint8_t *p = intra_scratch_;
   b.ic8 = (uint32_t *)p; p += nb8 * 4; b.ic16 = (uint32_t *)p; p += nb8; b.ic32 = (uint32_t *)p; p += nb8 / 4;
   b.im8 = p; p += nb8; b.im16 = p; p += nb8 / 4; b.im32 = p;
-  b.tok_buf = tok_buf_; b.tok_cap = tok_cap_; b.tok_seg = tok_seg_; b.tok_list = tok_list_; b.tok_dense_cap = (uint32_t)tok_dense_cap_;
+  b.tok_cap = tok_cap_; b.tok_dense_cap = (uint32_t)tok_dense_cap_;
   point_chain(b, sync_, edge_col_, edge_row_);
   b.err = err_; b.trace = trace_; b.intra_order = intra_order_;
   b.analyse_alone = depth_ < 2 && cfg.band_rows == 0 ? 1 : 0;
@@ -325,7 +319,7 @@
   hipFree(intra_scratch_); hipFree(d_scaling_);
   delete entropy_; delete entropy2_;
   for (int k = 0; k < kSets; k++) { hipFree(me_block_[k]); hipFree(sync_set_[k]); }
-  hipFree(trace_); hipFree(intra_order_); hipFree(tok_buf_); hipFree(tok_count_); hipFree(tok_seg_); hipFree(tok_list_); hipFree(sync_); hipFree(me_cost16_); hipFree(edge_col_); hipFree(err_);
+  hipFree(trace_); hipFree(intra_order_); hipFree(sync_); hipFree(me_cost16_); hipFree(edge_col_); hipFree(err_);
   stream_release(stream_, cfg_.device, 'M', prio_[0]);
 }
 
@@ -603,7 +597,6 @@
   if (col_[k] && !p.intra) { f.col_out = col_[k]; f.col_prev = poc_ >= 2 ? col_[(k + kSets - 1) % kSets] : nullptr; }
   if (p.ahead && me_block_[k]) { point_me_block(f, me_block_[k]); f.sync = sync_set_[k]; }
   f.tok_dense = sl.d_tok_dense; f.tok_count_out = sl.d_tok_count; f.tok_off_out = sl.d_tok_off; f.err_out = sl.d_err; f.ent_cursors = sl.g_cursors;
-  f.tok_cursor = (uint32_t *)tok_count_ + (size_t)(frame_idx_ & 1) * tok_nctu_; f.tok_cursor_next = (uint32_t *)tok_count_ + (size_t)((frame_idx_ + 1) & 1) * tok_nctu_;
   f.chain_gen = chain_gen;
   if (p.side) {
     point_chain(f, sync_idr_, edge_col_idr_, edge_row_idr_);
@@ -769,7 +762,6 @@
   if (wait_on_stream) HIP_CHECK(hipStreamWaitEvent(stream_tok_, cfg_.sao ? ev_src_free_[sl.set] : ev_signalled_, 0));
   if (!intra) timed_slot(sl, prof, K_INTER_SIGNAL, stream_tok_, [&] { launch_inter_signal(f, stream_tok_); });
   timed_slot(sl, prof, K_TOKENIZE, stream_tok_, [&] { launch_tokenize(f, stream_tok_); });
-  timed_slot(sl, prof, K_TOK_COMPACT, stream_tok_, [&] { launch_tok_compact(f, stream_tok_); });
   HIP_CHECK(hipEventRecord(ev_tok_done_[sl.set], stream_tok_));
   if (tok_deferred_) HIP_CHECK(hipEventRecord(sl.done, stream_tok_));
   return true;
@@ -1000,7 +992,7 @@
   const EncFrame &f = band_f_;
   Slot &sl = slot_[0];
   if (cfg_.deblock) launch_deblock_h(f, stream_, 1);
-  launch_tokenize(f, stream_); launch_tok_compact(f, stream_);
+  launch_tokenize(f, stream_);
   HIP_CHECK(hipStreamSynchronize(stream_));
   if (*sl.h_err) { fprintf(stderr, "kvazzup_amd: device error flags 0x%x\n", *sl.h_err); return false; }
   const int wc = cw_ / 64;
diff --git a/kvazzup_amd/csrc/hevc_core.h b/kvazzup_amd/csrc/hevc_core.h
--- a/kvazzup_amd/csrc/hevc_core.h
+++ b/kvazzup_amd/csrc/hevc_core.h
@@ -73,8 +73,7 @@
   uint8_t *cu_log2, *cu_intra, *cu_flags, *cu_merge_idx, *cu_mvp_idx, *cu_intra_mode, *cu_cbf;
   int16_t *cu_mv, *cu_mvd;
   uint8_t *im8, *im16, *im32; uint32_t *ic8, *ic16, *ic32;
-  uint32_t *tok_list;
-  uint16_t *tok_buf; int tok_cap; uint32_t *tok_cursor; uint32_t *tok_seg; uint32_t *tok_cursor_next;
+  int tok_cap;
   uint16_t *tok_dense; uint32_t tok_dense_cap; int32_t *tok_count_out; uint32_t *tok_off_out; uint32_t *err_out;
   uint32_t *ent_cursors;
   const int8_t *ctu_qt; int8_t *ctu_qy, *ctu_delta; uint8_t *ctu_first;
@@ -498,14 +497,21 @@
 }
 
 template <class S>
+KVZ_HD void enc_last_pos_at(S &c, int log2, int cidx, int scan_idx, int last_sb, int last_pos);
+template <class S>
 KVZ_HD void enc_last_pos(S &c, const TuDigest &d, int log2, int cidx, int scan_idx, int &last_sb, int &last_pos)
 {
-  const int sbl = log2 - 2;
-  const CoreTabs *t = c.tabs;
   last_sb = 63;
   while (!((d.sbmask >> last_sb) & 1)) last_sb--;
   last_pos = 15;
   { uint32_t m = d.mask[last_sb]; while (!((m >> last_pos) & 1)) last_pos--; }
+  enc_last_pos_at(c, log2, cidx, scan_idx, last_sb, last_pos);
+}
+template <class S>
+KVZ_HD void enc_last_pos_at(S &c, int log2, int cidx, int scan_idx, int last_sb, int last_pos)
+{
+  const int sbl = log2 - 2;
+  const CoreTabs *t = c.tabs;
   int xs0, ys0, xp0, yp0;
   scan_pos(t, scan_idx, sbl, last_sb, xs0, ys0); scan_pos(t, scan_idx, 2, last_pos, xp0, yp0);
   int lx = (xs0 << 2) + xp0, ly = (ys0 << 2) + yp0;
diff --git a/kvazzup_amd/csrc/tok_lanes.h b/kvazzup_amd/csrc/tok_lanes.h
--- /dev/null
+++ b/kvazzup_amd/csrc/tok_lanes.h
@@ -0,0 +1,197 @@
+#pragma once
+#include "hevc_core.h"
+
+namespace kvzx {
+
+struct TokInvScan { uint8_t d2[4], d4[16], d8[64]; };
+constexpr TokInvScan make_tok_inv_scan()
+{
+  TokInvScan t{};
+  for (int i = 0; i < 4; i++) t.d2[kDiag2y[i] * 2 + kDiag2x[i]] = (uint8_t)i;
+  for (int i = 0; i < 16; i++) t.d4[kDiag4y[i] * 4 + kDiag4x[i]] = (uint8_t)i;
+  for (int i = 0; i < 64; i++) t.d8[kDiag8y[i] * 8 + kDiag8x[i]] = (uint8_t)i;
+  return t;
+}
+KVZ_HD int scan_index(const TokInvScan &t, int scan_idx, int sbl, int xs, int ys)
+{
+  if (sbl == 0) return 0;
+  if (scan_idx == 1) return (ys << sbl) | xs;
+  if (scan_idx == 2) return (xs << sbl) | ys;
+  return sbl == 1 ? t.d2[ys * 2 + xs] : sbl == 2 ? t.d4[ys * 4 + xs] : t.d8[ys * 8 + xs];
+}
+
+struct SbCtx {
+  int i, last_sb, last_pos, log2, cidx, scan_idx, sign_hiding;
+  int patt;
+  bool prev_g1;
+};
+struct SbMasks { uint32_t m, g1, g2, neg; uint64_t t; };
+
+KVZ_HD uint32_t sb_mask_of(uint64_t ballot, int g)
+{
+#if defined(__HIP_DEVICE_COMPILE__)
+  return __brev((uint32_t)(ballot >> (g * 16)) << 16);
+#endif
+  uint32_t v = (uint32_t)(ballot >> (g * 16)) & 0xffffu, r = 0;
+  v = ((v & 0x5555u) << 1) | ((v >> 1) & 0x5555u); v = ((v & 0x3333u) << 2) | ((v >> 2) & 0x3333u);
+  v = ((v & 0x0f0fu) << 4) | ((v >> 4) & 0x0f0fu); r = ((v & 0x00ffu) << 8) | ((v >> 8) & 0x00ffu);
+  return r;
+}
+KVZ_HD int sb_popc(uint32_t v) { return __builtin_popcount(v); }
+KVZ_HD uint32_t sb_first8(uint32_t m) { for (int n = sb_popc(m); n > 8; n--) m &= m - 1; return m; }
+KVZ_HD bool sb_g1_any(const SbMasks &s) { return (s.g1 & sb_first8(s.m)) != 0; }
+
+struct SbHead {
+  int n_csbf, n_sig, n_gt1, n_gt2, n_sign, head;
+  int start, skip0;
+  int nsig, g1idx, ctx_set, sign_bits;
+  uint32_t csbf_tok, gt2_tok;
+};
+KVZ_HD SbHead sb_head(const SbCtx &c, const SbMasks &s)
+{
+  SbHead h{};
+  const uint32_t m = s.m;
+  h.start = -1; h.g1idx = -1;
+  bool infer_dc = false;
+  if (c.i < c.last_sb && c.i > 0) {
+    h.n_csbf = 1; h.csbf_tok = ((uint32_t)(CTX_CSBF + (c.patt ? 1 : 0) + (c.cidx ? 2 : 0)) << 1) | (m ? 1u : 0u);
+    infer_dc = true;
+    if (!m) { h.head = 1; return h; }
+  }
+  h.start = (c.i == c.last_sb) ? c.last_pos - 1 : 15;
+  h.skip0 = infer_dc && (m >> 1) == 0;
+  h.n_sig = h.start >= 0 ? h.start + 1 - (h.skip0 ? 1 : 0) : 0;
+  if (m) {
+    h.ctx_set = ((c.i > 0 && c.cidx == 0) ? 2 : 0) + (c.prev_g1 ? 1 : 0);
+    h.nsig = sb_popc(m);
+    h.n_gt1 = h.nsig < 8 ? h.nsig : 8;
+    const uint32_t gg = s.g1 & sb_first8(m);
+    if (gg) {
+      const int kk = 31 - kv_clz32(gg);
+      h.g1idx = sb_popc(m >> (kk + 1));
+      h.n_gt2 = 1; h.gt2_tok = ((uint32_t)(CTX_GT2 + (c.cidx ? 4 : 0) + h.ctx_set) << 1) | ((s.g2 >> kk) & 1u);
+    }
+    const bool hide = c.sign_hiding && (31 - kv_clz32(m)) - kv_ctz32(m) > 3;
+    h.sign_bits = h.nsig - (hide ? 1 : 0);
+    h.n_sign = (h.sign_bits + 9) / 10;
+  }
+  h.head = h.n_csbf + h.n_sig + h.n_gt1 + h.n_gt2 + h.n_sign;
+  return h;
+}
+KVZ_HD uint32_t sb_sign_tokens(const SbMasks &s, const SbHead &h)
+{
+  uint32_t signs = 0;
+  for (uint32_t mm = s.m; mm;) { const int k = 31 - kv_clz32(mm); mm ^= 1u << k; signs = (signs << 1) | ((s.neg >> k) & 1u); }
+  if (h.sign_bits < h.nsig) signs >>= 1;
+  const int n = h.sign_bits;
+  if (n <= 10) return 0x8000u | ((uint32_t)(n - 1) << 10) | (signs & ((1u << n) - 1u));
+  const int n2 = n - 10;
+  return (0x8000u | (9u << 10) | ((signs >> n2) & 0x3ffu)) | ((0x8000u | ((uint32_t)(n2 - 1) << 10) | (signs & ((1u << n2) - 1u))) << 16);
+}
+
+struct SbLane { int sig_off, gt1_off, rem_n, rem_v, rice; uint32_t sig_tok, gt1_tok; };
+KVZ_HD SbLane sb_lane(const SbCtx &c, const SbMasks &s, const SbHead &h, int k, int a, int sk)
+{
+  SbLane l{};
+  l.sig_off = -1; l.gt1_off = -1;
+  const uint32_t m = s.m;
+  if (k <= h.start && !(k == 0 && h.skip0)) {
+    const int off = c.log2 == 2 ? 0 : (c.cidx == 0 ? ((c.i > 0 ? 3 : 0) + ((c.log2 == 3) ? ((c.scan_idx == 0) ? 9 : 15) : 21)) : ((c.log2 == 3) ? 9 : 12));
+    const int sc = (k == 0 && c.i == 0 && c.log2 != 2) ? 0 : sk + off;
+    l.sig_off = h.n_csbf + (h.start - k);
+    l.sig_tok = ((uint32_t)(CTX_SIG + (c.cidx ? 27 : 0) + sc) << 1) | ((m >> k) & 1u);
+  }
+  if (!a || !((m >> k) & 1u)) return l;
+  const int j = sb_popc(m >> (k + 1));
+  if (j < 8) {
+    const int c1 = (s.g1 >> (k + 1)) ? 0 : (j < 2 ? 1 + j : 3);
+    l.gt1_off = h.n_csbf + h.n_sig + j;
+    l.gt1_tok = ((uint32_t)(CTX_GT1 + (c.cidx ? 16 : 0) + h.ctx_set * 4 + c1) << 1) | (a > 1 ? 1u : 0u);
+  }
+  const int base = (j < 8) ? ((j == h.g1idx) ? 3 : 2) : 1;
+  if (a >= base) {
+    int rice = 0; uint32_t below = 0xffffu;
+    while (rice < 4) {
+      const uint32_t cand = (uint32_t)(s.t >> (16 * rice)) & below;
+      if (!cand) break;
+      const int kk = 31 - kv_clz32(cand);
+      if (kk <= k) break;
+      rice++; below = (1u << kk) - 1u;
+    }
+    l.rice = rice; l.rem_v = a - base;
+    TokCount t; t.tabs = nullptr; t.n = 0;
+    enc_abs_remaining(t, l.rem_v, rice);
+    l.rem_n = t.n;
+  }
+  return l;
+}
+
+#define TOK_HDR_SLOT 64
+#define TOK_LP_SLOT 16
+#define TOK_STAGE 4096
+
+struct CtuView {
+  const CuRec *tile;
+  int bx0, by0;
+  KVZ_HD CuRec at(int x, int y) const { return tile[((y >> 3) - by0) * 9 + ((x >> 3) - bx0)]; }
+};
+struct alignas(16) TokCtu {
+  uint16_t stage[TOK_STAGE];
+  uint16_t hdr[64 * TOK_HDR_SLOT];
+  uint16_t lp[3][64 * TOK_LP_SLOT];
+  CuRec tile[81];
+  uint16_t sbm[3][256];
+  uint32_t tb_nz[3][64][2];
+  uint32_t tb_g1[3][64][2];
+  uint32_t cnt[385];
+  uint32_t pbase[257];
+  uint16_t hdr_n[64];
+  uint8_t lp_n[3][64];
+  int total;
+};
+KVZ_HD int tok_z8(int x, int y) { int z = 0; for (int b = 0; b < 3; b++) z |= ((x >> b) & 1) << (2 * b) | ((y >> b) & 1) << (2 * b + 1); return z; }
+KVZ_HD int tok_unz(int z) { return (z & 1) | ((z >> 1) & 2) | ((z >> 2) & 4); }
+
+struct SbGeo { int ci, SX, SY, W, l2, scan, xs, ys, nsb, i, z8o, base, idx; bool coded; };
+KVZ_HD SbGeo tok_geo(const TokCtu &S, const TokInvScan &inv, int ux4, int uy4, int it, int g)
+{
+  SbGeo q;
+  q.ci = it < 4 ? 0 : it - 3;
+  int bx, by;
+  if (q.ci == 0) { q.SX = ux4 * 4 + g; q.SY = uy4 * 4 + it; bx = q.SX >> 1; by = q.SY >> 1; q.W = 16; }
+  else { q.SX = ux4 * 2 + (g & 1); q.SY = uy4 * 2 + (g >> 1); bx = q.SX; by = q.SY; q.W = 8; }
+  const CuRec cu = S.tile[(by + 1) * 9 + bx + 1];
+  const int cl = cu.log2 < 3 ? 3 : (cu.log2 > 5 ? 5 : cu.log2);
+  q.l2 = q.ci ? cl - 1 : cl;
+  const int sbl = q.l2 - 2;
+  q.nsb = 1 << sbl;
+  q.xs = q.SX & (q.nsb - 1); q.ys = q.SY & (q.nsb - 1);
+  const int ox = q.SX - q.xs, oy = q.SY - q.ys;
+  q.z8o = q.ci ? tok_z8(ox, oy) : tok_z8(ox >> 1, oy >> 1);
+  q.scan = intra_scan_idx(cu.intra, q.l2, q.ci, cu.intra_mode);
+  q.i = scan_index(inv, q.scan, sbl, q.xs, q.ys);
+  q.coded = !(cu.flags & CU_SKIP) && ((cu.cbf >> q.ci) & 1);
+  q.base = q.ci ? 256 + (q.ci - 1) * 64 + q.z8o : q.z8o * 4;
+  q.idx = q.base + (1 << (2 * sbl)) - 1 - q.i;
+  return q;
+}
+KVZ_HD bool tok_ctx(const TokCtu &S, const CoreTabs *tabs, const SbGeo &q, int sign_hiding, SbCtx &c)
+{
+  const uint64_t nz = (uint64_t)S.tb_nz[q.ci][q.z8o][0] | ((uint64_t)S.tb_nz[q.ci][q.z8o][1] << 32);
+  if (!q.coded || !nz) return false;
+  const int last_sb = 63 - __builtin_clzll(nz);
+  if (q.i > last_sb) return false;
+  int lx, ly; scan_pos(tabs, q.scan, q.l2 - 2, last_sb, lx, ly);
+  const uint32_t lm = S.sbm[q.ci][(q.SY - q.ys + ly) * q.W + (q.SX - q.xs + lx)];
+  c.i = q.i; c.last_sb = last_sb; c.last_pos = 31 - __builtin_clz(lm | 1u);
+  c.log2 = q.l2; c.cidx = q.ci; c.scan_idx = q.scan; c.sign_hiding = sign_hiding;
+  const int right = (q.xs < q.nsb - 1) ? S.sbm[q.ci][q.SY * q.W + q.SX + 1] != 0 : 0, below = (q.ys < q.nsb - 1) ? S.sbm[q.ci][(q.SY + 1) * q.W + q.SX] != 0 : 0;
+  c.patt = right | (below << 1);
+  const uint64_t above = q.i < 63 ? nz >> (q.i + 1) : 0;
+  c.prev_g1 = false;
+  if (above) { const int j = q.i + 1 + __builtin_ctzll(above); c.prev_g1 = (S.tb_g1[q.ci][q.z8o][j >> 5] >> (j & 31)) & 1u; }
+  return true;
+}
+
+
+}
```

New measurement: 7165. 0.751x the previous value.
